# DerekGloudemans/3D-playground

Hardware: AMD Instinct MI355X
Metric: training images/sec at 1920x1080, ResNet-50 3D-RetinaNet (higher is better)
Workload: dtype f32; 1 GPU; resnet50 directional 3D-RetinaNet, 1920x1080 synthetic frames, batch 8 per GPU, 10 GT boxes/image, fp32, fwd+loss+bwd+clip+Adam (BASELINE configs[1]); global_batch=8, parallelism=dp1

## Files before the change

### 3d-playground_amd/csrc/conv_igemm_mf16.hip

```cpp
#include <type_traits>

#include "conv_igemm_tile.h"
#include "conv_wgrad_geom.h"

typedef float f32x4a __attribute__((ext_vector_type(4)));

#ifndef RN_MF16_STG
#define RN_MF16_STG 1
#endif
#ifndef RN_MF16_PF
#define RN_MF16_PF 1
#endif
#ifndef RN_MF16_KO
#define RN_MF16_KO 0
#endif

#define RN_SPLIT_MFMA16(ACC, A, B)                                                        \
    do {                                                                                  \
        ACC = __builtin_amdgcn_mfma_f32_16x16x32_bf16((A).l, (B).h, ACC, 0, 0, 0);        \
        ACC = __builtin_amdgcn_mfma_f32_16x16x32_bf16((A).h, (B).l, ACC, 0, 0, 0);        \
        ACC = __builtin_amdgcn_mfma_f32_16x16x32_bf16((A).m, (B).m, ACC, 0, 0, 0);        \
        ACC = __builtin_amdgcn_mfma_f32_16x16x32_bf16((A).m, (B).h, ACC, 0, 0, 0);        \
        ACC = __builtin_amdgcn_mfma_f32_16x16x32_bf16((A).h, (B).m, ACC, 0, 0, 0);        \
        ACC = __builtin_amdgcn_mfma_f32_16x16x32_bf16((A).h, (B).h, ACC, 0, 0, 0);        \
// ... 311 lines not shown
                        float4 t = *reinterpret_cast<const float4 *>(T + r * LDT + 4 * c4);
                        if constexpr (HALF) { const float ru = row_unscale[32 * wave + 16 * sm + hp * SR + r]; t.x *= ru; t.y *= ru; t.z *= ru; t.w *= ru; }
                        const int64_t off = off_[i];
                        float mk[4] = {mk_[i].x, mk_[i].y, mk_[i].z, mk_[i].w}, ad[4] = {ad_[i].x, ad_[i].y, ad_[i].z, ad_[i].w};
                        if (!RAW && d.add2_mode == 3) {
                            int64_t a2;
                            { RN_EPI_ADDR(GENERAL) a2 = a2off; (void)aoff; (void)off; }
                            if (a2 >= 0) { const float4 q = *reinterpret_cast<const float4 *>(add2 + a2); ad[0] += q.x; ad[1] += q.y; ad[2] += q.z; ad[3] += q.w; }
                        }
#if RN_MF16_KO & 4
                        if (t.x != 1.2345f) continue;
#endif
                        if (RAW) *reinterpret_cast<float4 *>(y + off) = HALF ? make_float4(t.x * sc[0], t.y * sc[1], t.z * sc[2], t.w * sc[3]) : t;
                        else { RN_EPI_FINISH() }
                    }
                }
            }
        }
        __builtin_amdgcn_fence(__ATOMIC_RELEASE, "wavefront");
        __builtin_amdgcn_wave_barrier();
    }
    if (!RAW && !rn_span) rn_amax_note(d.y_amax, m0 / HoWo, rn_am);
}

#ifndef RN_MF16H_OCC
#define RN_MF16H_OCC 3
#endif
template <bool GENERAL, bool RAW, int TERMS, bool STG, int WV = 4>
__global__ __launch_bounds__(64 * WV, WV == 8 ? 2 : (TERMS == 2 ? RN_MF16H_OCC : 3)) void conv_igemm_mf16_kernel(const rn_conv_desc d, const float *__restrict__ x,
                                                              const float *__restrict__ w, float *__restrict__ y,
                                                              const float *__restrict__ scale, const float *__restrict__ shift,
                                                              const float *__restrict__ add, const float *__restrict__ mask,
                                                              const float *__restrict__ add2) {
    conv_mf16_tile<GENERAL, RAW, TERMS, STG, WV>(d, x, w, y, scale, shift, add, mask, add2, xcd_remap(blockIdx.x, gridDim.x));
}

template <int TERMS>
__global__ __launch_bounds__(256, TERMS == 2 ? RN_MF16H_OCC : 3) void conv_igemm_mf16_grouped_kernel(const rn_conv_group g, const float *__restrict__ w,
                                                                      const float *__restrict__ scale,
                                                                      const float *__restrict__ shift) {
    const int tile = xcd_remap(blockIdx.x, gridDim.x);
    const int p = rn_group_index(g, tile);
    rn_conv_desc d = g.d[0];
    const float *x = g.x[0], *add = g.add[0], *mask = g.mask[0];
    float *y = g.y[0];
    int first = 0;
#pragma unroll
    for (int i = 1; i < RN_MAX_GROUP; ++i)
        if (p == i) { d = g.d[i]; x = g.x[i]; y = g.y[i]; add = g.add[i]; mask = g.mask[i]; first = g.tile_end[i - 1]; }
    conv_mf16_tile<true, false, TERMS, TERMS == 2 && RN_MF16_STG != 0>(d, x, w, y, scale, shift, add, mask, nullptr, tile - first);
}

static int mf16_on() { return rn_get_option(RN_OPT_MF16); }
static int mf16_min_tiles() { return rn_get_option(RN_OPT_MF16_MIN); }
static bool mf16_geom_ok(const rn_conv_desc *d) {
    return (d->Cin % 32) == 0 && d->div_shift == 0 && d->kh * d->kw <= 24 && (d->Cout % 4) == 0 && d->Cout > 64 && !d->in_relu;
}
static bool mf16_ok(const rn_conv_desc *d) {
    if (!mf16_on() || !mf16_geom_ok(d)) return false;
    if (d->w_format == 3) return d->x_amax != nullptr && d->w_unscale != nullptr;
    return d->w_format == 1;
}
static int64_t mf16_tiles(const rn_conv_desc *d) { return rn_conv_tiles(d, 128, 128); }

extern "C" int rn_conv_igemm_wants_f16(const rn_conv_desc *d) {
    return rn_get_fp32_mfma() == RN_FP32_SPLIT3 && d->w_batch_stride >= 0;
}

bool rn_igemm_mf16_launch(int variant, const rn_conv_desc *d, const float *x, const float *w, float *y, const float *scale,
                          const float *shift, const float *add, const float *mask, const float *add2, hipStream_t s, int *rc) {
    if (!mf16_ok(d) || (variant != 0 && variant != 4 && variant != 5)) return false;
    const int64_t tiles = mf16_tiles(d);
    if (tiles < mf16_min_tiles() || tiles > 0x7fffffff) return false;
    const dim3 grid((unsigned)tiles), block(256);
#define RN_MF16_LAUNCH(G, R, T, S) hipLaunchKernelGGL((conv_igemm_mf16_kernel<G, R, T, S>), grid, block, 0, s, *d, x, w, y, scale, shift, add, mask, add2)
    if (d->w_format == 3) {
        static const int stg_min_k = rn_env_int("RN_MF16_STG_MIN_K", 256);
        const bool stg = RN_MF16_STG != 0 && d->kh * d->kw * d->Cin >= stg_min_k;
        static const int wv8_min = rn_env_int("RN_MF16_WV8_MIN", 1);
        const int64_t tiles8 = rn_conv_tiles(d, 256, 128);
        if (stg && wv8_min > 0 && d->w_batch_stride == 0 && tiles8 >= wv8_min && tiles8 <= 0x7fffffff) {
            const dim3 grid8((unsigned)tiles8), block8(512);
#define RN_MF16_LAUNCH8(G, R) hipLaunchKernelGGL((conv_igemm_mf16_kernel<G, R, 2, true, 8>), grid8, block8, 0, s, *d, x, w, y, scale, shift, add, mask, add2)
            if (variant == 0) RN_MF16_LAUNCH8(false, true);
            else if (variant == 4) RN_MF16_LAUNCH8(false, false);
            else RN_MF16_LAUNCH8(true, false);
#undef RN_MF16_LAUNCH8
        } else
        if (variant == 0) { if (stg) RN_MF16_LAUNCH(false, true, 2, true); else RN_MF16_LAUNCH(false, true, 2, false); }
        else if (variant == 4) { if (stg) RN_MF16_LAUNCH(false, false, 2, true); else RN_MF16_LAUNCH(false, false, 2, false); }
        else { if (stg) RN_MF16_LAUNCH(true, false, 2, true); else RN_MF16_LAUNCH(true, false, 2, false); }
    } else {
        if (variant == 0) RN_MF16_LAUNCH(false, true, 3, false);
        else if (variant == 4) RN_MF16_LAUNCH(false, false, 3, false);
        else RN_MF16_LAUNCH(true, false, 3, false);
    }
#undef RN_MF16_LAUNCH
    const hipError_t e = hipGetLastError();
    *rc = e == hipSuccess ? RN_OK : (int)e;
    return true;
}

bool rn_igemm_mf16_grouped_launch(const rn_conv_group *g, const float *w, const float *scale, const float *shift, hipStream_t s, int *rc) {
    for (int i = 0; i < g->n; ++i)
        if (!mf16_ok(&g->d[i]) || g->d[i].w_format != g->d[0].w_format) return false;
    rn_conv_group gb = *g;
// ... 14 lines not shown
```

### 3d-playground_amd/csrc/conv_wgrad.hip

```cpp
#include <stdlib.h>
#include <type_traits>

#include "common.h"
#include "conv_wgrad_geom.h"

#ifndef RN_WG_KO
#define RN_WG_KO 0
#endif
#if RN_WG_KO == 1
#define RN_WG_ATOMIC(P, V) do { if ((V) == 1.2345e-30f) atomicAdd((P), (V)); } while (0)
#elif RN_WG_KO == 2
#define RN_WG_ATOMIC(P, V) __hip_atomic_fetch_add((P), (V), __ATOMIC_RELAXED, __HIP_MEMORY_SCOPE_WORKGROUP)
#else
#define RN_WG_ATOMIC(P, V) atomicAdd((P), (V))
#endif
#include "mfma_split.h"

typedef float f32x16 __attribute__((ext_vector_type(16)));
#define WK_MAX 32

struct WgradArgs {
    const float *dy, *x;
    float *dw;
    float *colsum;
    int ldy, N, Hi, Wi, Cin, Ho, Wo, Cout, kh, kw, stride, pad, in_relu;
    int Kflat, Kpad;
    int tiles_n;
    int tiles, splits;
    int xcd_map;
    int tiles_per_batch;
    int colsum_batch;
    int64_t dy_bstride, x_bstride, dw_bstride;
    int64_t pixels, per_split;
    float *slab, *cs_slab;
    int64_t slab_stride;
    const void *dy_amax, *x_amax;
    int dy_amax_n, x_amax_n;
};

__device__ __forceinline__ void wgrad_scales(const void *amax, int count, float &scale, float &unscale) {
    const int e = count > 0 ? rn_amax_exp_all(amax, count)
                            : (int)((__builtin_amdgcn_readfirstlane(*reinterpret_cast<const unsigned *>(amax)) >> 23) & 0xffu);
    const int se = rn_f16_scale_exp_of(e);
    scale = rn_exp_to_float(se);
    unscale = rn_exp_to_float(254 - se);
}

template <int WM, int WN, bool RELU, int WK, int OCC, bool SPLIT = false, bool HALF = false>
__global__ __launch_bounds__(256, OCC) void conv_wgrad_kernel(const WgradArgs p) {
    static_assert(!SPLIT || WK == 16, "split-operand form: 16-pixel K-steps");
    static_assert(!HALF || SPLIT, "the fp16 form is a split form");
    using G = WgradGeom<WM, WN, WK>;
    constexpr int BM = G::BM, BN = G::BN;
    constexpr int TB = G::TB;
    constexpr int CA = G::CA, CB = G::CB;
    constexpr int PA = G::PA, PB = G::PB;
    constexpr int IA = G::IA, IB = G::IB;
    __shared__ float lds[2][WK * (BM + BN)];
    __shared__ int4 pixtab[2][TB * WK];

    const int tid = threadIdx.x, lane = tid & 63, wave = tid >> 6;
    const int wm = wave / WN, wn = wave % WN;
    int slice, tile;
    if (p.xcd_map) {
        const int xcd = blockIdx.x & 7, wi = blockIdx.x >> 3;
        slice = (wi / p.tiles) * 8 + xcd;
        tile = wi % p.tiles;
    } else {
        slice = blockIdx.x / p.tiles;
        tile = blockIdx.x % p.tiles;
// ... 183 lines not shown
                if (c + 1 < p.Cout) atomicAdd(p.colsum + c + 1, cs.y);
            }
        }
    }
    float *out = dw_b;
    if (p.slab != nullptr) out = p.slab + (int64_t)slice * p.slab_stride + (int64_t)batch * p.dw_bstride;
#pragma unroll
    for (int tm = 0; tm < 2; ++tm)
#pragma unroll
        for (int tn = 0; tn < 2; ++tn) {
            const int col = n0 + wn * 64 + tn * 32 + (lane & 31);
#pragma unroll
            for (int e = 0; e < 16; ++e) {
                const int row = m0 + wm * 64 + 2 * ((e & 3) + 8 * (e >> 2) + 4 * (lane >> 5)) + tm;
                if (row < p.Cout && col < p.Kflat) {
                    const float v = HALF ? acc[tm][tn][e] * us : acc[tm][tn][e];
                    if (p.slab != nullptr) out[(int64_t)row * p.Kpad + col] = v;
                    else RN_WG_ATOMIC(out + (int64_t)row * p.Kpad + col, v);
                }
            }
        }
}

typedef short s16x4w __attribute__((ext_vector_type(4)));
__device__ __forceinline__ bf16x8 wgs_operand(const char *img, unsigned a0, unsigned a1) {
    typedef __attribute__((address_space(3))) s16x4w *lp;
    const s16x4w lo = __builtin_amdgcn_ds_read_tr16_b64_v4i16((lp)(__attribute__((address_space(3))) char *)(img + a0));
    const s16x4w hi = __builtin_amdgcn_ds_read_tr16_b64_v4i16((lp)(__attribute__((address_space(3))) char *)(img + a1));
    typedef short s16x8w __attribute__((ext_vector_type(8)));
    const s16x8w v = {lo[0], lo[1], lo[2], lo[3], hi[0], hi[1], hi[2], hi[3]};
    return __builtin_bit_cast(bf16x8, v);
}

template <bool RELU, bool HALF = false>
__global__ __launch_bounds__(256, 3) void conv_wgrad_once_kernel(const WgradArgs p) {
    using G = WgradSplitGeom;
    constexpr int BM = 128, BN = 128, WK = G::WK, TB = G::TB;
    constexpr int NP = HALF ? 2 : 3;
    constexpr int BUFB = 2 * NP * G::IMG;
    static_assert(BUFB <= G::BUF && 8 * BM * 4 <= BUFB, "planes fit; the column-sum reduction fits a buffer");
    __shared__ __attribute__((aligned(16))) char lds[2][BUFB];
    __shared__ int2 pixtab[2][TB * WK];

    const int tid = threadIdx.x, lane = tid & 63, wave = tid >> 6;
    const int wm = wave >> 1, wn = wave & 1;
    int slice, tile;
    if (p.xcd_map) {
        const int xcd = blockIdx.x & 7, wi = blockIdx.x >> 3;
        slice = (wi / p.tiles) * 8 + xcd;
        tile = wi % p.tiles;
    } else {
        slice = blockIdx.x / p.tiles;
        tile = blockIdx.x % p.tiles;
    }
    if (slice >= p.splits) return;
    const int batch = tile / p.tiles_per_batch;
    tile -= batch * p.tiles_per_batch;
    const float *dy_b = p.dy + (int64_t)batch * p.dy_bstride;
    const float *x_b = p.x + (int64_t)batch * p.x_bstride;
    float *dw_b = p.dw + (int64_t)batch * p.dw_bstride;
    const int m0 = (tile / p.tiles_n) * BM, n0 = (tile % p.tiles_n) * BN;
    const int64_t kbeg = (int64_t)slice * p.per_split;
    const int64_t kend = (kbeg + p.per_split < p.pixels) ? kbeg + p.per_split : p.pixels;
    const int nks = (int)((kend - kbeg + WK - 1) / WK);
    if (nks <= 0) return;
    const int HoWo = p.Ho * p.Wo;
    const int n_first = (int)(kbeg / HoWo);
    const int rel0 = (int)(kbeg - (int64_t)n_first * HoWo);
    const int64_t img = (int64_t)p.Hi * p.Wi * p.Cin;
    int64_t xbytes = ((int64_t)p.N - n_first) * img * 4;
    if (xbytes > 0x7FFFFFFF) xbytes = 0x7FFFFFFF;
    const __amdgpu_buffer_rsrc_t rs_a = __builtin_amdgcn_make_buffer_rsrc(const_cast<float *>(dy_b + kbeg * p.ldy), (short)0,
                                                                          (int)(unsigned)((kend - kbeg) * p.ldy * 4), 0x00020000);
    const __amdgpu_buffer_rsrc_t rs_b = __builtin_amdgcn_make_buffer_rsrc(const_cast<float *>(x_b + (int64_t)n_first * img), (short)0,
                                                                          (int)(unsigned)xbytes, 0x00020000);
    const int c = G::chunk(tid), px0 = G::pixel(tid, 0);
    const bool a_col_ok = (m0 + 4 * c) < p.ldy;
    const unsigned a_voff = a_col_ok ? (unsigned)((px0 * p.ldy + m0 + 4 * c) * 4) : 0x80000000u;
    const unsigned a_half = (unsigned)(8 * p.ldy * 4);
    const int jcol = n0 + 4 * c;
    const int tap = jcol / p.Cin;
    const int ci0 = jcol - tap * p.Cin;
    const int fr = tap / p.kw, fs = tap - fr * p.kw;
    const int fr_t = jcol < p.Kflat ? fr : (1 << 24);
    const int tap_off = ((fr * p.Wi + fs) * p.Cin + ci0) * 4;
    const unsigned wr0 = (unsigned)G::wr_addr(tid, 0), wr1 = (unsigned)G::wr_addr(tid, 1);

    auto fill_batch = [&](int j) {
        const int rel = rel0 + j * (TB * WK) + tid;
        int2 e = make_int2(0, 0x8000);
        if (kbeg + (int64_t)j * (TB * WK) + tid < kend) {
            const unsigned n = (unsigned)rel / (unsigned)HoWo;
            const unsigned rem = (unsigned)rel - n * (unsigned)HoWo;
            const unsigned oh = rem / (unsigned)p.Wo, ow = rem - oh * (unsigned)p.Wo;
            const int ih0 = (int)oh * p.stride - p.pad, iw0 = (int)ow * p.stride - p.pad;
            e = make_int2((((int)n * p.Hi + ih0) * p.Wi + iw0) * p.Cin * 4, (ih0 & 0xffff) | (iw0 << 16));
        }
        pixtab[j & 1][tid] = e;
    };
    typedef float f32x4v __attribute__((ext_vector_type(4)));
    struct Regs { f32x4v a[2], b[2]; };
    auto load_step = [&](int ks, Regs &r) {
        const int2 *tab = pixtab[(ks / TB) & 1];
        const unsigned so = (unsigned)ks * (unsigned)(WK * 4) * (unsigned)p.ldy;
        r.a[0] = __builtin_bit_cast(f32x4v, __builtin_amdgcn_raw_buffer_load_b128(rs_a, (int)a_voff, (int)so, 0));
        r.a[1] = __builtin_bit_cast(f32x4v, __builtin_amdgcn_raw_buffer_load_b128(rs_a, (int)a_voff, (int)(so + a_half), 0));
#pragma unroll
        for (int h = 0; h < 2; ++h) {
            const int2 e = tab[G::tab_index(ks, tid, h)];
            const int ih0 = (int)(short)(e.y & 0xffff), iw0 = e.y >> 16;
            const unsigned ok = (((unsigned)(ih0 + fr_t) < (unsigned)p.Hi) & ((unsigned)(iw0 + fs) < (unsigned)p.Wi)) ? 0xFFFFFFFFu : 0u;
            const unsigned v = ((unsigned)(e.x + tap_off) & ok) | (0x80000000u & ~ok);
            r.b[h] = __builtin_bit_cast(f32x4v, __builtin_amdgcn_raw_buffer_load_b128(rs_b, (int)v, 0, 0));
        }
    };
    float cs4[4] = {0.f, 0.f, 0.f, 0.f};
    const bool do_cs = p.colsum != nullptr && batch == p.colsum_batch && (tile % p.tiles_n) == 0;
    float s_a = 1.f, s_b = 1.f, us = 1.f;
    if constexpr (HALF) {
        float ua, ub;
        wgrad_scales(p.dy_amax, p.dy_amax_n, s_a, ua);
        wgrad_scales(p.x_amax, p.x_amax_n, s_b, ub);
        us = ua * ub;
    }
    auto split_store = [&](int buf, const Regs &r) {
        char *B = &lds[buf][0];
#pragma unroll
        for (int h = 0; h < 2; ++h) {
            const unsigned wr = h ? wr1 : wr0;
            float av[4] = {r.a[h][0], r.a[h][1], r.a[h][2], r.a[h][3]};
            float bv[4] = {r.b[h][0], r.b[h][1], r.b[h][2], r.b[h][3]};
            if (RELU) {
#pragma unroll
                for (int j = 0; j < 4; ++j) bv[j] = fmaxf(bv[j], 0.f);
            }
// ... 12 lines not shown
                *reinterpret_cast<uint2 *>(B + 2 * G::IMG + wr) = make_uint2(bh[0], bh[1]);
                *reinterpret_cast<uint2 *>(B + 3 * G::IMG + wr) = make_uint2(bl[0], bl[1]);
                continue;
            }
            unsigned ah[2], am[2], al[2], bh[2], bm[2], bl[2];
            split_pair(av[0], av[1], ah[0], am[0], al[0]);
            split_pair(av[2], av[3], ah[1], am[1], al[1]);
            split_pair(bv[0], bv[1], bh[0], bm[0], bl[0]);
            split_pair(bv[2], bv[3], bh[1], bm[1], bl[1]);
            *reinterpret_cast<uint2 *>(B + 0 * G::IMG + wr) = make_uint2(ah[0], ah[1]);
            *reinterpret_cast<uint2 *>(B + 1 * G::IMG + wr) = make_uint2(am[0], am[1]);
            *reinterpret_cast<uint2 *>(B + 2 * G::IMG + wr) = make_uint2(al[0], al[1]);
            *reinterpret_cast<uint2 *>(B + 3 * G::IMG + wr) = make_uint2(bh[0], bh[1]);
            *reinterpret_cast<uint2 *>(B + 4 * G::IMG + wr) = make_uint2(bm[0], bm[1]);
            *reinterpret_cast<uint2 *>(B + 5 * G::IMG + wr) = make_uint2(bl[0], bl[1]);
        }
    };
    unsigned fa[2][2], fb[2][2];
#pragma unroll
    for (int t = 0; t < 2; ++t)
#pragma unroll
        for (int rd = 0; rd < 2; ++rd) {
            fa[t][rd] = (unsigned)G::tr_addr(wm, t, rd, lane);
            fb[t][rd] = (unsigned)(NP * G::IMG + G::tr_addr(wn, t, rd, lane));
        }
    f32x16 acc[2][2];
#pragma unroll
    for (int i = 0; i < 2; ++i)
#pragma unroll
        for (int j = 0; j < 2; ++j)
#pragma unroll
            for (int e_ = 0; e_ < 16; ++e_) acc[i][j][e_] = 0.f;

    fill_batch(0);
    __syncthreads();
    Regs r0, r1;
    load_step(0, r0);
    split_store(0, r0);
    load_step(1, r0);
    __syncthreads();
    auto k_step = [&](int ks, int buf, Regs &cur, Regs &nxt) {
        const char *S = &lds[buf][0];
        if constexpr (HALF) {
            SplitH8 sa[2], sb[2];
#pragma unroll
            for (int t = 0; t < 2; ++t) {
                sa[t].h = __builtin_bit_cast(f16x8, wgs_operand(S, fa[t][0], fa[t][1]));
                sa[t].l = __builtin_bit_cast(f16x8, wgs_operand(S + G::IMG, fa[t][0], fa[t][1]));
                sb[t].h = __builtin_bit_cast(f16x8, wgs_operand(S, fb[t][0], fb[t][1]));
                sb[t].l = __builtin_bit_cast(f16x8, wgs_operand(S + G::IMG, fb[t][0], fb[t][1]));
            }
            split_store(buf ^ 1, cur);
            load_step(ks + 2, nxt);
#pragma unroll
            for (int tm = 0; tm < 2; ++tm)
#pragma unroll
                for (int tn = 0; tn < 2; ++tn) RN_SPLITH_MFMA(acc[tm][tn], sa[tm], sb[tn]);
        } else {
        Split8 sa[2], sb[2];
#pragma unroll
        for (int t = 0; t < 2; ++t) {
            sa[t].h = wgs_operand(S, fa[t][0], fa[t][1]);
            sa[t].m = wgs_operand(S + G::IMG, fa[t][0], fa[t][1]);
            sa[t].l = wgs_operand(S + 2 * G::IMG, fa[t][0], fa[t][1]);
            sb[t].h = wgs_operand(S, fb[t][0], fb[t][1]);
            sb[t].m = wgs_operand(S + G::IMG, fb[t][0], fb[t][1]);
            sb[t].l = wgs_operand(S + 2 * G::IMG, fb[t][0], fb[t][1]);
        }
        split_store(buf ^ 1, cur);
        load_step(ks + 2, nxt);
#pragma unroll
        for (int tm = 0; tm < 2; ++tm)
#pragma unroll
            for (int tn = 0; tn < 2; ++tn) RN_SPLIT_MFMA(acc[tm][tn], sa[tm], sb[tn]);
        }
        if ((ks % TB) == 4 && (ks / TB + 1) * TB < nks + 2) fill_batch(ks / TB + 1);
        __syncthreads();
    };
    for (int ks = 0; ks < nks; ks += 2) {
        k_step(ks, 0, r0, r1);
        if (ks + 1 < nks) k_step(ks + 1, 1, r1, r0);
    }
    if (do_cs) {
        float (*csred)[BM] = reinterpret_cast<float (*)[BM]>(&lds[0][0]);
#pragma unroll
        for (int j = 0; j < 4; ++j) csred[tid >> 5][4 * c + j] = cs4[j];
        __syncthreads();
        if (tid < BM) {
            float s_ = 0.f;
#pragma unroll
            for (int k = 0; k < 8; ++k) s_ += csred[k][tid];
            const int ch = m0 + tid;
            if (ch < p.Cout) {
                if (p.cs_slab != nullptr) p.cs_slab[(int64_t)slice * p.Cout + ch] = s_;
                else atomicAdd(p.colsum + ch, s_);
            }
        }
    }
    float *out = dw_b;
    if (p.slab != nullptr) out = p.slab + (int64_t)slice * p.slab_stride + (int64_t)batch * p.dw_bstride;
#pragma unroll
    for (int tm = 0; tm < 2; ++tm)
#pragma unroll
        for (int tn = 0; tn < 2; ++tn) {
            const int col = n0 + wn * 64 + tn * 32 + (lane & 31);
#pragma unroll
            for (int e = 0; e < 16; ++e) {
                const int row = m0 + wm * 64 + tm * 32 + (e & 3) + 8 * (e >> 2) + 4 * (lane >> 5);
                if (row < p.Cout && col < p.Kflat) {
                    const float v = HALF ? acc[tm][tn][e] * us : acc[tm][tn][e];
                    if (p.slab != nullptr) out[(int64_t)row * p.Kpad + col] = v;
                    else RN_WG_ATOMIC(out + (int64_t)row * p.Kpad + col, v);
                }
            }
        }
}

__global__ __launch_bounds__(256) void wgrad_combine_kernel(float *__restrict__ dw, const float *__restrict__ slab, int64_t slab_stride,
                                                            int splits, int nbatch, int64_t dw_bstride, int Cout, int Kflat, int Kpad,
                                                            float *__restrict__ colsum, const float *__restrict__ cs_slab) {
    const int64_t per = (int64_t)Cout * Kflat, total = per * nbatch;
    const int64_t i = (int64_t)blockIdx.x * 256 + threadIdx.x;
    if (i < total) {
        const int64_t b = i / per, r = i - b * per;
        const int row = (int)(r / Kflat), col = (int)(r - (int64_t)row * Kflat);
        const int64_t e = b * dw_bstride + (int64_t)row * Kpad + col;
        float v = dw[e];
        for (int s = 0; s < splits; ++s) v += slab[(int64_t)s * slab_stride + e];
        dw[e] = v;
    }
    if (colsum != nullptr && i < Cout) {
        float v = colsum[i];
        for (int s = 0; s < splits; ++s) v += cs_slab[(int64_t)s * Cout + i];
        colsum[i] = v;
    }
}

static int wgrad_launch(const float *dy, int ldy, const float *x, float *dw, float *colsum, int nbatch,
                        int64_t dy_bstride, int64_t x_bstride, int64_t dw_bstride, int colsum_batch, int N, int Hi,
                        int Wi, int Cin, int Ho, int Wo, int Cout, int kh, int kw, int stride, int pad,
                        int in_relu, void *stream, bool det, void *workspace, int64_t workspace_bytes, int64_t *need_bytes,
                        const void *dy_amax = nullptr, int dy_amax_n = 0, const void *x_amax = nullptr, int x_amax_n = 0);

extern "C" int rn_conv_wgrad_batched(const float *dy, int ldy, const float *x, float *dw, float *colsum, int nbatch,
                                     int64_t dy_bstride, int64_t x_bstride, int64_t dw_bstride, int colsum_batch, int N, int Hi,
                                     int Wi, int Cin, int Ho, int Wo, int Cout, int kh, int kw, int stride, int pad,
                                     int in_relu, const void *dy_amax, int dy_amax_n, const void *x_amax, int x_amax_n, void *stream) {
    return wgrad_launch(dy, ldy, x, dw, colsum, nbatch, dy_bstride, x_bstride, dw_bstride, colsum_batch, N, Hi, Wi, Cin, Ho, Wo, Cout,
                        kh, kw, stride, pad, in_relu, stream, false, nullptr, 0, nullptr, dy_amax, dy_amax_n, x_amax, x_amax_n);
}

extern "C" int rn_conv_wgrad_batched_det(const float *dy, int ldy, const float *x, float *dw, float *colsum, int nbatch,
                                         int64_t dy_bstride, int64_t x_bstride, int64_t dw_bstride, int colsum_batch, int N, int Hi,
                                         int Wi, int Cin, int Ho, int Wo, int Cout, int kh, int kw, int stride, int pad,
                                         int in_relu, const void *dy_amax, int dy_amax_n, const void *x_amax, int x_amax_n,
                                         void *workspace, int64_t workspace_bytes, void *stream) {
    if (workspace == nullptr) return RN_EINVAL;
    return wgrad_launch(dy, ldy, x, dw, colsum, nbatch, dy_bstride, x_bstride, dw_bstride, colsum_batch, N, Hi, Wi, Cin, Ho, Wo, Cout,
                        kh, kw, stride, pad, in_relu, stream, true, workspace, workspace_bytes, nullptr, dy_amax, dy_amax_n, x_amax, x_amax_n);
}

extern "C" int64_t rn_conv_wgrad_det_workspace_bytes(int ldy, int nbatch, int64_t dw_bstride, int N, int Hi, int Wi, int Cin, int Ho,
                                                     int Wo, int Cout, int kh, int kw) {
    int64_t need = 0;
    const int rc = wgrad_launch(nullptr, ldy, nullptr, nullptr, nullptr, nbatch, 0, 0, dw_bstride, 0, N, Hi, Wi, Cin, Ho, Wo, Cout, kh, kw,
                                1, 0, 0, nullptr, true, nullptr, 0, &need);
    return rc == RN_OK ? need : -1;
}

static int wgrad_launch(const float *dy, int ldy, const float *x, float *dw, float *colsum, int nbatch,
                        int64_t dy_bstride, int64_t x_bstride, int64_t dw_bstride, int colsum_batch, int N, int Hi,
                        int Wi, int Cin, int Ho, int Wo, int Cout, int kh, int kw, int stride, int pad,
                        int in_relu, void *stream, bool det, void *workspace, int64_t workspace_bytes, int64_t *need_bytes,
                        const void *dy_amax, int dy_amax_n, const void *x_amax, int x_amax_n) {
    if (N <= 0 || Hi <= 0 || Wi <= 0 || Ho <= 0 || Wo <= 0 || Cout <= 0 || Cin < 4 || (Cin & 3) || (ldy & 3) || ldy < Cout)
        return RN_EINVAL;
    if (nbatch < 1 || nbatch > 4096 || dy_bstride < 0 || x_bstride < 0 || dw_bstride < 0 || colsum_batch < 0 || colsum_batch >= nbatch)
        return RN_EINVAL;
    WgradArgs a;
    a.dy_bstride = dy_bstride; a.x_bstride = x_bstride; a.dw_bstride = dw_bstride; a.colsum_batch = colsum_batch;
    a.dy = dy; a.x = x; a.dw = dw; a.colsum = colsum; a.ldy = ldy;
    a.N = N; a.Hi = Hi; a.Wi = Wi; a.Cin = Cin; a.Ho = Ho; a.Wo = Wo; a.Cout = Cout;
    a.kh = kh; a.kw = kw; a.stride = stride; a.pad = pad; a.in_relu = in_relu;
    a.Kflat = kh * kw * Cin;
    a.Kpad = (a.Kflat + 31) / 32 * 32;
    a.pixels = (int64_t)N * Ho * Wo;
    const int shape = Cout <= 64 ? 0 : (a.Kflat <= 64 ? 1 : 2);
    const int BM = shape == 0 ? 64 : (shape == 1 ? 256 : 128), BN = shape == 0 ? 256 : (shape == 1 ? 64 : 128);
    const int tiles_m = (Cout + BM - 1) / BM;
    a.tiles_n = (a.Kflat + BN - 1) / BN;
    a.tiles_per_batch = tiles_m * a.tiles_n;
    const int tiles = a.tiles_per_batch * nbatch;
    static const int wgs_native = rn_env_int("RN_WGRAD_WGS", 2048);
    static const int wgs_split = rn_env_int("RN_WGRAD_SPLIT_WGS", 1536);
    const int wg_target = rn_get_fp32_mfma() != RN_FP32_NATIVE ? wgs_split : wgs_native;
    int64_t splits = (wg_target + tiles - 1) / tiles;
    const int64_t max_splits = (a.pixels + 16 * WK_MAX - 1) / (16 * WK_MAX);
    if (splits > max_splits) splits = max_splits;
    if (splits < 1) splits = 1;
    if (splits > 65535) splits = 65535;
    a.xcd_map = tiles >= 16 && splits > 8 && splits + 7 <= max_splits;
    if (a.xcd_map) splits = (splits + 7) / 8 * 8;
    const int64_t HoWo = (int64_t)Ho * Wo, img_bytes = (int64_t)Hi * Wi * Cin * 4;
    for (;;) {
        a.per_split = ((a.pixels + splits - 1) / splits + WK_MAX - 1) / WK_MAX * WK_MAX;
        const int64_t span_imgs = (a.per_split + HoWo - 2) / HoWo + 1;
        if ((a.per_split + WK_MAX) * ldy * 4 <= 0x7FFFFFFF && span_imgs * img_bytes <= 0x7FFFFFFF) break;
        if (a.per_split <= WK_MAX || splits >= 65535) return RN_EINVAL;
        splits = splits * 2 > 65535 ? 65535 : splits * 2;
        a.xcd_map = 0;
    }
    splits = (a.pixels + a.per_split - 1) / a.per_split;
    a.tiles = tiles;
    a.splits = (int)splits;
    a.slab = a.cs_slab = nullptr;
    a.slab_stride = 0;
    if (det) {
        a.slab_stride = nbatch > 1 ? (int64_t)nbatch * dw_bstride : (int64_t)Cout * a.Kpad;
        const int64_t need = splits * (a.slab_stride + Cout) * (int64_t)sizeof(float);
        if (need_bytes != nullptr) { *need_bytes = need; return RN_OK; }
        if (workspace_bytes < need) return RN_EINVAL;
        a.slab = reinterpret_cast<float *>(workspace);
        a.cs_slab = a.slab + splits * a.slab_stride;
    }
    const dim3 grid((unsigned)(tiles * (a.xcd_map ? (splits + 7) / 8 * 8 : splits)));
    const bool split = rn_get_fp32_mfma() != RN_FP32_NATIVE;
    const bool half = rn_get_fp32_mfma() == RN_FP32_SPLIT3 && dy_amax != nullptr && x_amax != nullptr && dy_amax_n != 0 && x_amax_n != 0;
    a.dy_amax = dy_amax;
    a.x_amax = x_amax;
    a.dy_amax_n = dy_amax_n;
    a.x_amax_n = x_amax_n;
#define RN_WGRAD_LAUNCH(WM_, WN_)                                                                                        \
    do {                                                                                                                 \
        if (half) {                                                                                                      \
            if (in_relu) hipLaunchKernelGGL((conv_wgrad_kernel<WM_, WN_, true, 16, 3, true, true>), grid, dim3(256), 0, (hipStream_t)stream, a);  \
            else hipLaunchKernelGGL((conv_wgrad_kernel<WM_, WN_, false, 16, 3, true, true>), grid, dim3(256), 0, (hipStream_t)stream, a);         \
        } else if (split) {                                                                                              \
            if (in_relu) hipLaunchKernelGGL((conv_wgrad_kernel<WM_, WN_, true, 16, 3, true>), grid, dim3(256), 0, (hipStream_t)stream, a);  \
            else hipLaunchKernelGGL((conv_wgrad_kernel<WM_, WN_, false, 16, 3, true>), grid, dim3(256), 0, (hipStream_t)stream, a);         \
        } else if (in_relu) hipLaunchKernelGGL((conv_wgrad_kernel<WM_, WN_, true, 16, 3>), grid, dim3(256), 0, (hipStream_t)stream, a);  \
        else hipLaunchKernelGGL((conv_wgrad_kernel<WM_, WN_, false, 16, 3>), grid, dim3(256), 0, (hipStream_t)stream, a);         \
    } while (0)
    const bool once = split && shape == 2 && rn_get_option(RN_OPT_WGRAD_ONCE) != 0 && Hi + pad < 32000 && Wi + pad < 32000;
    if (once && half) {
        if (in_relu) hipLaunchKernelGGL((conv_wgrad_once_kernel<true, true>), grid, dim3(256), 0, (hipStream_t)stream, a);
        else hipLaunchKernelGGL((conv_wgrad_once_kernel<false, true>), grid, dim3(256), 0, (hipStream_t)stream, a);
    } else if (once) {
        if (in_relu) hipLaunchKernelGGL((conv_wgrad_once_kernel<true>), grid, dim3(256), 0, (hipStream_t)stream, a);
        else hipLaunchKernelGGL((conv_wgrad_once_kernel<false>), grid, dim3(256), 0, (hipStream_t)stream, a);
    } else if (shape == 0) RN_WGRAD_LAUNCH(1, 4);
    else if (shape == 1) RN_WGRAD_LAUNCH(4, 1);
    else RN_WGRAD_LAUNCH(2, 2);
#undef RN_WGRAD_LAUNCH
    RN_LAUNCH_CHECK();
    if (det) {
        const int64_t total = (int64_t)nbatch * Cout * a.Kflat;
        hipLaunchKernelGGL(wgrad_combine_kernel, dim3((unsigned)((total + 255) / 256)), dim3(256), 0, (hipStream_t)stream, dw,
                           (const float *)a.slab, a.slab_stride, a.splits, nbatch, dw_bstride, Cout, a.Kflat, a.Kpad, colsum,
                           (const float *)a.cs_slab);
        RN_LAUNCH_CHECK();
    }
    return RN_OK;
}

extern "C" int rn_conv_wgrad(const float *dy, int ldy, const float *x, float *dw, float *colsum, int N, int Hi, int Wi,
                             int Cin, int Ho, int Wo, int Cout, int kh, int kw, int stride, int pad, int in_relu,
                             void *stream) {
    return rn_conv_wgrad_batched(dy, ldy, x, dw, colsum, 1, 0, 0, 0, 0, N, Hi, Wi, Cin, Ho, Wo, Cout, kh, kw, stride, pad,
                                 in_relu, nullptr, 0, nullptr, 0, stream);
}
```

### 3d-playground_amd/csrc/conv_wino.hip

```cpp
#include "common.h"
#include "mfma_split.h"

__device__ __forceinline__ float4 f4(float s) { return make_float4(s, s, s, s); }
typedef float nt_f4 __attribute__((ext_vector_type(4)));
__device__ __forceinline__ float4 ld_stream(const float *p) {
    const nt_f4 v = __builtin_nontemporal_load(reinterpret_cast<const nt_f4 *>(p));
    return make_float4(v.x, v.y, v.z, v.w);
}
__device__ __forceinline__ void st_stream(float *p, float4 v) { *reinterpret_cast<float4 *>(p) = v; }
__device__ __forceinline__ float4 operator+(float4 a, float4 b) { return make_float4(a.x + b.x, a.y + b.y, a.z + b.z, a.w + b.w); }
__device__ __forceinline__ float4 operator-(float4 a, float4 b) { return make_float4(a.x - b.x, a.y - b.y, a.z - b.z, a.w - b.w); }
__device__ __forceinline__ float4 operator*(float s, float4 a) { return make_float4(s * a.x, s * a.y, s * a.z, s * a.w); }

__device__ __forceinline__ void bt6(const float4 d[6], float4 o[6]) {
    o[0] = 4.f * d[0] - 5.f * d[2] + d[4];
    o[1] = d[3] + d[4] - 4.f * (d[1] + d[2]);
    o[2] = 4.f * (d[1] - d[2]) - d[3] + d[4];
    o[3] = 2.f * (d[3] - d[1]) - d[2] + d[4];
    o[4] = 2.f * (d[1] - d[3]) - d[2] + d[4];
    o[5] = 4.f * d[1] - 5.f * d[3] + d[5];
}
__device__ __forceinline__ void at6(const float4 m[6], float4 o[4]) {
    const float4 s12 = m[1] + m[2], d12 = m[1] - m[2], s34 = m[3] + m[4], d34 = m[3] - m[4];
    o[0] = m[0] + s12 + s34;
// ... 66 lines not shown
        const int e_img = rn_amax_exp_lanes(xw != nullptr ? reinterpret_cast<const unsigned char *>(xw) + (int64_t)n * RN_AMAX_BYTES : nullptr);
        if (gt_raw < t_last && c4 == 0) row_amax[t0 + gt] = rn_amax_word_of_exp(e_img, WINO_GAIN_BT);
    }
    if (gt_raw >= t_last) return;
    float4 t[6][6];
#pragma unroll
    for (int j = 0; j < 6; ++j) {
        float4 d[6], o[6];
        const int w = w0 + j;
#pragma unroll
        for (int i = 0; i < 6; ++i) {
            const int h = h0 + i;
#ifdef RN_WINO_ABL
            const bool ok = (unsigned)h < (unsigned)H && (unsigned)w < (unsigned)W && i >= 1 && i <= 4 && j >= 1 && j <= 4;
#else
            const bool ok = (unsigned)h < (unsigned)H && (unsigned)w < (unsigned)W;
#endif
            d[i] = ok ? *reinterpret_cast<const float4 *>(xb + ((int64_t)h * W + w) * C) : f4(0.f);
        }
        bt6(d, o);
#pragma unroll
        for (int i = 0; i < 6; ++i) t[i][j] = o[i];
    }
    float *vb = V + (t0 + gt) * C + c4;
#pragma unroll
    for (int i = 0; i < 6; ++i) {
        float4 o[6];
        bt6(t[i], o);
#pragma unroll
        for (int j = 0; j < 6; ++j) st_stream(vb + (int64_t)(i * 6 + j) * Tpad * C, o[j]);
    }
}

template <bool PBITS, bool PADD>
__global__ __launch_bounds__(256, 2) void wino_out_kernel(const WinoTable g, const float *__restrict__ M, int Cout, int64_t t0,
                                                       int64_t Tpad, const float *__restrict__ scale,
                                                       const float *__restrict__ shift, int mask_mode, int act, int64_t y_bs) {
    const int cq = Cout >> 2;
    const int64_t id = (int64_t)blockIdx.x * 256 + threadIdx.x;
    const int64_t gt = id / cq;
    float am = 0.f;
    unsigned *yam = nullptr;
    int n_img = 0;
    bool live = false;
    do {
    if (gt >= g.tile_end[g.n - 1]) break;
    live = true;
    const int c4 = (int)(id - gt * cq) * 4;
    int64_t tile;
    const int q = wino_locate(g, gt, tile);
    float *y = g.dst[0];
    const float *add = g.add[0], *mask = g.mask[0];
    unsigned *sign = g.sign[0];
    yam = g.amax[0];
    WINO_SELECT(q, g, pr, y = g.dst[i_]; add = g.add[i_]; mask = g.mask[i_]; sign = g.sign[i_]; yam = g.amax[i_];)
    n_img = (int)(tile / (pr.TH * pr.TW));
    const bool mbits = (mask_mode & RN_MASK_BITS) != 0;
    mask_mode &= 3;
    const int H = pr.H, W = pr.W, TW = pr.TW;
    const int n = (int)(tile / (pr.TH * TW));
    const int r = (int)(tile - (int64_t)n * pr.TH * TW);
    const int th = r / TW, tw = r - th * TW;
    const float *mb = M + (t0 + gt) * Cout + c4;
    float4 t[4][6];
#pragma unroll
    for (int j = 0; j < 6; ++j) {
        float4 m[6], o[4];
#pragma unroll
        for (int i = 0; i < 6; ++i) m[i] = ld_stream(mb + (int64_t)(i * 6 + j) * Tpad * Cout);
        at6(m, o);
#pragma unroll
        for (int i = 0; i < 4; ++i) t[i][j] = o[i];
    }
    float4 sc = f4(1.f), sh = f4(0.f);
    if (scale) sc = *reinterpret_cast<const float4 *>(scale + c4);
    if (shift) sh = *reinterpret_cast<const float4 *>(shift + c4);
    const int64_t ybs = y_bs ? y_bs : (int64_t)H * W * Cout;
#pragma unroll
    for (int i = 0; i < 4; ++i) {
        float4 o[4];
        at6(t[i], o);
        const int oh = 4 * th + i;
        if (oh >= H) break;
        unsigned mkw[4];
        float4 adv[4];
        if constexpr (PBITS || PADD) {
#pragma unroll
            for (int j = 0; j < 4; ++j) {
                const int owc = 4 * tw + j < W ? 4 * tw + j : W - 1;
                const int64_t off = (((int64_t)n * H + oh) * W + owc) * Cout + c4;
                if constexpr (PBITS) mkw[j] = reinterpret_cast<const unsigned *>(mask)[off >> 5] >> ((unsigned)off & 28u);
                if constexpr (PADD) adv[j] = *reinterpret_cast<const float4 *>(add + off);
            }
        }
#pragma unroll
        for (int j = 0; j < 4; ++j) {
            const int ow = 4 * tw + j;
            if (ow >= W) break;
            const int64_t off = (((int64_t)n * H + oh) * W + ow) * Cout + c4;
            const int64_t yoff = (int64_t)n * ybs + ((int64_t)oh * W + ow) * Cout + c4;
            float v[4] = {sc.x * o[j].x + sh.x, sc.y * o[j].y + sh.y, sc.z * o[j].z + sh.z, sc.w * o[j].w + sh.w};
            float mk[4] = {1.f, 1.f, 1.f, 1.f}, ad[4] = {0.f, 0.f, 0.f, 0.f};
            if constexpr (PBITS) {
                const unsigned nb = mkw[j];
                mk[0] = (nb & 1u) ? 1.f : 0.f; mk[1] = (nb & 2u) ? 1.f : 0.f; mk[2] = (nb & 4u) ? 1.f : 0.f; mk[3] = (nb & 8u) ? 1.f : 0.f;
            } else if (mask_mode != 0) { const float4 q4 = rn_mask_load4(mask, off, mbits); mk[0] = q4.x; mk[1] = q4.y; mk[2] = q4.z; mk[3] = q4.w; }
            if constexpr (PADD) { const float4 q4 = adv[j]; ad[0] = q4.x; ad[1] = q4.y; ad[2] = q4.z; ad[3] = q4.w; }
            else if (add) { const float4 q4 = *reinterpret_cast<const float4 *>(add + off); ad[0] = q4.x; ad[1] = q4.y; ad[2] = q4.z; ad[3] = q4.w; }
#pragma unroll
            for (int k = 0; k < 4; ++k) {
                float u = v[k];
                if (mask_mode == 1) u = mk[k] > 0.f ? u : 0.f;
                u += ad[k];
                if (act == 1) u = fmaxf(u, 0.f);
                else if (act == 2) u = 1.0f / (1.0f + expf(-u));
                if (mask_mode == 2) u = mk[k] > 0.f ? u : 0.f;
                v[k] = u;
            }
            *reinterpret_cast<float4 *>(y + yoff) = make_float4(v[0], v[1], v[2], v[3]);
            if (sign != nullptr) rn_sign_store(sign, off, v[0], v[1], v[2], v[3]);
            am = fmaxf(fmaxf(am, fmaxf(fabsf(v[0]), fabsf(v[1]))), fmaxf(fabsf(v[2]), fabsf(v[3])));
        }
    }
    } while (0);
    if (live) rn_amax_note(yam, n_img, am);
}

__global__ void wino_weight_kernel(const float *__restrict__ w, float *__restrict__ U, int Cout, int Cin, int mode,
                                   const float *__restrict__ scale, int rows, int Kpad) {
    const int64_t id = (int64_t)blockIdx.x * 256 + threadIdx.x;
    if (id >= (int64_t)rows * Kpad) return;
    const int row = (int)(id / Kpad), k = (int)(id - (int64_t)row * Kpad);
    const int kdim = mode == 0 ? Cin : Cout;
    float g[3][3];
#pragma unroll
    for (int r = 0; r < 3; ++r)
#pragma unroll
        for (int s = 0; s < 3; ++s) {
            float v = 0.f;
            if (k < kdim) {
                if (mode == 0) v = w[(((int64_t)row * Cin + k) * 3 + r) * 3 + s];
                else v = w[(((int64_t)k * Cin + row) * 3 + (2 - r)) * 3 + (2 - s)] * (scale ? scale[k] : 1.f);
            }
            g[r][s] = v;
        }
    float t[6][3];
#pragma unroll
    for (int s = 0; s < 3; ++s) {
        const float a = g[0][s], b = g[1][s], c = g[2][s];
        t[0][s] = a * (1.f / 4.f);
        t[1][s] = -(a + b + c) * (1.f / 6.f);
        t[2][s] = (b - a - c) * (1.f / 6.f);
        t[3][s] = a * (1.f / 24.f) + b * (1.f / 12.f) + c * (1.f / 6.f);
        t[4][s] = a * (1.f / 24.f) - b * (1.f / 12.f) + c * (1.f / 6.f);
// ... 32 lines not shown
    int64_t tile;
    const int q = wino_locate(g, gt, tile);
    const float *dy = g.src[0];
    WINO_SELECT(q, g, pr, dy = g.src[i_];)
    const int H = pr.H, W = pr.W, TW = pr.TW;
    const int n = (int)(tile / (pr.TH * TW));
    const int r = (int)(tile - (int64_t)n * pr.TH * TW);
    const int th = r / TW, tw = r - th * TW;
    const float *yb = dy + (int64_t)n * H * W * C + c4;
    float4 t[6][4];
#pragma unroll
    for (int j = 0; j < 4; ++j) {
        float4 v[4], o[6];
        const int w = 4 * tw + j;
#pragma unroll
        for (int i = 0; i < 4; ++i) {
            const int h = 4 * th + i;
            v[i] = (h < H && w < W) ? *reinterpret_cast<const float4 *>(yb + ((int64_t)h * W + w) * C) : f4(0.f);
        }
        a6(v, o);
#pragma unroll
        for (int a = 0; a < 6; ++a) t[a][j] = o[a];
    }
    float *zb = Z + (t0 + gt) * C + c4;
#pragma unroll
    for (int a = 0; a < 6; ++a) {
        float4 o[6];
        a6(t[a], o);
#pragma unroll
        for (int b = 0; b < 6; ++b) st_stream(zb + (int64_t)(a * 6 + b) * Tpad * C, o[b]);
    }
}

__global__ __launch_bounds__(256) void wino_in_both_kernel(const WinoTable g, float *__restrict__ V, float *__restrict__ Z, int C,
                                                           int64_t t0, int64_t Tpad, unsigned *__restrict__ v_row_amax,
                                                           unsigned *__restrict__ z_tensor_amax) {
    wino_tensor_word(g, z_tensor_amax, WINO_GAIN_A);
    const int cq = C >> 2;
    const int64_t id = (int64_t)xcd_remap(blockIdx.x, gridDim.x) * 256 + threadIdx.x;
    const int64_t gt_raw = id / cq, t_last = g.tile_end[g.n - 1];
    const int64_t gt = gt_raw < t_last ? gt_raw : t_last - 1;
    const int c4 = (int)(id - gt_raw * cq) * 4;
    int64_t tile;
    const int q = wino_locate(g, gt, tile);
    const float *x = g.src[0];
    const unsigned *xw = g.amax[0];
    WINO_SELECT(q, g, pr, x = g.src[i_]; xw = g.amax[i_];)
    const int H = pr.H, W = pr.W, TW = pr.TW;
    const int n = (int)(tile / (pr.TH * TW));
    const int r = (int)(tile - (int64_t)n * pr.TH * TW);
    const int th = r / TW, tw = r - th * TW;
    const int h0 = 4 * th - 1, w0 = 4 * tw - 1;
    const float *xb = x + (int64_t)n * H * W * C + c4;
    if (v_row_amax != nullptr) {
        const int e_img = rn_amax_exp_lanes(xw != nullptr ? reinterpret_cast<const unsigned char *>(xw) + (int64_t)n * RN_AMAX_BYTES : nullptr);
        if (gt_raw < t_last && c4 == 0) v_row_amax[t0 + gt] = rn_amax_word_of_exp(e_img, WINO_GAIN_BT);
    }
    if (gt_raw >= t_last) return;
    float4 t[6][6];
    float4 tz[6][4];
#pragma unroll
    for (int j = 0; j < 6; ++j) {
        float4 d[6], o[6];
        const int w = w0 + j;
#pragma unroll
        for (int i = 0; i < 6; ++i) {
            const int h = h0 + i;
            const bool ok = (unsigned)h < (unsigned)H && (unsigned)w < (unsigned)W;
            d[i] = ok ? *reinterpret_cast<const float4 *>(xb + ((int64_t)h * W + w) * C) : f4(0.f);
        }
        bt6(d, o);
#pragma unroll
        for (int i = 0; i < 6; ++i) t[i][j] = o[i];
        if (j >= 1 && j <= 4) {
            float4 oz[6];
            a6(d + 1, oz);
#pragma unroll
            for (int a = 0; a < 6; ++a) tz[a][j - 1] = oz[a];
        }
    }
    float *zb = Z + (t0 + gt) * C + c4;
#pragma unroll
    for (int a = 0; a < 6; ++a) {
        float4 o[6];
        a6(tz[a], o);
#pragma unroll
        for (int b = 0; b < 6; ++b) st_stream(zb + (int64_t)(a * 6 + b) * Tpad * C, o[b]);
    }
    float *vb = V + (t0 + gt) * C + c4;
#pragma unroll
    for (int i = 0; i < 6; ++i) {
// ... 36 lines not shown
    int64_t end = 0;
    for (int i = 0; i < RN_MAX_GROUP; ++i) {
        const int k = i < g->n ? i : g->n - 1;
        if (g->N[k] <= 0 || g->H[k] <= 0 || g->W[k] <= 0) return RN_EINVAL;
        t.p[i].N = g->N[k]; t.p[i].H = g->H[k]; t.p[i].W = g->W[k];
        t.p[i].TH = (g->H[k] + 3) / 4; t.p[i].TW = (g->W[k] + 3) / 4;
        if (i < g->n) end += (int64_t)g->N[k] * t.p[i].TH * t.p[i].TW;
        t.tile_end[i] = end;
        t.src[i] = g->src[k]; t.dst[i] = g->dst[k]; t.add[i] = g->add[k]; t.mask[i] = g->mask[k];
        t.sign[i] = reinterpret_cast<unsigned *>(g->sign[k]);
        t.amax[i] = reinterpret_cast<unsigned *>(g->amax[k]);
    }
    return RN_OK;
}

extern "C" int rn_wino_input_group(const rn_wino_group *g, float *V, int C, int64_t tile_offset, int64_t Tpad, int dy_form,
                                   void *row_amax, void *tensor_amax, void *stream) {
    WinoTable t;
    const int rc = wino_table(g, t);
    if (rc) return rc;
    if (C <= 0 || (C & 3) || tile_offset < 0 || tile_offset + t.tile_end[t.n - 1] > Tpad) return RN_EINVAL;
    for (int i = 0; i < t.n; ++i)
        if (!t.src[i]) return RN_EINVAL;
    const dim3 grid(rn_blocks(t.tile_end[t.n - 1] * (C >> 2), 256));
    if (dy_form && row_amax != nullptr) return RN_EINVAL;
    if (dy_form) hipLaunchKernelGGL(wino_dy_kernel, grid, dim3(256), 0, (hipStream_t)stream, t, V, C, tile_offset, Tpad,
                                    reinterpret_cast<unsigned *>(tensor_amax));
    else hipLaunchKernelGGL(wino_in_kernel, grid, dim3(256), 0, (hipStream_t)stream, t, V, C, tile_offset, Tpad,
                            reinterpret_cast<unsigned *>(row_amax), reinterpret_cast<unsigned *>(tensor_amax));
    RN_LAUNCH_CHECK();
    return RN_OK;
}

extern "C" int rn_wino_input_both_group(const rn_wino_group *g, float *V, float *Z, int C, int64_t tile_offset, int64_t Tpad,
                                        void *v_row_amax, void *z_tensor_amax, void *stream) {
    WinoTable t;
    const int rc = wino_table(g, t);
    if (rc) return rc;
    if (!V || !Z || C <= 0 || (C & 3) || tile_offset < 0 || tile_offset + t.tile_end[t.n - 1] > Tpad) return RN_EINVAL;
    for (int i = 0; i < t.n; ++i)
        if (!t.src[i]) return RN_EINVAL;
    hipLaunchKernelGGL(wino_in_both_kernel, dim3(rn_blocks(t.tile_end[t.n - 1] * (C >> 2), 256)), dim3(256), 0, (hipStream_t)stream, t,
                       V, Z, C, tile_offset, Tpad, reinterpret_cast<unsigned *>(v_row_amax), reinterpret_cast<unsigned *>(z_tensor_amax));
    RN_LAUNCH_CHECK();
    return RN_OK;
}

extern "C" int rn_wino_output_group(const rn_wino_group *g, const float *M, int Cout, int64_t tile_offset, int64_t Tpad,
                                    const float *scale, const float *shift, int mask_mode, int act, int64_t y_batch_stride,
                                    void *stream) {
    WinoTable t;
    const int rc = wino_table(g, t);
    if (rc) return rc;
    if (Cout <= 0 || (Cout & 3) || tile_offset < 0 || tile_offset + t.tile_end[t.n - 1] > Tpad) return RN_EINVAL;
    if (mask_mode < 0 || (mask_mode & ~(3 | RN_MASK_BITS)) || (mask_mode & 3) == 3 || mask_mode == RN_MASK_BITS) return RN_EINVAL;
    if (act < 0 || act > 2 || y_batch_stride < 0 || (y_batch_stride & 3)) return RN_EINVAL;
    for (int i = 0; i < t.n; ++i) {
        if (!t.dst[i] || (mask_mode != 0) != (t.mask[i] != nullptr)) return RN_EINVAL;
        if (((mask_mode & RN_MASK_BITS) || t.sign[i]) && (Cout & 31)) return RN_EINVAL;
        if (y_batch_stride && y_batch_stride < (int64_t)t.p[i].H * t.p[i].W * Cout) return RN_EINVAL;
    }
    const bool pbits = (mask_mode & RN_MASK_BITS) != 0;
    bool padd = true;
    for (int i = 0; i < t.n; ++i) padd = padd && t.add[i] != nullptr;
    const dim3 grid(rn_blocks(t.tile_end[t.n - 1] * (Cout >> 2), 256));
#define RN_WINO_OUT(B, A) hipLaunchKernelGGL((wino_out_kernel<B, A>), grid, dim3(256), 0, (hipStream_t)stream, t, M, Cout, tile_offset, Tpad, \
                                             scale, shift, mask_mode, act, y_batch_stride)
    if (pbits && padd) RN_WINO_OUT(true, true);
    else if (pbits) RN_WINO_OUT(true, false);
    else if (padd) RN_WINO_OUT(false, true);
    else RN_WINO_OUT(false, false);
#undef RN_WINO_OUT
    RN_LAUNCH_CHECK();
    return RN_OK;
}

static rn_wino_group wino_single(const float *src, float *dst, const float *add, const float *mask, int N, int H, int W) {
    rn_wino_group g = {};
    g.n = 1; g.N[0] = N; g.H[0] = H; g.W[0] = W; g.src[0] = src; g.dst[0] = dst; g.add[0] = add; g.mask[0] = mask;
    return g;
}
extern "C" int rn_wino_input(const float *x, float *V, int N, int H, int W, int C, int64_t tile_offset, int64_t Tpad,
                             void *stream) {
    const rn_wino_group g = wino_single(x, nullptr, nullptr, nullptr, N, H, W);
    return rn_wino_input_group(&g, V, C, tile_offset, Tpad, 0, nullptr, nullptr, stream);
}
extern "C" int rn_wino_dy(const float *dy, float *Z, int N, int H, int W, int C, int64_t tile_offset, int64_t Tpad, void *stream) {
    const rn_wino_group g = wino_single(dy, nullptr, nullptr, nullptr, N, H, W);
    return rn_wino_input_group(&g, Z, C, tile_offset, Tpad, 1, nullptr, nullptr, stream);
}
extern "C" int rn_wino_output(const float *M, float *y, int N, int H, int W, int Cout, int64_t tile_offset, int64_t Tpad,
                              const float *scale, const float *shift, const float *add, const float *mask, int mask_mode,
                              int act, int64_t y_batch_stride, void *stream) {
    const rn_wino_group g = wino_single(nullptr, y, add, mask, N, H, W);
    return rn_wino_output_group(&g, M, Cout, tile_offset, Tpad, scale, shift, mask_mode, act, y_batch_stride, stream);
}

extern "C" int rn_wino_weights(const float *w, float *U, int Cout, int Cin, int mode, const float *scale, void *stream) {
    if (Cout <= 0 || Cin <= 0 || mode < 0 || mode > 1) return RN_EINVAL;
    const int rows = mode == 0 ? Cout : Cin;
    const int Kpad = ((mode == 0 ? Cin : Cout) + 31) / 32 * 32;
    hipLaunchKernelGGL(wino_weight_kernel, dim3(rn_blocks((int64_t)rows * Kpad, 256)), dim3(256), 0, (hipStream_t)stream, w, U,
                       Cout, Cin, mode, scale, rows, Kpad);
    RN_LAUNCH_CHECK();
    return RN_OK;
}

// ... 9 lines not shown
```

### 3d-playground_amd/csrc/elementwise.hip

```cpp
#include "common.h"
#include "mfma_split.h"

__global__ void pack_weights_kernel(const float *__restrict__ src, float *__restrict__ dst, int Cout, int Cin, int kh, int kw,
                                    int kw_pad, int c_pad, int mode, const float *__restrict__ scale, int rows, int Kpad,
                                    int r0, int nr, int s0, int ns) {
    const int64_t i = (int64_t)blockIdx.x * 256 + threadIdx.x;
    if (i >= (int64_t)rows * Kpad) return;
    const int row = (int)(i / Kpad), k = (int)(i - (int64_t)row * Kpad);
    const int tap = k / c_pad, c = k - tap * c_pad;
    int r = tap / kw_pad, s = tap - r * kw_pad;
    bool in_filter = r < kh && s < kw;
    if (mode == 2) {
        r = tap / ns;
        s = tap - r * ns;
        in_filter = r < nr;
        r = r0 + 2 * r;
        s = s0 + 2 * s;
    }
    float v = 0.f;
    if (in_filter) {
        if (mode == 0) {
            if (c < Cin) v = src[(((int64_t)row * Cin + c) * kh + r) * kw + s];
        } else {
            if (c < Cout) {
// ... 399 lines not shown
extern "C" int rn_relu_mask(float *g, const float *z, int64_t n, void *stream) {
    if (n <= 0) return RN_EINVAL;
    hipLaunchKernelGGL(relu_mask_kernel, dim3(rn_blocks(n, 256)), dim3(256), 0, (hipStream_t)stream, g, z, n);
    RN_LAUNCH_CHECK();
    return RN_OK;
}

__global__ void sigmoid_bwd_pad_kernel(const float *__restrict__ dy, const float *__restrict__ s, float *__restrict__ out,
                                       int64_t rows, int64_t rpi, int C, int ld, int64_t bstride, unsigned *__restrict__ amax) {
    const int64_t i = (int64_t)blockIdx.x * 256 + threadIdx.x;
    if (i >= rows * ld) return;
    const int64_t r = i / ld;
    const int c = (int)(i - r * ld);
    const int64_t b = r / rpi;
    float v = 0.f;
    if (c < C) {
        const int64_t src = b * bstride + (r - b * rpi) * C + c;
        v = dy[src];
        if (s) { const float p = s[src]; v *= p * (1.0f - p); }
    }
    out[i] = v;
    rn_amax_note(amax, b, fabsf(v));
}
extern "C" int rn_sigmoid_bwd_pad(const float *dy, const float *s, float *out, int B, int64_t rows_per_image, int C, int ld,
                                  int64_t src_batch_stride, void *amax, void *stream) {
    const int64_t rows = (int64_t)B * rows_per_image;
    if (rows <= 0 || C <= 0 || ld < C) return RN_EINVAL;
    hipLaunchKernelGGL(sigmoid_bwd_pad_kernel, dim3(rn_blocks(rows * ld, 256)), dim3(256), 0, (hipStream_t)stream, dy, s, out,
                       rows, rows_per_image, C, ld, src_batch_stride, reinterpret_cast<unsigned *>(amax));
    RN_LAUNCH_CHECK();
    return RN_OK;
}

__global__ void add_inplace_kernel(float *__restrict__ dst, const float *__restrict__ src, int64_t n, int64_t per_image, unsigned *__restrict__ amax) {
    const int64_t i = (int64_t)blockIdx.x * 256 + threadIdx.x;
    if (i >= n) return;
    const int64_t img = amax != nullptr ? i / per_image : 0;
    const float v = dst[i] + src[i];
    dst[i] = v;
    rn_amax_note(amax, img, fabsf(v));
}
extern "C" int rn_add_inplace(float *dst, const float *src, int64_t n, int64_t per_image, void *amax, void *stream) {
    if (n <= 0 || (amax != nullptr && per_image <= 0)) return RN_EINVAL;
    hipLaunchKernelGGL(add_inplace_kernel, dim3(rn_blocks(n, 256)), dim3(256), 0, (hipStream_t)stream, dst, src, n, per_image,
                       reinterpret_cast<unsigned *>(amax));
    RN_LAUNCH_CHECK();
    return RN_OK;
}
```

### 3d-playground_amd/retinanet_mi355x/_hip.py

```python
import ctypes
import os

import torch

_HERE = os.path.dirname(os.path.abspath(__file__))
LIB_PATH = os.environ.get("RN_LIB_PATH") or os.path.join(_HERE, "lib", "libretinanet_mi355x.so")
_lib = None

c_i32, c_i64, c_f32, c_f64, c_vp = ctypes.c_int, ctypes.c_int64, ctypes.c_float, ctypes.c_double, ctypes.c_void_p

SIGNATURES = {
    "rn_version": (ctypes.c_char_p, []),
    "rn_check_device": (c_i32, []),
    "rn_get_fp32_mfma": (c_i32, []),
    "rn_set_fp32_mfma": (c_i32, [c_i32]),
    "rn_get_option": (c_i32, [c_i32]),
    "rn_set_option": (c_i32, [c_i32, c_i32]),
    "rn_fp32_split_min_k": (c_i32, []),
    "rn_split_weights": (c_i32, [c_vp, c_vp, c_i64, c_i32, c_vp]),
    "rn_split_weights_f16": (c_i32, [c_vp, c_vp, c_vp, c_i64, c_i32, c_vp]),
    "rn_amax": (c_i32, [c_vp, c_i64, c_i32, c_vp, c_vp]),
    "rn_stream_capture_id": (c_i32, [c_vp, ctypes.POINTER(ctypes.c_ulonglong)]),
    "rn_anchor_count": (c_i64, [c_i32, c_i32]),
    "rn_anchor_base_boxes": (None, [c_vp]),
# ... 58 lines not shown
    "rn_vanishing_points": (c_i32, [c_vp, c_i64, c_vp, c_i64, c_vp, c_vp, c_vp, c_vp]),
    "rn_hg_reproj_error": (c_i32, [c_vp, c_vp, c_vp, c_vp, c_vp, c_i64, c_i64, c_vp, c_vp]),
    "rn_hg_scale_z": (c_i32, [c_vp, c_vp, c_vp, c_vp, c_i64, c_f64, c_f64, c_i32, c_vp, c_vp, c_vp, c_vp]),
    "rn_fit_homography": (c_i32, [c_vp, c_vp, c_i64, c_vp, c_i64, c_i32, c_vp, c_vp, c_vp]),
    "rn_reinterp_mate": (c_i32, [c_vp, c_vp, c_i64, c_i64, c_vp, c_vp, c_vp]),
    "rn_reinterp_offsets": (c_i32, [c_vp, c_vp, c_i64, c_i64, c_vp, c_i64] + [c_vp] * 5),
    "rn_reinterp_rows": (c_i32, [c_vp] * 7 + [c_i64] * 4 + [c_vp] * 5),
    "rn_track_rows": (c_i32, [c_vp] * 5 + [c_i64, c_i64] + [c_vp] * 7),
    "rn_render_edges": (c_i32, [c_vp, c_vp, c_i64, c_i32, c_i32, c_vp, c_i32, c_i32, c_i32, c_vp]),
    "rn_render_rects": (c_i32, [c_vp, c_i64, c_vp, c_i64, c_vp, c_i32, c_i32, c_i32, c_vp]),
    "rn_render_text": (c_i32, [c_vp, c_i64, c_vp, c_i64, c_vp, c_vp, c_i64, c_vp, c_i32, c_i32, c_i32, c_vp]),
    "rn_render_compose": (c_i32, [c_vp] + [c_f32] * 6 + [c_vp, c_i32, c_vp, c_i32, c_i32, c_i32, c_i32, c_vp]),
    "rn_replay_boxes": (c_i32, [c_vp, c_i64, c_vp, c_vp, c_vp, c_i32, c_vp, c_vp, c_vp, c_vp, c_vp]),
    "rn_replay_compose": (c_i32, [c_vp, c_i32, c_vp, c_vp] + [c_i32] * 6 + [c_vp]),
    "rn_frame_absdiff": (c_i32, [c_vp, c_vp] + [c_i32] * 6 + [c_vp, c_vp, c_vp]),
    "rn_running_frame": (c_i32, [c_vp, c_vp, c_i64, c_i32, c_vp]),
    "rn_label_pair_samples": (c_i32, [c_vp, c_vp, c_i64, c_i32, c_i64, c_i32, c_i32, c_i32, c_vp, c_vp, c_vp, c_vp]),
    "rn_label_outliers": (c_i32, [c_vp, c_vp, c_vp, c_i64, c_i64, c_i64, c_i64, c_vp, c_vp, c_vp]),
    "rn_label_interpolate_workspace_bytes": (c_i64, [c_i64, c_i64]),
    "rn_label_interpolate": (c_i32, [c_vp] * 4 + [c_i64] * 3 + [c_i32, c_i64] + [c_vp] * 7),
}

class ConvDesc(ctypes.Structure):
    _fields_ = [("N", c_i32), ("Hi", c_i32), ("Wi", c_i32), ("Cin", c_i32),
                ("Ho", c_i32), ("Wo", c_i32), ("Cout", c_i32),
                ("kh", c_i32), ("kw", c_i32),
                ("a", c_i32), ("b", c_i32), ("p", c_i32), ("p_w", c_i32), ("div_shift", c_i32),
                ("act", c_i32), ("add_mode", c_i32), ("Ha", c_i32), ("Wa", c_i32),
                ("mask_mode", c_i32), ("in_relu", c_i32),
                ("os", c_i32), ("oo_h", c_i32), ("oo_w", c_i32), ("Hy", c_i32), ("Wy", c_i32),
                ("add2_mode", c_i32), ("Ha2", c_i32), ("Wa2", c_i32), ("add2_batch_stride", c_i64),
                ("x_batch_stride", c_i64), ("y_batch_stride", c_i64), ("add_batch_stride", c_i64),
                ("w_batch_stride", c_i64), ("w_format", c_i32), ("sign_out", c_vp),
                ("x_amax", c_vp), ("y_amax", c_vp), ("w_unscale", c_vp), ("x_amax_img_stride", c_i32), ("x_amax_row_stride", c_i32)]


RN_MAX_GROUP = 5


class ConvGroup(ctypes.Structure):
    _fields_ = [("n", c_i32), ("tile_end", c_i32 * RN_MAX_GROUP), ("d", ConvDesc * RN_MAX_GROUP),
                ("x", c_vp * RN_MAX_GROUP), ("y", c_vp * RN_MAX_GROUP), ("add", c_vp * RN_MAX_GROUP),
                ("mask", c_vp * RN_MAX_GROUP)]


class PrepJob(ctypes.Structure):
    _fields_ = [("kind", c_i32)] + [(n, c_i32) for n in ("Cout", "Cin", "kh", "kw", "kw_pad", "c_pad", "mode", "r0", "nr", "s0",
                                                          "ns", "rows", "Kpad")] + \
               [("eps", c_f32), ("src", c_vp), ("dst", c_vp), ("scale", c_vp), ("gamma", c_vp), ("beta", c_vp), ("mean", c_vp),
                ("var", c_vp), ("bn_scale", c_vp), ("bn_shift", c_vp), ("bn_rstd", c_vp)]


class UnpackJob(ctypes.Structure):
    _fields_ = [("dw", c_vp), ("w_packed", c_vp), ("dweight", c_vp)] + \
               [(n, c_i32) for n in ("Cout", "Cin", "kh", "kw", "kw_pad", "c_pad", "Kpad")] + \
               [("scale", c_vp), ("mean", c_vp), ("rstd", c_vp), ("colsum", c_vp), ("dgamma", c_vp), ("dbeta", c_vp)]


class WinoGroup(ctypes.Structure):
    _fields_ = [("n", c_i32), ("N", c_i32 * RN_MAX_GROUP), ("H", c_i32 * RN_MAX_GROUP), ("W", c_i32 * RN_MAX_GROUP),
                ("src", c_vp * RN_MAX_GROUP), ("dst", c_vp * RN_MAX_GROUP), ("add", c_vp * RN_MAX_GROUP),
                ("mask", c_vp * RN_MAX_GROUP), ("sign", c_vp * RN_MAX_GROUP), ("amax", c_vp * RN_MAX_GROUP)]


SIGNATURES.update({
    "rn_unpack_batched": (c_i32, [c_vp, c_vp, c_i32, c_vp]),
    "rn_prep_batched": (c_i32, [c_vp, c_vp, c_i32, c_vp]),
    "rn_wino_input_group": (c_i32, [ctypes.POINTER(WinoGroup), c_vp, c_i32, c_i64, c_i64, c_i32, c_vp, c_vp, c_vp]),
    "rn_wino_input_both_group": (c_i32, [ctypes.POINTER(WinoGroup), c_vp, c_vp, c_i32, c_i64, c_i64, c_vp, c_vp, c_vp]),
    "rn_wino_output_group": (c_i32, [ctypes.POINTER(WinoGroup), c_vp, c_i32, c_i64, c_i64, c_vp, c_vp, c_i32, c_i32, c_i64, c_vp]),
    "rn_conv_igemm_grouped": (c_i32, [ctypes.POINTER(ConvGroup), c_vp, c_vp, c_vp, c_vp]),
    "rn_conv_igemm": (c_i32, [ctypes.POINTER(ConvDesc), c_vp, c_vp, c_vp, c_vp, c_vp, c_vp, c_vp, c_vp, c_vp]),
    "rn_conv_splitk_workspace_bytes": (c_i64, [ctypes.POINTER(ConvDesc)]),
    "rn_conv_igemm_wants_f16": (c_i32, [ctypes.POINTER(ConvDesc)]),
    "rn_conv_igemm_splitk": (c_i32, [ctypes.POINTER(ConvDesc)] + [c_vp] * 10),
    "rn_conv_wgrad": (c_i32, [c_vp, c_i32, c_vp, c_vp, c_vp] + [c_i32] * 12 + [c_vp]),
    "rn_pack_weights": (c_i32, [c_vp, c_vp] + [c_i32] * 7 + [c_vp] + [c_i32] * 4 + [c_vp]),
    "rn_unpack_wgrad": (c_i32, [c_vp, c_vp, c_vp] + [c_i32] * 6 + [c_vp] * 7),
    "rn_bn_fold": (c_i32, [c_vp, c_vp, c_vp, c_vp, c_f32, c_i32, c_vp, c_vp, c_vp, c_vp]),
    "rn_nchw_to_nhwc4": (c_i32, [c_vp, c_vp, c_i32, c_i32, c_i32, c_vp, c_vp]),
    "rn_maxpool_fwd": (c_i32, [c_vp, c_vp, c_vp] + [c_i32] * 6 + [c_vp]),
    "rn_maxpool_bwd": (c_i32, [c_vp, c_vp, c_vp, c_vp] + [c_i32] * 7 + [c_vp, c_vp]),
    "rn_colsum": (c_i32, [c_vp, c_i64, c_i32, c_i32, c_vp, c_i32, c_vp, c_vp]),
    "rn_colsum_workspace_bytes": (c_i64, [c_i64, c_i32]),
    "rn_upsample_add_bwd": (c_i32, [c_vp, c_vp] + [c_i32] * 6 + [c_vp, c_vp]),
    "rn_relu_mask": (c_i32, [c_vp, c_vp, c_i64, c_vp]),
    "rn_sigmoid_bwd_pad": (c_i32, [c_vp, c_vp, c_vp, c_i32, c_i64, c_i32, c_i32, c_i64, c_vp, c_vp]),
    "rn_add_inplace": (c_i32, [c_vp, c_vp, c_i64, c_i64, c_vp, c_vp]),
    "rn_wino_input": (c_i32, [c_vp, c_vp, c_i32, c_i32, c_i32, c_i32, c_i64, c_i64, c_vp]),
    "rn_wino_output": (c_i32, [c_vp, c_vp, c_i32, c_i32, c_i32, c_i32, c_i64, c_i64, c_vp, c_vp, c_vp, c_vp, c_i32, c_i32, c_i64, c_vp]),
    "rn_wino_weights": (c_i32, [c_vp, c_vp, c_i32, c_i32, c_i32, c_vp, c_vp]),
    "rn_wino_dy": (c_i32, [c_vp, c_vp, c_i32, c_i32, c_i32, c_i32, c_i64, c_i64, c_vp]),
    "rn_wino_dw": (c_i32, [c_vp, c_vp, c_i32, c_i32, c_vp]),
    "rn_conv_wgrad_batched": (c_i32, [c_vp, c_i32, c_vp, c_vp, c_vp, c_i32, c_i64, c_i64, c_i64, c_i32] + [c_i32] * 12 + [c_vp, c_i32, c_vp, c_i32, c_vp]),
    "rn_conv_wgrad_batched_det": (c_i32, [c_vp, c_i32, c_vp, c_vp, c_vp, c_i32, c_i64, c_i64, c_i64, c_i32] + [c_i32] * 12 + [c_vp, c_i32, c_vp, c_i32, c_vp, c_i64, c_vp]),
    "rn_conv_wgrad_det_workspace_bytes": (c_i64, [c_i32, c_i32, c_i64] + [c_i32] * 9),
    "rn_f32_to_bf16": (c_i32, [c_vp, c_vp, c_i64, c_vp]),
    "rn_bf16_to_f32": (c_i32, [c_vp, c_vp, c_i64, c_vp]),
    "rn_conv_igemm_bf16": (c_i32, [ctypes.POINTER(ConvDesc), c_vp, c_vp, c_vp, c_i32, c_vp, c_vp, c_vp, c_vp, c_vp]),
    "rn_conv_igemm_bf16_grouped": (c_i32, [ctypes.POINTER(ConvGroup), c_vp, c_i32, c_vp, c_vp, c_vp]),
    "rn_conv_igemm_bf16_tile_rows": (c_i32, [ctypes.POINTER(ConvGroup), c_i32]),
    "rn_maxpool_fwd_fp8out": (c_i32, [c_vp, c_vp] + [c_i32] * 6 + [c_f32, c_vp]),
    "rn_conv_igemm_fp8_tile_rows": (c_i32, [ctypes.POINTER(ConvGroup), c_i32]),
    "rn_conv_igemm_fp8_tile": (c_i32, [ctypes.POINTER(ConvDesc), c_i32]),
    "rn_conv_igemm_bf16_tile": (c_i32, [ctypes.POINTER(ConvDesc), c_i32]),
    "rn_fp8_quantize": (c_i32, [c_vp, c_vp, c_i64, c_f32, c_vp]),
    "rn_fp8_dequantize": (c_i32, [c_vp, c_vp, c_i64, c_f32, c_vp]),
    "rn_fp8_to_bf16": (c_i32, [c_vp, c_vp, c_i64, c_f32, c_vp]),
    "rn_bf16_to_fp8": (c_i32, [c_vp, c_vp, c_i64, c_f32, c_vp]),
    "rn_fp8_quantize_rows": (c_i32, [c_vp, c_vp, c_vp, c_i64, c_i32, c_vp]),
    "rn_conv_igemm_fp8": (c_i32, [ctypes.POINTER(ConvDesc), c_vp, c_vp, c_vp, c_i32, c_vp, c_vp, c_vp, c_f32, c_f32, c_vp]),
    "rn_conv_igemm_fp8_grouped": (c_i32, [ctypes.POINTER(ConvGroup), c_vp, c_i32, c_vp, c_vp, c_f32, c_f32, c_vp]),
    "rn_conv_wgrad_bf16": (c_i32, [c_vp, c_i32, c_vp, c_vp, c_vp] + [c_i32] * 11 + [c_vp]),
    "rn_conv_wgrad_bf16_grouped": (c_i32, [c_i32, ctypes.POINTER(c_vp), c_i32, ctypes.POINTER(c_vp), c_vp, c_vp, c_i32,
                                           ctypes.POINTER(c_i32), ctypes.POINTER(c_i32)] + [c_i32] * 6 + [c_vp]),
    "rn_maxpool_fwd_bf16out": (c_i32, [c_vp, c_vp, c_vp] + [c_i32] * 6 + [c_vp]),
    "rn_maxpool_bwd_bf16in": (c_i32, [c_vp, c_vp, c_vp, c_vp] + [c_i32] * 7 + [c_vp]),
    "rn_upsample_add_bwd_bf16": (c_i32, [c_vp, c_vp] + [c_i32] * 6 + [c_vp]),
    "rn_sigmoid_bwd_pad_bf16": (c_i32, [c_vp, c_vp, c_vp, c_i32, c_i64, c_i32, c_i32, c_i64, c_vp]),
    "rn_relu_bf16": (c_i32, [c_vp, c_vp, c_i64, c_vp]),
    "rn_opt_workspace_bytes": (c_i64, [c_i32]),
    "rn_opt_clip_adam": (c_i32, [c_vp, c_vp, c_i32, c_f32, c_f32, c_f32, c_f32, c_f32, c_i32, c_i32, c_vp, c_vp, c_vp]),
    "rn_opt_clip_adam_dev": (c_i32, [c_vp, c_vp, c_i32, c_f32, c_f32, c_f32, c_f32, c_f32, c_vp, c_i32, c_vp, c_vp, c_vp]),
    "rn_opt_clip_adam_hp": (c_i32, [c_vp, c_vp, c_i32, c_vp, c_vp, c_i32, c_vp, c_vp, c_vp]),
})


RN_ERRORS = {10001: "RN_EINVAL (bad size / unsupported shape)",
# ... 43 lines not shown
```

### 3d-playground_amd/retinanet_mi355x/conv.py

```python
import ctypes
import os

import torch

from . import _hip, prof

ConvDesc = _hip.ConvDesc

ACT_NONE, ACT_RELU, ACT_SIGMOID = 0, 1, 2


def kpad(kh, kw, c):
    return (kh * kw * c + 31) // 32 * 32


def out_size(n, k, stride, pad):
    return (n + 2 * pad - k) // stride + 1


def pack_weights(weight, mode=0, scale=None, kw_pad=None, c_pad=None, taps=None, presplit=True):
    lib = _hip.load()
    w = _hip.f32c(weight.detach())
    _hip.need_gpu(w, scale)
    cout, cin, kh, kw = w.shape
# ... 9 lines not shown
    out = torch.empty((rows, (ktaps * c_pad + 31) // 32 * 32), dtype=torch.float32, device=w.device)
    _hip.check(lib.rn_pack_weights(w.data_ptr(), out.data_ptr(), cout, cin, kh, kw, kw_pad, c_pad, mode,
                                   _hip.ptr(scale), r0, nr, s0, ns, _hip.stream()), "rn_pack_weights")
    return _maybe_split(out, rows=rows, cin=c_pad, taps=ktaps) if presplit else out


BITMASKS = os.environ.get("RN_BITMASKS", "1") != "0"
BITMASKS_BF16 = os.environ.get("RN_BITMASKS_BF16", "0") == "1"
MASK_BITS = 4


def _sign_words(y, want):
    if hasattr(y, "_rn_sign"):
        del y._rn_sign
    if not (want and BITMASKS) or y.dtype not in (torch.float32, torch.bfloat16) or y.shape[-1] % 32 or not y.is_contiguous():
        return None
    bits = torch.empty(y.numel() // 32, dtype=torch.int32, device=y.device)
    y._rn_sign = bits
    return bits


def _mask_operand(mask, mask_mode):
    if mask is None:
        return None, 0
    bits = getattr(mask, "_rn_sign", None) if BITMASKS else None
    if bits is not None:
        return bits.data_ptr(), mask_mode | MASK_BITS
    return mask.data_ptr(), mask_mode


def conv_igemm(x, w_packed, y, geom, scale=None, shift=None, add=None, add_mode=0, add_hw=(0, 0), mask=None,
               mask_mode=2, act=ACT_NONE, y_batch_stride=None, add_batch_stride=None, in_relu=False, flops=0.0,
               out_map=None, add2=None, w_batch_stride=0, kind=None, sign=False, bf16_products=False, x_amax=None, x_amax_rows=False,
               amax=None):
    lib = _hip.load()
    N, Hi, Wi, Cin = x.shape
    Ho, Wo, Cout, kh, kw, a, b, p, ds = geom
    p_h, p_w = p if isinstance(p, tuple) else (p, p)
    os_, oo_h, oo_w, Hy, Wy = (1, 0, 0, Ho, Wo) if out_map is None else out_map
    ybs = Hy * Wy * Cout if y_batch_stride is None else y_batch_stride
    if add_batch_stride is None:
        add_batch_stride = ybs if add_mode == 1 else add_hw[0] * add_hw[1] * Cout
    a2 = (0, 0, 0, 0) if add2 is None else (3, add2.shape[1], add2.shape[2], add2.shape[1] * add2.shape[2] * Cout)
    mask_ptr, mask_mode = _mask_operand(mask, mask_mode)
    d = ConvDesc(N, Hi, Wi, Cin, Ho, Wo, Cout, kh, kw, a, b, p_h, p_w, ds, act, add_mode, add_hw[0], add_hw[1],
                 mask_mode, int(in_relu), os_, oo_h, oo_w, Hy, Wy,
                 a2[0], a2[1], a2[2], a2[3], Hi * Wi * Cin, ybs, add_batch_stride, w_batch_stride)
    amax_drop(y)
    bits = _sign_words(y, sign and y_batch_stride is None and out_map is None)
    d.sign_out = None if bits is None else bits.data_ptr()
    yam = None
    if want_amax() and not w_batch_stride and y_batch_stride is None and (out_map is None or amax is not None):
        yam = amax if amax is not None else amax_slot(y.device, N)
        d.y_amax = yam.data_ptr()
    if kind is None:
        kind = "conv_igemm_4x1" if Cout <= 64 else "conv_igemm_2x2"
    if prof.BY_SHAPE:
        kind += " %dx%dx%d %d->%d k%d a%d b%d ds%d%s" % (N, Ho, Wo, Cin, Cout, kh, a, b, ds, " x36" if w_batch_stride else "")
    ws_bytes = 0 if w_batch_stride else lib.rn_conv_splitk_workspace_bytes(ctypes.byref(d))
    if ws_bytes > 0:
        ws = torch.empty(ws_bytes, dtype=torch.uint8, device=x.device)
        rc = prof.timed(kind, flops, lambda: lib.rn_conv_igemm_splitk(
            ctypes.byref(d), x.data_ptr(), w_packed.data_ptr(), y.data_ptr(), _hip.ptr(scale), _hip.ptr(shift),
            _hip.ptr(add), mask_ptr, _hip.ptr(add2), ws.data_ptr(), _hip.stream()))
        _hip.check(rc, "rn_conv_igemm_splitk")
        if yam is not None and amax is None:
            amax_attach(y, yam)
        return y
    wptr, d.w_format, d.w_unscale = _w_operand(w_packed, d)
    if d.w_format == 3:
        d.x_amax = (x_amax if x_amax is not None else amax_words(x)).data_ptr()
        d.x_amax_img_stride, d.x_amax_row_stride = (0, 1) if x_amax_rows else (1, 0)
    if bf16_products:
        ws = getattr(w_packed, "_rn_split", None)
        if ws is None:
            ws = split_weights(w_packed)._rn_split
        wptr, d.w_format = ws.data_ptr(), 2
    nb = 0.0
    if prof.ACTIVE is not None:
        out_el = N * Ho * Wo * Cout
        mask_el = 0.0 if mask is None else (1.0 / 32 if mask_mode & MASK_BITS else 1.0)
# ... 150 lines not shown


def amax_carry(view, src):
    w = getattr(src, "_rn_amax_words", None)
    if w is not None and w.numel() == view.shape[0] * AMAX_SUB:
        amax_attach(view, w)
    return view


def amax_drop(t):
    if hasattr(t, "_rn_amax"):
        del t._rn_amax


def want_amax():
    return get_fp32_mfma() == "split3"


OPT_SPLITK, OPT_DETERMINISTIC, OPT_MF16, OPT_MF16_MIN, OPT_WGRAD_ONCE, OPT_BF16_P8, OPT_FP8_P8 = range(7)


def set_option(option, value):
    _hip.check(_hip.load().rn_set_option(option, int(value)), "rn_set_option")


def get_option(option):
    return int(_hip.load().rn_get_option(option))


def set_deterministic(on=True):
    set_option(OPT_DETERMINISTIC, on)


def _wgrad_call(lib, dev, dy_ptr, ldy, x_ptr, dw_ptr, cs_ptr, nbatch, dy_bs, x_bs, dw_bs, cs_batch, geom, amax=(None, None)):
    cnt = lambda a: 0 if a is None else (-1 if a.numel() == 1 else a.numel() // AMAX_SUB)
    am = (_hip.ptr(amax[0]), cnt(amax[0]), _hip.ptr(amax[1]), cnt(amax[1]))
    if not lib.rn_get_option(OPT_DETERMINISTIC):
        return lib.rn_conv_wgrad_batched(dy_ptr, ldy, x_ptr, dw_ptr, cs_ptr, nbatch, dy_bs, x_bs, dw_bs, cs_batch, *geom, *am, _hip.stream())
    N, Hi, Wi, Cin, Ho, Wo, Cout, kh, kw = geom[:9]
    nb = lib.rn_conv_wgrad_det_workspace_bytes(ldy, nbatch, dw_bs, N, Hi, Wi, Cin, Ho, Wo, Cout, kh, kw)
    if nb < 0:
        return 1
    ws = torch.empty(nb, dtype=torch.uint8, device=dev)
    return lib.rn_conv_wgrad_batched_det(dy_ptr, ldy, x_ptr, dw_ptr, cs_ptr, nbatch, dy_bs, x_bs, dw_bs, cs_batch, *geom, *am,
                                         ws.data_ptr(), nb, _hip.stream())


def wino_weights(weight, mode=0, scale=None):
    lib = _hip.load()
    w = _hip.f32c(weight.detach())
    _hip.need_gpu(w, scale)
    cout, cin, kh, kw = w.shape
    assert kh == 3 and kw == 3
    rows, k = (cout, cin) if mode == 0 else (cin, cout)
    U = torch.empty((36, rows, (k + 31) // 32 * 32), dtype=torch.float32, device=w.device)
    _hip.check(lib.rn_wino_weights(w.data_ptr(), U.data_ptr(), cout, cin, mode, _hip.ptr(scale), _hip.stream()),
               "rn_wino_weights")
    return _maybe_split(U, rows=rows, cin=U.shape[2], taps=1)


_WINO_WS = {}
_WINO_ODD_PLANES = os.environ.get("RN_WINO_ODD_PLANES", "1") != "0"


def wino_tpad(T):
    n = (T + 255) // 256
    if _WINO_ODD_PLANES and n % 2 == 0:
        n += 1
    return n * 256
# ... 13 lines not shown
            g.mask[i] = masks[i]._rn_sign.data_ptr() if mask_bits else masks[i].data_ptr()
        g.sign[i] = None if signs is None or signs[i] is None else signs[i].data_ptr()
        g.amax[i] = None if amaxs is None or amaxs[i] is None else amaxs[i].data_ptr()
    return g


def _wino_transform_in(xs, V, C, Tpad, dy_form, want_rows=False, want_tensor=False):
    lib = _hip.load()
    off = 0
    am = want_amax() and (want_rows or want_tensor)
    rows = torch.zeros(Tpad, dtype=torch.int32, device=V.device) if am and want_rows else None
    tword = amax_single(V.device) if am and want_tensor else None
    for k in range(0, len(xs), _hip.RN_MAX_GROUP):
        part = xs[k:k + _hip.RN_MAX_GROUP]
        t = sum(x.shape[0] * ((x.shape[1] + 3) // 4) * ((x.shape[2] + 3) // 4) for x in part)
        g = _wino_group(part, srcs=part, amaxs=[amax_words(x) for x in part] if am else None)
        nb = 4.0 * (sum(x.numel() for x in part) + 36 * t * C)
        _hip.check(prof.timed("wino_input", nb, lambda: lib.rn_wino_input_group(
            ctypes.byref(g), V.data_ptr(), C, off, Tpad, dy_form, _hip.ptr(rows), _hip.ptr(tword), _hip.stream())), "rn_wino_input_group")
        off += t
    return rows, tword


def _wino_workspace(device, floats_v, floats_m):
    key = (device, torch.cuda.current_stream(device).cuda_stream)
    ws = _WINO_WS.get(key)
    if ws is None or ws[0].numel() < floats_v or ws[1].numel() < floats_m:
        ws = (torch.empty(max(floats_v, ws[0].numel() if ws else 0), dtype=torch.float32, device=device),
              torch.empty(max(floats_m, ws[1].numel() if ws else 0), dtype=torch.float32, device=device))
        _WINO_WS[key] = ws
    return ws


def wino_conv_group(xs, U, outs=None, scale=None, shift=None, act=ACT_NONE, adds=None, masks=None, mask_mode=2,
                    flops=0.0, keep_v=False, y_batch_stride=0, V_in=None, V_ready=None, sign=False):
    lib = _hip.load()
    dev = xs[0].device
    C = xs[0].shape[3]
    cout = U.shape[1]
    tiles = [x.shape[0] * ((x.shape[1] + 3) // 4) * ((x.shape[2] + 3) // 4) for x in xs]
    T = sum(tiles)
    Tpad = wino_tpad(T)
    V, M = _wino_workspace(dev, 0 if keep_v else 36 * Tpad * C, 36 * Tpad * cout)
    shapes = tuple(tuple(x.shape) for x in xs)
    reuse = keep_v and V_in is not None and V_in[1] == shapes and V_in[0].numel() == 36 * Tpad * C
    ready = not keep_v and isinstance(V_ready, tuple) and V_ready[1] == shapes and V_ready[0].numel() >= 36 * Tpad * C
    if ready:
        V, reuse = V_ready[0], True
    elif reuse:
        V = V_in[0]
    elif keep_v:
        V = torch.empty(36 * Tpad * C, dtype=torch.float32, device=dev)
    assert all(x.is_contiguous() for x in xs)
    v_am = (None, None)
    if reuse:
        src = V_ready if ready else V_in
        v_am = src[2] if len(src) > 2 and src[2] is not None else (None, None)
    else:
        v_am = _wino_transform_in(xs, V, C, Tpad, 0, want_rows=True, want_tensor=keep_v)
    Vv = V[:36 * Tpad * C].view(36, 1, Tpad, C)
    Mv = M[:36 * Tpad * cout].view(36, 1, Tpad, cout)
    Uv = _carry_split(U, U.view(36 * cout, U.shape[2]))
    if want_amax() and v_am[0] is None:
        Uv = U.view(36 * cout, U.shape[2])
    conv_igemm(Vv, Uv, Mv, (1, Tpad, cout, 1, 1, 1, 1, 0, 0), flops=2.0 * 36 * T * cout * C, w_batch_stride=cout * U.shape[2],
               x_amax=v_am[0], x_amax_rows=True)
    if outs is None:
        outs = [torch.empty((x.shape[0], x.shape[1], x.shape[2], cout), dtype=torch.float32, device=dev) for x in xs]
    off = 0
    for k in range(0, len(xs), _hip.RN_MAX_GROUP):
        sl = slice(k, k + _hip.RN_MAX_GROUP)
        part, t = xs[sl], sum(tiles[sl])
        pa = None if adds is None else adds[sl]
        pm = None if masks is None else masks[sl]
        has_mask = pm is not None and pm[0] is not None
        mbits = has_mask and BITMASKS and all(getattr(m, "_rn_sign", None) is not None for m in pm)
        for o in outs[sl]:
            amax_drop(o)
        signs = [_sign_words(o, sign and not y_batch_stride) for o in outs[sl]]
        yams = [amax_slot(dev, o.shape[0]) for o in outs[sl]] if want_amax() and not y_batch_stride else None
        g = _wino_group(part, dsts=outs[sl], adds=pa, masks=pm, mask_bits=mbits, signs=signs, amaxs=yams)
        nops = 1 + (pa is not None and pa[0] is not None) + (1.0 / 32 if mbits else 1.0) * has_mask + (1.0 / 32 if signs[0] is not None else 0.0)
        nb = 4.0 * (36 * t * cout + nops * sum(x.shape[0] * x.shape[1] * x.shape[2] for x in part) * cout)
        mm = (mask_mode | (MASK_BITS if mbits else 0)) if has_mask else 0
        _hip.check(prof.timed("wino_output", nb, lambda: lib.rn_wino_output_group(
            ctypes.byref(g), M.data_ptr(), cout, off, Tpad, _hip.ptr(scale), _hip.ptr(shift), mm,
            act, y_batch_stride, _hip.stream())), "rn_wino_output_group")
        if yams is not None:
            for o, w_ in zip(outs[sl], yams):
                amax_attach(o, w_)
        off += t
    return (outs, (V, tuple(tuple(x.shape) for x in xs), v_am)) if keep_v else outs


_WINO_Z = {}
SIDE_HELD = {}


def side_release(side=None):
    if side is None:
        SIDE_HELD.clear()
    else:
        SIDE_HELD.pop(side.cuda_stream, None)


def _wino_z_buffer(device, floats):
    cur = torch.cuda.current_stream(device)
    st = _WINO_Z.setdefault((device, cur.cuda_stream), {"bufs": [None, None], "ev": [None, None], "i": 0})
    k = st["i"]
    st["i"] ^= 1
    if st["bufs"][k] is None or st["bufs"][k].numel() < floats:
        st["bufs"][k] = torch.empty(floats, dtype=torch.float32, device=device)
    if st["ev"][k] is not None:
        cur.wait_event(st["ev"][k])
    return st, k


def wino_wgrad_group(gs, xs, dw, colsum, flops=0.0, V=None, dU=None, fuse_dgrad_input=False, side=None):
    lib = _hip.load()
    dev = xs[0].device
    C, cout = xs[0].shape[3], gs[0].shape[3]
    zst = None
    tiles = [x.shape[0] * ((x.shape[1] + 3) // 4) * ((x.shape[2] + 3) // 4) for x in xs]
    T = sum(tiles)
    Tpad = wino_tpad(T)
    have_v = V is not None and V[1] == tuple(tuple(x.shape) for x in xs) and V[0].numel() == 36 * Tpad * C
    v_tw = V[2][1] if have_v and len(V) > 2 and V[2] is not None else None
    V = V[0] if have_v else None
    Vw, Z = _wino_workspace(dev, 0 if have_v else 36 * Tpad * C, 36 * Tpad * cout)
    if not have_v:
        V = Vw
    assert all(g.shape[:3] == x.shape[:3] and g.is_contiguous() and x.is_contiguous() for g, x in zip(gs, xs))
    if not have_v:
        v_tw = _wino_transform_in(xs, V, C, Tpad, 0, want_tensor=True)[1]
    v_dy, z_tw = None, None
    if fuse_dgrad_input and have_v and len(gs) <= _hip.RN_MAX_GROUP:
        Vd, Z = _wino_workspace(dev, 36 * Tpad * cout, 36 * Tpad * cout)
        if side is not None:
            zst, zk = _wino_z_buffer(dev, 36 * Tpad * cout)
            Z = zst["bufs"][zk]
        am_on = want_amax()
        g = _wino_group(gs, srcs=gs, amaxs=[amax_words(t) for t in gs] if am_on else None)
        vd_rows = torch.zeros(Tpad, dtype=torch.int32, device=dev) if am_on else None
        z_tw = amax_single(dev) if am_on else None
        nb = 4.0 * (sum(t.numel() for t in gs) + 2 * 36 * T * cout)
        _hip.check(prof.timed("wino_input", nb, lambda: lib.rn_wino_input_both_group(
            ctypes.byref(g), Vd.data_ptr(), Z.data_ptr(), cout, 0, Tpad, _hip.ptr(vd_rows), _hip.ptr(z_tw), _hip.stream())),
            "rn_wino_input_both_group")
        v_dy = (Vd, tuple(tuple(t.shape) for t in gs), (vd_rows, None))
    else:
        z_tw = _wino_transform_in(gs, Z, cout, Tpad, 1, want_tensor=True)[1]
    am = (z_tw, v_tw) if (want_amax() and z_tw is not None and v_tw is not None) else (None, None)
    ku = (C + 31) // 32 * 32
    if dU is None or tuple(dU.shape) != (36, cout, ku):
        dU = torch.zeros((36, cout, ku), dtype=torch.float32, device=dev)
    def reductions():
        rc = prof.timed("conv_wgrad" + (" winograd T%d %d->%d" % (T, C, cout) if prof.BY_SHAPE else ""), 2.0 * 36 * T * cout * C, lambda: _wgrad_call(
            lib, dev, Z.data_ptr(), cout, V.data_ptr(), dU.data_ptr(), _hip.ptr(colsum), 36, Tpad * cout, Tpad * C, cout * ku, 7,
            (1, 1, T, C, 1, T, cout, 1, 1, 1, 0, 0), amax=am))
        _hip.check(rc, "rn_conv_wgrad_batched")
        _hip.check(lib.rn_wino_dw(dU.data_ptr(), dw.data_ptr(), cout, C, _hip.stream()), "rn_wino_dw")
    if zst is None:
        reductions()
    else:
        side.wait_event(torch.cuda.current_stream(dev).record_event())
        with torch.cuda.stream(side):
            reductions()
            zst["ev"][zk] = side.record_event()
        SIDE_HELD.setdefault(side.cuda_stream, []).append((V, dU) + tuple(am))
    return v_dy


def conv_igemm_grouped(problems, w_packed, scale=None, shift=None, act=ACT_NONE, flops=0.0):
    lib = _hip.load()
    g = _hip.ConvGroup()
    g.n = len(problems)
    total = 0
    wptr, wfmt, wus = None, None, None
    yams = []
    for i, pr in enumerate(problems):
        x, geom = pr["x"], pr["geom"]
        add, mask = pr.get("add"), pr.get("mask")
        mask_ptr, mmode = _mask_operand(mask, pr.get("mask_mode", 2))
        d = _make_desc(x, geom, act, 1 if add is not None else 0, (0, 0), mmode, False, None, pr.get("y_batch_stride"), None, None)
        if wfmt is None:
            wptr, wfmt, wus = _w_operand(w_packed, d)
        d.w_format, d.w_unscale = wfmt, wus
        if wfmt == 3:
            d.x_amax, d.x_amax_img_stride, d.x_amax_row_stride = amax_words(x).data_ptr(), 1, 0
        amax_drop(pr["y"])
        bits = _sign_words(pr["y"], pr.get("sign", False) and pr.get("y_batch_stride") is None)
        d.sign_out = None if bits is None else bits.data_ptr()
        yam = amax_slot(x.device, x.shape[0]) if want_amax() and pr.get("y_batch_stride") is None else None
        yams.append(yam)
        d.y_amax = None if yam is None else yam.data_ptr()
        g.d[i] = d
        M = d.N * d.Ho * d.Wo
        total += (M + 255) // 256 if d.Cout <= 64 else ((M + 127) // 128) * ((d.Cout + 127) // 128)
        g.tile_end[i] = total
        g.x[i], g.y[i], g.add[i], g.mask[i] = x.data_ptr(), pr["y"].data_ptr(), _hip.ptr(add), mask_ptr
    kind = "conv_igemm_4x1" if problems[0]["geom"][2] <= 64 else "conv_igemm_2x2"
    if prof.BY_SHAPE:
# ... 151 lines not shown
    C = ld if C is None else C
    rows = g.numel() // ld
    ws = torch.empty(lib.rn_colsum_workspace_bytes(rows, C), dtype=torch.uint8, device=g.device)
    acc = out is not None
    if out is None:
        out = torch.empty(C, dtype=torch.float32, device=g.device)
    _hip.check(lib.rn_colsum(g.data_ptr(), rows, C, ld, out.data_ptr(), int(acc), ws.data_ptr(), _hip.stream()),
               "rn_colsum")
    return out


def upsample_add_bwd(src, dst):
    lib = _hip.load()
    N, Hs, Ws, C = src.shape
    assert src.dtype == dst.dtype
    amax_drop(dst)
    if src.dtype == torch.bfloat16:
        _hip.check(lib.rn_upsample_add_bwd_bf16(src.data_ptr(), dst.data_ptr(), N, Hs, Ws, dst.shape[1], dst.shape[2], C, _hip.stream()),
                   "rn_upsample_add_bwd_bf16")
        return dst
    am = amax_slot(dst.device, N) if want_amax() else None
    _hip.check(lib.rn_upsample_add_bwd(src.data_ptr(), dst.data_ptr(), N, Hs, Ws, dst.shape[1], dst.shape[2], C, _hip.ptr(am), _hip.stream()),
               "rn_upsample_add_bwd")
    if am is not None:
        amax_attach(dst, am)
    return dst


def relu_mask_(g, z):
    _hip.check(_hip.load().rn_relu_mask(g.data_ptr(), z.data_ptr(), g.numel(), _hip.stream()), "rn_relu_mask")
    return g


def sigmoid_bwd_pad(dy_ptr, s_ptr, B, rows_per_image, C, ld, src_batch_stride, device, bf16=False):
    lib = _hip.load()
    out = torch.empty((B * rows_per_image, ld), dtype=torch.bfloat16 if bf16 else torch.float32, device=device)
    if bf16:
        _hip.check(lib.rn_sigmoid_bwd_pad_bf16(dy_ptr, s_ptr, out.data_ptr(), B, rows_per_image, C, ld, src_batch_stride, _hip.stream()),
                   "rn_sigmoid_bwd_pad_bf16")
        return out
    am = amax_slot(device, B) if want_amax() else None
    _hip.check(lib.rn_sigmoid_bwd_pad(dy_ptr, s_ptr, out.data_ptr(), B, rows_per_image, C, ld, src_batch_stride, _hip.ptr(am), _hip.stream()),
               "rn_sigmoid_bwd_pad")
    if am is not None:
        out._rn_amax_words = am
    return out


def add_(dst, src):
    amax_drop(dst)
    am = amax_slot(dst.device, dst.shape[0]) if want_amax() and dst.dim() == 4 else None
    _hip.check(_hip.load().rn_add_inplace(dst.data_ptr(), src.data_ptr(), dst.numel(), dst.numel() // max(dst.shape[0], 1), _hip.ptr(am),
                                          _hip.stream()), "rn_add_inplace")
    if am is not None:
        amax_attach(dst, am)
    return dst


def to_bf16(t):
    t = _hip.f32c(t)
    _hip.need_gpu(t)
    out = torch.empty(t.shape, dtype=torch.bfloat16, device=t.device)
    if t.numel():
        _hip.check(_hip.load().rn_f32_to_bf16(t.data_ptr(), out.data_ptr(), t.numel(), _hip.stream()), "rn_f32_to_bf16")
    return out


def to_f32(t):
    _hip.need_gpu(t)
# ... 278 lines not shown
```

### 3d-playground_amd/retinanet_mi355x/engine.py

```python
import os

import torch

from . import _hip, arch, conv as cv, ops, prof


FUSE_DY = os.environ.get("RN_WINO_FUSE_DY", "1") != "0"
GROUPED_WGRAD_BF16 = os.environ.get("RN_GROUPED_WGRAD_BF16", "1") != "0"
S2_SHORTCUT_COMPACT = os.environ.get("RN_S2_SHORTCUT_COMPACT", "1") != "0"
STEM_BF16_PRODUCTS = os.environ.get("RN_STEM_BF16_PRODUCTS", "1") != "0"


def _qscale(t):
    return getattr(t, "_rn_scale", None) or getattr(t, "_rn_qscale", None)


def _as_fp8(t):
    if t is None or t.dtype == torch.uint8:
        return t
    q = getattr(t, "_rn_q8", None)
    if q is None:
        sc = _qscale(t)
        assert sc, "a tensor entering an fp8 layer needs its calibrated scale (Layer.fwd tags its outputs)"
        q = t._rn_q8 = cv.fp8_quantize(t, sc) if t.dtype == torch.float32 else cv.bf16_to_fp8(t, sc)
    return q


def _as_f32(t):
    if t is None or t.dtype == torch.float32:
        return t
    y = cv.fp8_dequantize(t) if t.dtype == torch.uint8 else cv.to_f32(t)
    y._rn_qscale = _qscale(t)
    return y


def _as_bf16(t):
    if t is None or t.dtype == torch.bfloat16:
        return t
    y = cv.fp8_to_bf16(t) if t.dtype == torch.uint8 else cv.to_bf16(t)
    y._rn_qscale = _qscale(t)
# ... 186 lines not shown
                N, Hi, Wi, _ = x.shape
                y = outs[i] if outs is not None else torch.empty((N, Hi, Wi, s.cout), dtype=torch.bfloat16, device=x.device)
                ys.append(y)
                fl += self.flops(N, Hi, Wi)
                probs.append({"x": x, "y": y, "geom": (Hi, Wi, s.cout, s.k, self.kw_pad, 1, 1, -s.pad, 0),
                              "y_batch_stride": y_batch_stride, "sign": self.sign and act == cv.ACT_RELU})
            cv.conv_igemm_bf16_grouped(probs, self.wf16, scale=self.scale, shift=self.shift, act=act, flops=fl)
            for y in ys:
                y._rn_qscale = self.out_scale
            return ys
        if (wino or self.wino_active) and self.wino_ok and (outs is None or y_batch_stride is not None):
            fl = sum(self.flops(x.shape[0], x.shape[1], x.shape[2]) for x in xs)
            r = cv.wino_conv_group(xs, self.wino_weights(0), outs=outs, scale=self.scale, shift=self.shift, act=act, flops=fl,
                                   keep_v=self.keep_v, y_batch_stride=y_batch_stride or 0, V_in=shared_v if self.keep_v else None,
                                   sign=self.sign and act == cv.ACT_RELU)
            ys, self.saved_v = r if self.keep_v else (r, None)
            return ys
        probs, ys, fl = [], [], 0.0
        for i, x in enumerate(xs):
            N, Hi, Wi, _ = x.shape
            Ho, Wo = cv.out_size(Hi, s.k, s.stride, s.pad), cv.out_size(Wi, s.k, s.stride, s.pad)
            y = outs[i] if outs is not None else torch.empty((N, Ho, Wo, s.cout), dtype=torch.float32, device=x.device)
            ys.append(y)
            fl += self.flops(N, Ho, Wo)
            probs.append({"x": x, "y": y, "geom": (Ho, Wo, s.cout, s.k, self.kw_pad, s.stride, 1, -s.pad, 0),
                          "y_batch_stride": y_batch_stride, "sign": self.sign and act == cv.ACT_RELU})
        cv.conv_igemm_grouped(probs, self.wf, scale=self.scale, shift=self.shift, act=act, flops=fl)
        if outs is None:
            for y in ys:
                self._tap(y)
                y._rn_qscale = self.out_scale
        return ys

    def bwd_data_group(self, gs, in_hws, adds=None, masks=None, wino=False):
        s = self.spec
        assert s.stride == 1
        if self.bf16:
            probs, outs, fl = [], [], 0.0
            for i, g in enumerate(gs):
                Hi, Wi = in_hws[i]
                dx = torch.empty((g.shape[0], Hi, Wi, s.cin), dtype=torch.bfloat16, device=g.device)
                outs.append(dx)
                fl += self.flops(g.shape[0], g.shape[1], g.shape[2])
                probs.append({"x": g, "y": dx, "geom": (Hi, Wi, s.cin, s.k, s.k, 1, -1, s.pad, 0),
                              "add": None if adds is None else adds[i], "mask": None if masks is None else masks[i]})
            cv.conv_igemm_bf16_grouped(probs, self.dgrad_weights16(), flops=fl)
            return outs
        if (wino or self.wino_active) and self.wino_ok and all(g.shape[3] == s.cout for g in gs):
            fl = sum(self.flops(g.shape[0], g.shape[1], g.shape[2]) for g in gs)
            ready, self.dy_v = getattr(self, "dy_v", None), None
            return cv.wino_conv_group(gs, self.wino_weights(1), adds=adds, masks=masks, mask_mode=2, flops=fl, V_ready=ready)
        probs, outs, fl = [], [], 0.0
        for i, g in enumerate(gs):
            N = g.shape[0]
            Hi, Wi = in_hws[i]
            dx = torch.empty((N, Hi, Wi, s.cin), dtype=torch.float32, device=g.device)
            outs.append(dx)
            fl += self.flops(N, g.shape[1], g.shape[2])
            probs.append({"x": g, "y": dx, "geom": (Hi, Wi, s.cin, s.k, s.k, 1, -1, s.pad, 0),
                          "add": None if adds is None else adds[i], "mask": None if masks is None else masks[i]})
        cv.conv_igemm_grouped(probs, self.dgrad_weights(), flops=fl)
        return outs

    def flops(self, N, Ho, Wo):
        s = self.spec
        return 2.0 * N * Ho * Wo * s.cout * s.cin * s.k * s.k

    def bwd_params(self, g, x, in_relu=False, side=None):
        s = self.spec
        if self.dw is None:
            self.dw = torch.zeros_like(self.wf)
            self.cs = torch.zeros(s.cout, dtype=torch.float32, device=g.device)
        if self.bf16:
            assert not in_relu
            cv.wgrad_bf16(g, x, self.dw, s.cout, s.k, s.stride, s.pad, flops=self.flops(g.shape[0], g.shape[1], g.shape[2]),
                          colsum=self.cs)
            return
        if self.wino_active and not in_relu and g.shape[3] == s.cout and g.is_contiguous() and x.is_contiguous():
            du, self.du = getattr(self, "du", None), None
            self.dy_v = cv.wino_wgrad_group([g], [x], self.dw, self.cs, V=self.saved_v, dU=du, fuse_dgrad_input=FUSE_DY, side=side)
            self.saved_v = None
            return
        cv.wgrad(g, x, self.dw, s.cout, s.k, s.stride, s.pad, kw_pad=self.kw_pad, in_relu=in_relu,
                 flops=self.flops(g.shape[0], g.shape[1], g.shape[2]), colsum=self.cs)

    def bwd_params_group(self, gs, xs, wino=False, side=None):
        s = self.spec
        if (wino or self.wino_active) and self.wino_ok and all(g.shape[3] == s.cout and g.is_contiguous() for g in gs):
            if self.dw is None:
                self.dw = torch.zeros_like(self.wf)
                self.cs = torch.zeros(s.cout, dtype=torch.float32, device=gs[0].device)
            fl = sum(self.flops(g.shape[0], g.shape[1], g.shape[2]) for g in gs)
            du, self.du = getattr(self, "du", None), None
            self.dy_v = cv.wino_wgrad_group(gs, xs, self.dw, self.cs, flops=fl, V=self.saved_v, dU=du, fuse_dgrad_input=FUSE_DY, side=side)
            self.saved_v = None
            return
        if self.bf16 and GROUPED_WGRAD_BF16 and 1 < len(gs) <= 5 and all(g.is_contiguous() and x.is_contiguous() for g, x in zip(gs, xs)) \
                and len({g.shape[3] for g in gs}) == 1:
            if self.dw is None:
                self.dw = torch.zeros_like(self.wf)
                self.cs = torch.zeros(s.cout, dtype=torch.float32, device=gs[0].device)
            fl = sum(self.flops(g.shape[0], g.shape[1], g.shape[2]) for g in gs)
            cv.wgrad_bf16_grouped(gs, xs, self.dw, s.cout, s.k, s.stride, s.pad, flops=fl, colsum=self.cs)
            return
        for g, x in zip(gs, xs):
            self.bwd_params(g, x)

    def bwd_data(self, g, in_hw, add=None, mask=None, mask_mode=2, add2=None):
        s = self.spec
        if self.bf16:
            assert add2 is None
            kw = dict(add=add, add_mode=1 if add is not None else 0, mask=mask, mask_mode=mask_mode,
                      flops=self.flops(g.shape[0], g.shape[1], g.shape[2]))
            if s.stride == 2 and s.k > 1:
                return cv.dgrad_s2_classes_bf16(g, self.dgrad_weights16(), in_hw, s.cin, s.k, s.pad, **kw)
            if s.stride == 2 and s.k == 1 and s.pad == 0 and mask is None and S2_SHORTCUT_COMPACT:
                Hi, Wi = in_hw
                N, Ho, Wo, _ = g.shape
                if add is None:
                    dx = torch.zeros((N, Hi, Wi, s.cin), dtype=torch.bfloat16, device=g.device)
                else:
                    assert add.shape == (N, Hi, Wi, s.cin) and add.dtype == torch.bfloat16 and add.is_contiguous()
                    dx = add
                return cv.conv_igemm_bf16(g, self.dgrad_weights16(), dx, (Ho, Wo, s.cin, 1, 1, 1, -1, 0, 0), out_map=(2, 0, 0, Hi, Wi),
                                          add=add, add_mode=1 if add is not None else 0, flops=kw["flops"])
            return cv.dgrad_any_bf16(g, self.dgrad_weights16(), in_hw, s.cin, s.k, s.stride, s.pad, **kw)
        if self.wino_active and add2 is None and g.shape[3] == s.cout and g.is_contiguous():
# ... 350 lines not shown
                continue
            arr = (_hip.PrepJob * len(jobs))(*jobs)
            jt = torch.frombuffer(bytearray(bytes(arr)), dtype=torch.uint8).to(dev)
            ct = torch.tensor(chunks, dtype=torch.int32).to(dev)
            out.append((jt, ct, len(chunks)))
        return {"key": key, "launches": out, "bufs": bufs}

    def _unpack_bucket(self, index, layers, views):
        key = tuple((L.dw.data_ptr(), L.wf.data_ptr(), views[L.grad_names()[0]].data_ptr(), _hip.ptr(L.scale) or 0, _hip.ptr(L.mean) or 0)
                    for L in layers)
        cache = self.__dict__.setdefault("_unpack_tables", {})
        hit = cache.get(index)
        if hit is None or hit[0] != key:
            jobs, chunks = [], []
            for L in layers:
                s, names = L.spec, L.grad_names()
                cout, cin, kh, kw = L.weight.shape
                j = _hip.UnpackJob()
                j.dw, j.w_packed, j.dweight = L.dw.data_ptr(), L.wf.data_ptr(), views[names[0]].data_ptr()
                j.Cout, j.Cin, j.kh, j.kw, j.kw_pad, j.c_pad, j.Kpad = cout, cin, kh, kw, L.kw_pad, L.cin_pad, L.wf.shape[1]
                j.scale, j.mean, j.rstd, j.colsum = _hip.ptr(L.scale), _hip.ptr(L.mean), _hip.ptr(L.rstd), L.cs.data_ptr()
                j.dgamma = views[names[1]].data_ptr() if s.bn else None
                j.dbeta = views[names[-1]].data_ptr() if len(names) > 1 else None
                chunks.extend((len(jobs), co) for co in range(cout))
                jobs.append(j)
            arr = (_hip.UnpackJob * len(jobs))(*jobs)
            dev = layers[0].dw.device
            hit = cache[index] = (key, torch.frombuffer(bytearray(bytes(arr)), dtype=torch.uint8).to(dev),
                                  torch.tensor(chunks, dtype=torch.int32).to(dev), len(chunks))
        _hip.check(_hip.load().rn_unpack_batched(hit[1].data_ptr(), hit[2].data_ptr(), hit[3], _hip.stream()), "rn_unpack_batched")
        for L in layers:
            L.dw = L.cs = L.wd = L.uf = L.ud = L.saved_v = L.dy_v = None

    def _zero_grad_accumulators(self, device):
        wino = self.use_wino and not self.bwd16
        sizes = []
        for L in self.layers.values():
            s = L.spec
            du = 36 * s.cout * ((s.cin + 31) // 32 * 32) if (wino and L.wino_layer) else 0
            sizes.append((L, L.wf.numel(), (s.cout + 3) // 4 * 4, du))
        total = sum(a + b + c for _, a, b, c in sizes)
        arena = getattr(self, "_arena", None)
        if arena is None or arena.numel() != total or arena.device != device:
            arena = self._arena = torch.empty(total, dtype=torch.float32, device=device)
        arena.zero_()
        o = 0
        for L, a, b, c in sizes:
            L.dw = arena[o:o + a].view_as(L.wf)
            L.cs = arena[o + a:o + a + L.spec.cout]
            L.du = arena[o + a + b:o + a + b + c].view(36, L.spec.cout, -1) if c else None
            o += a + b + c

    def calibrate(self, P, frames, margin=1.0):
        if self.fp8 or self.bf16:
            raise RuntimeError("calibrate with the fp32 engine (ResNet.calibrate_fp8 switches to it): the magnitudes are recorded "
                               "by the fp32 direct kernels' path only")
        rec = {}
        wino_eval, self.wino_eval = self.wino_eval, False
        for L in self.layers.values():
            L.calib = rec
        self.calib = rec
        try:
            with torch.no_grad():
                self.forward(P, frames, save=False)
        finally:
            for L in self.layers.values():
                L.calib = None
            self.calib = None
            self.wino_eval = wino_eval
        missing = [n for n in self.fp8_scale_names() if n not in rec]
        assert not missing, "calibration pass did not record %s" % missing
        return {k: v * margin for k, v in rec.items()}

    def fp8_scale_names(self):
        return ["pool"] + [n for n in self.layers if n != "conv1" and not n.endswith(".output")]

    def set_fp8_layers(self, fp8=None, other="fp32"):
        assert self.fp8 and other in ("fp32", "bf16")
        pick = (lambda n: True) if fp8 is None else (fp8 if callable(fp8) else (lambda n, names=set(fp8): n in names))
        self._fp8_explicit = True
        on = []
        for n, L in self.layers.items():
            if n == "conv1":
                continue
# ... 109 lines not shown
                side[ti].wait_event(fork)
                if ti == 1 and v_ready is not None:
                    side[ti].wait_event(v_ready)
            with torch.cuda.stream(side[ti] if side is not None else main):
                ts = pyramid
                acts = []
                for i in range(1, 5):
                    first = Ls["regressionModel.conv1"]
                    shared = first.saved_v if (i == 1 and prefix == "classificationModel") else None
                    ts = Ls["%s.conv%d" % (prefix, i)].fwd_group(ts, act=cv.ACT_RELU, wino=save and self.use_wino and not self.bf16 and not self.fp8,
                                                                 shared_v=shared)
                    acts.append(ts)
                    if side is not None and ti == 0 and i == 1:
                        v_ready = side[0].record_event()
                views, off = [], 0
                for cnt in counts:
                    views.append(out.view(B, -1)[:, off * width:])
                    off += cnt
                Ls[prefix + ".output"].fwd_group(ts, act=act, outs=views, y_batch_stride=A * width)
            if save:
                S["towers"][prefix] = [[acts[i][li] for i in range(4)] for li in range(5)]
        if side is not None:
            main.wait_stream(side[0])
            main.wait_stream(side[1])
        if save:
            S["wino_v"] = {n: L.saved_v for n, L in Ls.items() if L.saved_v is not None}
        for L in Ls.values():
            L.saved_v = None
        return reg, cls, S

    def backward(self, S, dreg, dcls, cls):
        Ls = self.layers
        grads = {}
        self._zero_grad_accumulators(dreg.device)
        for L in Ls.values():
            L.saved_v = L.dy_v = None
        for n, v in S.pop("wino_v", {}).items():
            Ls[n].saved_v = v

        flat = views = None
        next_bucket = 0
        if self.flat_bucket_bytes:
            flat, views = self._flat_views(dreg.device)
            buckets = self._flat["buckets"]

        batched = flat is not None and self.grad_hook is None and os.environ.get("RN_BATCHED_UNPACK", "1") != "0"
        pending = []

        main0 = torch.cuda.current_stream(dreg.device) if dreg.is_cuda else None
        wss = self.wgrad_streams(dreg.device) if batched else None
        wg_count = 0
        held = []

        def join():
            for ws in wss or ():
                main0.wait_stream(ws)
                cv.side_release(ws)
            held.clear()

        def aside(fn, tensors):
            nonlocal wg_count
            ws = wss[wg_count % len(wss)]
            wg_count += 1
            if cv.want_amax():
                for t in tensors:
                    if t.dtype == torch.float32 and t.is_contiguous():
                        cv.amax_words(t)
            ws.wait_event(torch.cuda.current_stream(dreg.device).record_event())
            with torch.cuda.stream(ws):
                fn()
            held.append(tuple(tensors) + tuple(getattr(t, "_rn_amax", (None,))[0] for t in tensors))

        def wg(L, g, x, in_relu=False):
            if wss is None:
                L.bwd_params(g, x, in_relu=in_relu)
            elif L.wino_active and not L.bf16:
                L.bwd_params(g, x, in_relu=in_relu, side=wss[0] if os.environ.get("RN_WGRAD_WINO", "1") != "0" else None)
            else:
                aside(lambda: L.bwd_params(g, x, in_relu=in_relu), (g, x))

        def wg_group(L, gs, xs, wino=False):
            if wss is None or os.environ.get("RN_WGRAD_TOWERS", "0") == "0":
                L.bwd_params_group(gs, xs, wino=wino)
            elif wino or L.wino_active:
                L.bwd_params_group(gs, xs, wino=wino, side=wss[0])
            else:
                aside(lambda: L.bwd_params_group(gs, xs), tuple(gs) + tuple(xs))

        def done(layer):
            nonlocal next_bucket
            if batched:
                pending.append(layer)
                grads.update({n: views[n] for n in layer.grad_names()})
            else:
                g = layer.finish(views)
                grads.update(g)
                if self.grad_hook is not None:
                    self.grad_hook(g)
            if flat is not None and layer.spec.name == buckets[next_bucket][2]:
                if batched:
                    join()
                    self._unpack_bucket(next_bucket, pending, views)
                    pending.clear()
                if self.bucket_hook is not None:
                    self.bucket_hook(next_bucket, flat[buckets[next_bucket][0]:buckets[next_bucket][1]])
                next_bucket += 1

        ACT = _as_bf16 if self.fp8 else (lambda t: t)
        pyramid, counts = [ACT(t) for t in S["pyramid"]], S["counts"]
        B = dreg.shape[0]
        A = dreg.shape[1]
        dpyr = [None] * 5
        hws = [(f.shape[1], f.shape[2]) for f in pyramid]
        side = self.tower_streams(dreg.device)
        main = torch.cuda.current_stream(dreg.device)
        if side is not None:
            fork = main.record_event()
        retired = []
        for ti, (prefix, dout, width, sig) in enumerate((("regressionModel", dreg, self.n_reg, None),
                                                         ("classificationModel", dcls, self.num_classes, cls))):
            Lout = Ls[prefix + ".output"]
            tower = [Ls["%s.conv%d" % (prefix, i)] for i in range(1, 5)]
            if side is not None:
                side[ti].wait_event(fork)
            with torch.cuda.stream(side[ti] if side is not None else main):
                acts = [[ACT(t) for t in lvl] for lvl in S["towers"][prefix]]
                gs, off = [], 0
                for (Hh, Ww), cnt in zip(hws, counts):
                    byte_off = 4 * off * width
                    g = cv.sigmoid_bwd_pad(dout.data_ptr() + byte_off, None if sig is None else sig.data_ptr() + byte_off,
                                           B, Hh * Ww, arch.NUM_ANCHORS * width, Lout.cout_pad, A * width, dout.device,
                                           bf16=self.bwd16)
                    gs.append(cv.amax_carry(g.view(B, Hh, Ww, Lout.cout_pad), g))
                    off += cnt
                wg_group(Lout, gs, [acts[li][3] for li in range(5)])
                gs = Lout.bwd_data_group(gs, hws, masks=[acts[li][3] for li in range(5)])
                for i in (3, 2, 1):
                    wg_group(tower[i], gs, [acts[li][i - 1] for li in range(5)], wino=self.use_wino and not self.bwd16)
                    gs = tower[i].bwd_data_group(gs, hws, masks=[acts[li][i - 1] for li in range(5)], wino=self.use_wino and not self.bwd16)
                wg_group(tower[0], gs, pyramid, wino=self.use_wino and not self.bwd16)
                first = dpyr[0] is None
                if side is not None and not first:
                    side[ti].wait_stream(side[0])
                dpyr = tower[0].bwd_data_group(gs, hws, adds=None if first else dpyr, wino=self.use_wino and not self.bwd16)
            S["towers"][prefix] = None
            retired.append(Lout)
            retired.extend(reversed(tower))
        if side is not None:
            main.wait_stream(side[0])
            main.wait_stream(side[1])
        for L in retired:
            done(L)
        c3, c4, c5, p5lat, p4sum, p3sum, p6 = (ACT(t) for t in S["fpn"])
        dp3, dp4, dp5, dp6, dp7 = dpyr
        hw = lambda t: (t.shape[1], t.shape[2])
        L = Ls["fpn.P7_2"]
        if self.bwd16:
            wg(L, dp7, ACT(S["p6r"]))
        else:
            wg(L, dp7, p6, in_relu=True)
        dp6 = L.bwd_data(dp7, hw(p6), add=dp6, mask=p6, mask_mode=1)
        done(L)
        L = Ls["fpn.P6"]
        wg(L, dp6, c5)
        dc5 = L.bwd_data(dp6, hw(c5))
        done(L)
        L = Ls["fpn.P3_2"]
        wg(L, dp3, p3sum)
        dp3sum = L.bwd_data(dp3, hw(p3sum))
        done(L)
        L = Ls["fpn.P3_1"]
        wg(L, dp3sum, c3)
        dc3 = L.bwd_data(dp3sum, hw(c3))
# ... 64 lines not shown
```

### include/retinanet_mi355x.h

```cpp
#ifndef RETINANET_MI355X_H
#define RETINANET_MI355X_H

#include <stdint.h>

#ifdef __cplusplus
extern "C" {
#endif

#define RN_OK 0
#define RN_EINVAL 10001
#define RN_ETOOMANY 10002
#define RN_MAX_GT 256
#define RN_LEVELS 5

const char *rn_version(void);
int rn_check_device(void);

int64_t rn_anchor_count(int height, int width);
void rn_anchor_base_boxes(double out[RN_LEVELS * 9 * 4]);
int rn_anchors_fwd(float *out, int height, int width, void *stream);

int rn_pairwise_iou(const float *a, const float *b, float *iou, int64_t A, int N, void *stream);

int64_t rn_focal_workspace_bytes(int B, int64_t A);
// ... 154 lines not shown
    int32_t win[4];
    float factors[3];
    int32_t occluded;
    int32_t occlude[4];
} rn_augment_crop_params;
int64_t rn_augment_crops_workspace_bytes(int B, int win_max, int crop);
int rn_augment_crops(const uint8_t *frames, int B, int H, int W, const rn_augment_crop_params *params, const int32_t *table_x,
                     const int32_t *table_y, const int32_t *table_cx, const int32_t *table_cy, int K, int win_max, int crop,
                     const uint8_t *noise, const float *occlusion, uint64_t seed, float mean0, float mean1, float mean2,
                     float std0, float std1, float std2, void *workspace, float *out, void *stream);

typedef struct rn_conv_desc {
    int N, Hi, Wi, Cin;
    int Ho, Wo, Cout;
    int kh, kw;
    int a, b, p, p_w, div_shift;
    int act;
    int add_mode;
    int Ha, Wa;
    int mask_mode;
    int in_relu;
    int os, oo_h, oo_w, Hy, Wy;
    int add2_mode;
    int Ha2, Wa2;
    int64_t add2_batch_stride;
    int64_t x_batch_stride, y_batch_stride, add_batch_stride;
    int64_t w_batch_stride;
    int w_format;
    void *sign_out;
    const void *x_amax;
    void *y_amax;
    const float *w_unscale;
    int x_amax_img_stride, x_amax_row_stride;
} rn_conv_desc;
#define RN_MASK_BITS 4

#define RN_FP32_NATIVE 0
#define RN_FP32_SPLIT 1
#define RN_FP32_SPLIT3 2
#define RN_FP32_DEFAULT RN_FP32_SPLIT3
int rn_get_fp32_mfma(void);
int rn_set_fp32_mfma(int mode);
#define RN_OPT_SPLITK 0
#define RN_OPT_DETERMINISTIC 1
#define RN_OPT_MF16 2
#define RN_OPT_MF16_MIN 3
#define RN_OPT_WGRAD_ONCE 4
#define RN_OPT_BF16_P8 5
#define RN_OPT_FP8_P8 6
#define RN_OPT_COUNT 7
int rn_get_option(int option);
int rn_set_option(int option, int value);
int rn_fp32_split_min_k(void);
int rn_split_weights(const float *w_packed, void *w_split, int64_t rows, int Kpad, void *stream);
int rn_split_weights_f16(const float *w_packed, void *w_split, float *row_unscale, int64_t rows, int Kpad, void *stream);
int rn_amax(const float *x, int64_t per_image, int n_images, void *amax, void *stream);
int rn_stream_capture_id(void *stream, unsigned long long *id);
int rn_conv_igemm_wants_f16(const rn_conv_desc *d);

int rn_conv_igemm(const rn_conv_desc *d, const float *x, const float *w_packed, float *y,
                  const float *scale, const float *shift, const float *add, const float *mask, const float *add2,
                  void *stream);

int64_t rn_conv_splitk_workspace_bytes(const rn_conv_desc *d);
int rn_conv_igemm_splitk(const rn_conv_desc *d, const float *x, const float *w_packed, float *y, const float *scale,
                         const float *shift, const float *add, const float *mask, const float *add2, void *workspace,
                         void *stream);

#define RN_MAX_GROUP 5
typedef struct rn_conv_group {
    int n;
    int tile_end[RN_MAX_GROUP];
    rn_conv_desc d[RN_MAX_GROUP];
    const float *x[RN_MAX_GROUP];
    float *y[RN_MAX_GROUP];
    const float *add[RN_MAX_GROUP];
    const float *mask[RN_MAX_GROUP];
} rn_conv_group;
int rn_conv_igemm_grouped(const rn_conv_group *g, const float *w_packed, const float *scale, const float *shift,
                          void *stream);

int rn_conv_wgrad(const float *dy, int ldy, const float *x, float *dw, float *colsum, int N, int Hi, int Wi,
                  int Cin, int Ho, int Wo, int Cout, int kh, int kw, int stride, int pad, int in_relu, void *stream);
int rn_conv_wgrad_batched(const float *dy, int ldy, const float *x, float *dw, float *colsum, int nbatch,
                          int64_t dy_bstride, int64_t x_bstride, int64_t dw_bstride, int colsum_batch, int N, int Hi, int Wi,
                          int Cin, int Ho, int Wo, int Cout, int kh, int kw, int stride, int pad, int in_relu,
                          const void *dy_amax, int dy_amax_n, const void *x_amax, int x_amax_n, void *stream);
int64_t rn_conv_wgrad_det_workspace_bytes(int ldy, int nbatch, int64_t dw_bstride, int N, int Hi, int Wi, int Cin, int Ho, int Wo,
                                          int Cout, int kh, int kw);
int rn_conv_wgrad_batched_det(const float *dy, int ldy, const float *x, float *dw, float *colsum, int nbatch,
                              int64_t dy_bstride, int64_t x_bstride, int64_t dw_bstride, int colsum_batch, int N, int Hi, int Wi,
                              int Cin, int Ho, int Wo, int Cout, int kh, int kw, int stride, int pad, int in_relu,
                              const void *dy_amax, int dy_amax_n, const void *x_amax, int x_amax_n, void *workspace, int64_t workspace_bytes,
                              void *stream);

int rn_f32_to_bf16(const float *src, void *dst, int64_t n, void *stream);
int rn_bf16_to_f32(const void *src, float *dst, int64_t n, void *stream);
int rn_conv_igemm_bf16(const rn_conv_desc *d, const void *x, const void *w_packed, void *y, int y_is_f32,
                       const float *scale, const float *shift, const void *add, const void *mask, void *stream);
int rn_conv_igemm_bf16_grouped(const rn_conv_group *g, const void *w_packed, int y_is_f32, const float *scale,
                               const float *shift, void *stream);
int rn_conv_igemm_bf16_tile_rows(const rn_conv_group *g, int y_is_f32);
int rn_fp8_quantize(const float *src, void *dst, int64_t n, float inv_scale, void *stream);
int rn_maxpool_fwd_fp8out(const float *x, void *y, int N, int H, int W, int C, int Ho, int Wo, float inv_scale, void *stream);
int rn_fp8_dequantize(const void *src, float *dst, int64_t n, float scale, void *stream);
int rn_fp8_to_bf16(const void *src, void *dst, int64_t n, float scale, void *stream);
int rn_bf16_to_fp8(const void *src, void *dst, int64_t n, float inv_scale, void *stream);
int rn_fp8_quantize_rows(const float *w_packed, void *w_q, float *row_scale, int64_t rows, int Kpad, void *stream);
int rn_conv_igemm_fp8(const rn_conv_desc *d, const void *x_q, const void *w_q, void *y, int y_is_f32, const float *scale,
                      const float *shift, const void *add_q, float add_scale, float out_inv_scale, void *stream);
int rn_conv_igemm_fp8_tile_rows(const rn_conv_group *g, int y_is_f32);
int rn_conv_igemm_fp8_tile(const rn_conv_desc *d, int y_is_f32);
int rn_conv_igemm_bf16_tile(const rn_conv_desc *d, int y_is_f32);
int rn_conv_igemm_fp8_grouped(const rn_conv_group *g, const void *w_q, int y_is_f32, const float *scale, const float *shift,
                              float add_scale, float out_inv_scale, void *stream);

int rn_conv_wgrad_bf16(const void *dy, int ldy, const void *x, float *dw, float *colsum, int N, int Hi, int Wi, int Cin,
                       int Ho, int Wo, int Cout, int kh, int kw, int stride, int pad, void *stream);
int rn_conv_wgrad_bf16_grouped(int n, const void *const *dy, int ldy, const void *const *x, float *dw, float *colsum, int N,
                               const int *Hi, const int *Wi, int Cin, int Cout, int kh, int kw, int stride, int pad, void *stream);

int rn_maxpool_fwd_bf16out(const float *x, void *y, uint8_t *argmax, int N, int H, int W, int C, int Ho, int Wo, void *stream);
int rn_maxpool_bwd_bf16in(const float *x, const void *dy, const uint8_t *argmax, float *dx, int N, int H, int W, int C, int Ho,
                          int Wo, int relu_mask, void *stream);
int rn_upsample_add_bwd_bf16(const void *src, void *dst, int N, int Hs, int Ws, int Hd, int Wd, int C, void *stream);
int rn_sigmoid_bwd_pad_bf16(const float *dy, const float *s, void *out, int B, int64_t rows_per_image, int C, int ld,
                            int64_t src_batch_stride, void *stream);
int rn_relu_bf16(const void *src, void *dst, int64_t n, void *stream);

typedef struct rn_wino_group {
    int n;
    int N[RN_MAX_GROUP], H[RN_MAX_GROUP], W[RN_MAX_GROUP];
    const float *src[RN_MAX_GROUP];
    float *dst[RN_MAX_GROUP];
    const float *add[RN_MAX_GROUP];
    const float *mask[RN_MAX_GROUP];
    void *sign[RN_MAX_GROUP];
    void *amax[RN_MAX_GROUP];
} rn_wino_group;
int rn_wino_input_group(const rn_wino_group *g, float *V, int C, int64_t tile_offset, int64_t Tpad, int dy_form,
                        void *row_amax, void *tensor_amax, void *stream);
int rn_wino_input_both_group(const rn_wino_group *g, float *V, float *Z, int C, int64_t tile_offset, int64_t Tpad,
                             void *v_row_amax, void *z_tensor_amax, void *stream);
int rn_wino_output_group(const rn_wino_group *g, const float *M, int Cout, int64_t tile_offset, int64_t Tpad,
                         const float *scale, const float *shift, int mask_mode, int act, int64_t y_batch_stride, void *stream);
int rn_wino_input(const float *x, float *V, int N, int H, int W, int C, int64_t tile_offset, int64_t Tpad, void *stream);
int rn_wino_output(const float *M, float *y, int N, int H, int W, int Cout, int64_t tile_offset, int64_t Tpad,
                   const float *scale, const float *shift, const float *add, const float *mask, int mask_mode, int act,
                   int64_t y_batch_stride, void *stream);
int rn_wino_weights(const float *w, float *U, int Cout, int Cin, int mode, const float *scale, void *stream);
int rn_wino_dy(const float *dy, float *Z, int N, int H, int W, int C, int64_t tile_offset, int64_t Tpad, void *stream);
int rn_wino_dw(const float *dU, float *dw, int Cout, int Cin, void *stream);

typedef struct rn_prep_job {
    int kind;
    int Cout, Cin, kh, kw, kw_pad, c_pad, mode, r0, nr, s0, ns, rows, Kpad;
    float eps;
    const float *src;
    float *dst;
    const float *scale;
    const float *gamma, *beta, *mean, *var;
    float *bn_scale, *bn_shift, *bn_rstd;
} rn_prep_job;
int rn_prep_batched(const rn_prep_job *jobs_dev, const int32_t *chunks_dev, int nchunks, void *stream);

int rn_pack_weights(const float *src, float *dst, int Cout, int Cin, int kh, int kw, int kw_pad, int c_pad,
                    int mode, const float *scale, int r0, int nr, int s0, int ns, void *stream);
int rn_unpack_wgrad(const float *dw, const float *w_packed, float *dweight, int Cout, int Cin, int kh, int kw,
                    int kw_pad, int c_pad, const float *scale, const float *mean, const float *rstd,
                    const float *colsum, float *dgamma, float *dbeta, void *stream);

typedef struct rn_unpack_job {
    const float *dw, *w_packed;
    float *dweight;
    int Cout, Cin, kh, kw, kw_pad, c_pad, Kpad;
    const float *scale, *mean, *rstd, *colsum;
    float *dgamma, *dbeta;
} rn_unpack_job;
int rn_unpack_batched(const rn_unpack_job *jobs_dev, const int32_t *chunks_dev, int nchunks, void *stream);

int rn_bn_fold(const float *gamma, const float *beta, const float *mean, const float *var, float eps, int C,
               float *scale, float *shift, float *rstd, void *stream);

int rn_nchw_to_nhwc4(const float *src, float *dst, int N, int H, int W, void *amax, void *stream);
int rn_maxpool_fwd(const float *x, float *y, uint8_t *argmax, int N, int H, int W, int C, int Ho, int Wo, void *stream);
int rn_maxpool_bwd(const float *x, const float *dy, const uint8_t *argmax, float *dx, int N, int H, int W, int C,
                   int Ho, int Wo, int relu_mask, void *amax, void *stream);
int rn_colsum(const float *g, int64_t rows, int C, int ld, float *out, int accumulate, void *workspace, void *stream);
int64_t rn_colsum_workspace_bytes(int64_t rows, int C);
int rn_upsample_add_bwd(const float *src, float *dst, int N, int Hs, int Ws, int Hd, int Wd, int C, void *amax, void *stream);
int rn_relu_mask(float *g, const float *z, int64_t n, void *stream);
int rn_sigmoid_bwd_pad(const float *dy, const float *s, float *out, int B, int64_t rows_per_image, int C, int ld,
                       int64_t src_batch_stride, void *amax, void *stream);
int rn_add_inplace(float *dst, const float *src, int64_t n, int64_t per_image, void *amax, void *stream);

int64_t rn_opt_workspace_bytes(int n_chunks);
int rn_opt_clip_adam(const void *tensor_table, const void *chunk_table, int n_chunks, float max_norm, float lr,
                     float beta1, float beta2, float eps, int step, int write_clipped, void *workspace,
                     float *total_norm, void *stream);
int rn_opt_clip_adam_dev(const void *tensor_table, const void *chunk_table, int n_chunks, float max_norm, float lr,
                         float beta1, float beta2, float eps, int *step_dev, int write_clipped, void *workspace,
                         float *total_norm, void *stream);
int rn_opt_clip_adam_hp(const void *tensor_table, const void *chunk_table, int n_chunks, const float *hp, int *step_dev,
                        int write_clipped, void *workspace, float *total_norm, void *stream);

#define RN_MOT_MAX 512
#define RN_MOT_MAX_IDS 16384
#define RN_MOT_RESULT 152
#define RN_MOT_OK 0
#define RN_MOT_INVALID 1
#define RN_MOT_INFEASIBLE 2
#define RN_MOT_TOO_LARGE 3
int rn_mot_prepare(const double *gt_im, const float *gt_h0, const float *gt_vel, int64_t G, const float *pred_state,
                   int64_t M, const double *H, const double *P, float *gt_state, float *gt_box, float *pred_box,
                   double *pred_im, void *stream);
int rn_mot_iou(const float *gt_box, const float *pred_box, const int32_t *gt_off, const int32_t *pr_off,
               const int64_t *iou_off, int64_t F, int64_t max_cells, double *iou, void *stream);
int rn_mot_assign(const double *iou, const int32_t *gt_off, const int32_t *pr_off, const int64_t *iou_off,
                  const int32_t *slot_off, int64_t F, int64_t max_n, int64_t S, int64_t M, int32_t *slot_row,
                  int32_t *slot_col, uint8_t *pred_assigned, int32_t *frame_status, void *stream);
int rn_mot_frame_metrics(const double *iou, const int32_t *gt_off, const int32_t *pr_off, const int64_t *iou_off,
                         const int32_t *slot_off, int64_t F, int64_t S, const int32_t *slot_row, const int32_t *slot_col,
                         const int32_t *frame_status, double match_iou, const float *gt_state, const float *pred_state,
                         const double *gt_im, const double *pred_im, const int32_t *gt_cls, const int32_t *pred_cls,
                         const int32_t *gt_id, const int32_t *pred_id, const uint8_t *pred_assigned, double *slot_iou,
                         int32_t *slot_gid, int32_t *slot_pid, float *slot_state_err, double *slot_bot, double *slot_top,
// ... 103 lines not shown
```

Measured before the change: 127.1 images/sec.

## Propagate sparse regression-gradient tile flags to skip zero work in backward towers

Regression-head gradients are nonzero only near GT boxes, so activity flags per Winograd tile are now computed in sigmoid backward and carried through each tower layer's data-gradient pass. Each layer dilates the flags by one tile. Winograd input/output transforms, the RAW mf16 conv kernel and the wgrad once-kernel use them to skip zero tiles or K-steps; the wgrad kernel compacts the active steps into a list. This adds flag arrays in the accumulator arena and extra launch constraints such as alignment and a cap on the step count. It also depends on the inputs being sparse, so dense gradients would gain little.

```diff
diff --git a/3d-playground_amd/csrc/conv_igemm_mf16.hip b/3d-playground_amd/csrc/conv_igemm_mf16.hip
--- a/3d-playground_amd/csrc/conv_igemm_mf16.hip
+++ b/3d-playground_amd/csrc/conv_igemm_mf16.hip
@@ -367,7 +367,20 @@
                                                               const float *__restrict__ scale, const float *__restrict__ shift,
                                                               const float *__restrict__ add, const float *__restrict__ mask,
                                                               const float *__restrict__ add2) {
-    conv_mf16_tile<GENERAL, RAW, TERMS, STG, WV>(d, x, w, y, scale, shift, add, mask, add2, xcd_remap(blockIdx.x, gridDim.x));
+    const int tile = xcd_remap(blockIdx.x, gridDim.x);
+    if constexpr (RAW) {
+        if (d.row_active != nullptr && d.w_batch_stride != 0) {
+            constexpr int BM = 32 * WV;
+            const int m0 = (tile / ((d.Cout + 127) / 128)) * BM;
+            int nz = 0;
+            if (threadIdx.x < BM / 16) {
+                const uint4 u = reinterpret_cast<const uint4 *>(reinterpret_cast<const unsigned char *>(d.row_active) + m0 % (d.Ho * d.Wo))[threadIdx.x];
+                nz = (u.x | u.y | u.z | u.w) != 0u;
+            }
+            if (!__syncthreads_or(nz)) return;
+        }
+    }
+    conv_mf16_tile<GENERAL, RAW, TERMS, STG, WV>(d, x, w, y, scale, shift, add, mask, add2, tile);
 }
 
 template <int TERMS>
@@ -407,6 +420,8 @@
     if (!mf16_ok(d) || (variant != 0 && variant != 4 && variant != 5)) return false;
     const int64_t tiles = mf16_tiles(d);
     if (tiles < mf16_min_tiles() || tiles > 0x7fffffff) return false;
+    if (variant == 0 && d->row_active != nullptr && d->w_batch_stride != 0 &&
+        (((uintptr_t)d->row_active & 15) || ((int64_t)d->Ho * d->Wo) % 256 != 0)) { *rc = RN_EINVAL; return true; }
     const dim3 grid((unsigned)tiles), block(256);
 #define RN_MF16_LAUNCH(G, R, T, S) hipLaunchKernelGGL((conv_igemm_mf16_kernel<G, R, T, S>), grid, block, 0, s, *d, x, w, y, scale, shift, add, mask, add2)
     if (d->w_format == 3) {
diff --git a/3d-playground_amd/csrc/conv_wgrad.hip b/3d-playground_amd/csrc/conv_wgrad.hip
--- a/3d-playground_amd/csrc/conv_wgrad.hip
+++ b/3d-playground_amd/csrc/conv_wgrad.hip
@@ -36,6 +36,7 @@
     int64_t slab_stride;
     const void *dy_amax, *x_amax;
     int dy_amax_n, x_amax_n;
+    const unsigned char *k_active;
 };
 
 __device__ __forceinline__ void wgrad_scales(const void *amax, int count, float &scale, float &unscale) {
@@ -285,7 +286,8 @@
     return __builtin_bit_cast(bf16x8, v);
 }
 
-template <bool RELU, bool HALF = false>
+#define RN_WG_SKIP_MAX 2040
+template <bool RELU, bool HALF = false, bool SKIP = false>
 __global__ __launch_bounds__(256, 3) void conv_wgrad_once_kernel(const WgradArgs p) {
     using G = WgradSplitGeom;
     constexpr int BM = 128, BN = 128, WK = G::WK, TB = G::TB;
@@ -351,9 +353,52 @@
         }
         pixtab[j & 1][tid] = e;
     };
+    unsigned short *klist = reinterpret_cast<unsigned short *>(&pixtab[0][0]);
+    int *wcnt = reinterpret_cast<int *>(klist + RN_WG_SKIP_MAX);
+    int nact = nks;
+    if constexpr (SKIP) {
+        static_assert(RN_WG_SKIP_MAX * 2 + 16 <= (int)sizeof(pixtab), "the list fits the pixel table");
+        nact = 0;
+        for (int k0 = 0; k0 < nks; k0 += 256) {
+            const int ks = k0 + tid;
+            bool on = false;
+            if (ks < nks) {
+                const uint4 u = *reinterpret_cast<const uint4 *>(p.k_active + kbeg + (int64_t)ks * WK);
+                on = (u.x | u.y | u.z | u.w) != 0u;
+            }
+            const unsigned long long b = __ballot(on);
+            if (lane == 0) wcnt[wave] = __popcll(b);
+            __syncthreads();
+            int before = nact, all = 0;
+#pragma unroll
+            for (int w_ = 0; w_ < 4; ++w_) { const int c_ = wcnt[w_]; all += c_; before += w_ < wave ? c_ : 0; }
+            if (on) klist[before + __popcll(b & ((1ull << lane) - 1ull))] = (unsigned short)ks;
+            nact += all;
+            __syncthreads();
+        }
+        if (nact == 0 && p.slab == nullptr) return;
+    }
     typedef float f32x4v __attribute__((ext_vector_type(4)));
     struct Regs { f32x4v a[2], b[2]; };
     auto load_step = [&](int ks, Regs &r) {
+        if constexpr (SKIP) {
+            if (ks >= nact) {
+                r.a[0] = r.a[1] = r.b[0] = r.b[1] = f32x4v{0.f, 0.f, 0.f, 0.f};
+                return;
+            }
+            const int kq = klist[ks];
+            const unsigned so = (unsigned)kq * (unsigned)(WK * 4) * (unsigned)p.ldy;
+            r.a[0] = __builtin_bit_cast(f32x4v, __builtin_amdgcn_raw_buffer_load_b128(rs_a, (int)a_voff, (int)so, 0));
+            r.a[1] = __builtin_bit_cast(f32x4v, __builtin_amdgcn_raw_buffer_load_b128(rs_a, (int)a_voff, (int)(so + a_half), 0));
+#pragma unroll
+            for (int h = 0; h < 2; ++h) {
+                const int64_t px = kbeg + (int64_t)kq * WK + G::pixel(tid, h);
+                const bool ok = px < kend && jcol < p.Kflat;
+                const unsigned v = ok ? (unsigned)((int)px * p.Cin * 4 + tap_off) : 0x80000000u;
+                r.b[h] = __builtin_bit_cast(f32x4v, __builtin_amdgcn_raw_buffer_load_b128(rs_b, (int)v, 0, 0));
+            }
+            return;
+        }
         const int2 *tab = pixtab[(ks / TB) & 1];
         const unsigned so = (unsigned)ks * (unsigned)(WK * 4) * (unsigned)p.ldy;
         r.a[0] = __builtin_bit_cast(f32x4v, __builtin_amdgcn_raw_buffer_load_b128(rs_a, (int)a_voff, (int)so, 0));
@@ -432,8 +477,10 @@
 #pragma unroll
             for (int e_ = 0; e_ < 16; ++e_) acc[i][j][e_] = 0.f;
 
-    fill_batch(0);
-    __syncthreads();
+    if constexpr (!SKIP) {
+        fill_batch(0);
+        __syncthreads();
+    }
     Regs r0, r1;
     load_step(0, r0);
     split_store(0, r0);
@@ -474,12 +521,14 @@
 #pragma unroll
             for (int tn = 0; tn < 2; ++tn) RN_SPLIT_MFMA(acc[tm][tn], sa[tm], sb[tn]);
         }
-        if ((ks % TB) == 4 && (ks / TB + 1) * TB < nks + 2) fill_batch(ks / TB + 1);
+        if constexpr (!SKIP) {
+            if ((ks % TB) == 4 && (ks / TB + 1) * TB < nks + 2) fill_batch(ks / TB + 1);
+        }
         __syncthreads();
     };
-    for (int ks = 0; ks < nks; ks += 2) {
+    for (int ks = 0; ks < nact; ks += 2) {
         k_step(ks, 0, r0, r1);
-        if (ks + 1 < nks) k_step(ks + 1, 1, r1, r0);
+        if (ks + 1 < nact) k_step(ks + 1, 1, r1, r0);
     }
     if (do_cs) {
         float (*csred)[BM] = reinterpret_cast<float (*)[BM]>(&lds[0][0]);
@@ -540,7 +589,8 @@
                         int64_t dy_bstride, int64_t x_bstride, int64_t dw_bstride, int colsum_batch, int N, int Hi,
                         int Wi, int Cin, int Ho, int Wo, int Cout, int kh, int kw, int stride, int pad,
                         int in_relu, void *stream, bool det, void *workspace, int64_t workspace_bytes, int64_t *need_bytes,
-                        const void *dy_amax = nullptr, int dy_amax_n = 0, const void *x_amax = nullptr, int x_amax_n = 0);
+                        const void *dy_amax = nullptr, int dy_amax_n = 0, const void *x_amax = nullptr, int x_amax_n = 0,
+                        const void *k_active = nullptr);
 
 extern "C" int rn_conv_wgrad_batched(const float *dy, int ldy, const float *x, float *dw, float *colsum, int nbatch,
                                      int64_t dy_bstride, int64_t x_bstride, int64_t dw_bstride, int colsum_batch, int N, int Hi,
@@ -560,6 +610,18 @@
                         kh, kw, stride, pad, in_relu, stream, true, workspace, workspace_bytes, nullptr, dy_amax, dy_amax_n, x_amax, x_amax_n);
 }
 
+extern "C" int rn_conv_wgrad_batched_flags(const float *dy, int ldy, const float *x, float *dw, float *colsum, int nbatch,
+                                           int64_t dy_bstride, int64_t x_bstride, int64_t dw_bstride, int colsum_batch, int N, int Hi,
+                                           int Wi, int Cin, int Ho, int Wo, int Cout, int kh, int kw, int stride, int pad,
+                                           int in_relu, const void *dy_amax, int dy_amax_n, const void *x_amax, int x_amax_n,
+                                           const void *k_active, void *workspace, int64_t workspace_bytes, void *stream) {
+    if (k_active == nullptr || ((uintptr_t)k_active & 15)) return RN_EINVAL;
+    if (N != 1 || Hi != 1 || Ho != 1 || Wi != Wo || kh != 1 || kw != 1 || stride != 1 || pad != 0 || in_relu) return RN_EINVAL;
+    return wgrad_launch(dy, ldy, x, dw, colsum, nbatch, dy_bstride, x_bstride, dw_bstride, colsum_batch, N, Hi, Wi, Cin, Ho, Wo, Cout,
+                        kh, kw, stride, pad, in_relu, stream, workspace != nullptr, workspace, workspace_bytes, nullptr, dy_amax, dy_amax_n,
+                        x_amax, x_amax_n, k_active);
+}
+
 extern "C" int64_t rn_conv_wgrad_det_workspace_bytes(int ldy, int nbatch, int64_t dw_bstride, int N, int Hi, int Wi, int Cin, int Ho,
                                                      int Wo, int Cout, int kh, int kw) {
     int64_t need = 0;
@@ -572,7 +634,7 @@
                         int64_t dy_bstride, int64_t x_bstride, int64_t dw_bstride, int colsum_batch, int N, int Hi,
                         int Wi, int Cin, int Ho, int Wo, int Cout, int kh, int kw, int stride, int pad,
                         int in_relu, void *stream, bool det, void *workspace, int64_t workspace_bytes, int64_t *need_bytes,
-                        const void *dy_amax, int dy_amax_n, const void *x_amax, int x_amax_n) {
+                        const void *dy_amax, int dy_amax_n, const void *x_amax, int x_amax_n, const void *k_active) {
     if (N <= 0 || Hi <= 0 || Wi <= 0 || Ho <= 0 || Wo <= 0 || Cout <= 0 || Cin < 4 || (Cin & 3) || (ldy & 3) || ldy < Cout)
         return RN_EINVAL;
     if (nbatch < 1 || nbatch > 4096 || dy_bstride < 0 || x_bstride < 0 || dw_bstride < 0 || colsum_batch < 0 || colsum_batch >= nbatch)
@@ -630,6 +692,7 @@
     a.x_amax = x_amax;
     a.dy_amax_n = dy_amax_n;
     a.x_amax_n = x_amax_n;
+    a.k_active = reinterpret_cast<const unsigned char *>(k_active);
 #define RN_WGRAD_LAUNCH(WM_, WN_)                                                                                        \
     do {                                                                                                                 \
         if (half) {                                                                                                      \
@@ -642,7 +705,11 @@
         else hipLaunchKernelGGL((conv_wgrad_kernel<WM_, WN_, false, 16, 3>), grid, dim3(256), 0, (hipStream_t)stream, a);         \
     } while (0)
     const bool once = split && shape == 2 && rn_get_option(RN_OPT_WGRAD_ONCE) != 0 && Hi + pad < 32000 && Wi + pad < 32000;
-    if (once && half) {
+    if (k_active != nullptr) {
+        if (!once || in_relu || (a.per_split + 15) / 16 > RN_WG_SKIP_MAX) return RN_EINVAL;
+        if (half) hipLaunchKernelGGL((conv_wgrad_once_kernel<false, true, true>), grid, dim3(256), 0, (hipStream_t)stream, a);
+        else hipLaunchKernelGGL((conv_wgrad_once_kernel<false, false, true>), grid, dim3(256), 0, (hipStream_t)stream, a);
+    } else if (once && half) {
         if (in_relu) hipLaunchKernelGGL((conv_wgrad_once_kernel<true, true>), grid, dim3(256), 0, (hipStream_t)stream, a);
         else hipLaunchKernelGGL((conv_wgrad_once_kernel<false, true>), grid, dim3(256), 0, (hipStream_t)stream, a);
     } else if (once) {
diff --git a/3d-playground_amd/csrc/conv_wino.hip b/3d-playground_amd/csrc/conv_wino.hip
--- a/3d-playground_amd/csrc/conv_wino.hip
+++ b/3d-playground_amd/csrc/conv_wino.hip
@@ -122,10 +122,12 @@
     }
 }
 
-template <bool PBITS, bool PADD>
+template <bool PBITS, bool PADD, bool FLAGS = false>
 __global__ __launch_bounds__(256, 2) void wino_out_kernel(const WinoTable g, const float *__restrict__ M, int Cout, int64_t t0,
                                                        int64_t Tpad, const float *__restrict__ scale,
-                                                       const float *__restrict__ shift, int mask_mode, int act, int64_t y_bs) {
+                                                       const float *__restrict__ shift, int mask_mode, int act, int64_t y_bs,
+                                                       const unsigned char *__restrict__ fin = nullptr,
+                                                       unsigned char *__restrict__ fout = nullptr) {
     const int cq = Cout >> 2;
     const int64_t id = (int64_t)blockIdx.x * 256 + threadIdx.x;
     const int64_t gt = id / cq;
@@ -153,15 +155,25 @@
     const int th = r / TW, tw = r - th * TW;
     const float *mb = M + (t0 + gt) * Cout + c4;
     float4 t[4][6];
-#pragma unroll
-    for (int j = 0; j < 6; ++j) {
-        float4 m[6], o[4];
-#pragma unroll
-        for (int i = 0; i < 6; ++i) m[i] = ld_stream(mb + (int64_t)(i * 6 + j) * Tpad * Cout);
-        at6(m, o);
-#pragma unroll
-        for (int i = 0; i < 4; ++i) t[i][j] = o[i];
-    }
+    bool active = true;
+    if constexpr (FLAGS) active = fin == nullptr || fin[t0 + gt] != 0;
+    if (active) {
+#pragma unroll
+        for (int j = 0; j < 6; ++j) {
+            float4 m[6], o[4];
+#pragma unroll
+            for (int i = 0; i < 6; ++i) m[i] = ld_stream(mb + (int64_t)(i * 6 + j) * Tpad * Cout);
+            at6(m, o);
+#pragma unroll
+            for (int i = 0; i < 4; ++i) t[i][j] = o[i];
+        }
+    } else {
+#pragma unroll
+        for (int j = 0; j < 6; ++j)
+#pragma unroll
+            for (int i = 0; i < 4; ++i) t[i][j] = f4(0.f);
+    }
+    unsigned wake = 0u;
     float4 sc = f4(1.f), sh = f4(0.f);
     if (scale) sc = *reinterpret_cast<const float4 *>(scale + c4);
     if (shift) sh = *reinterpret_cast<const float4 *>(shift + c4);
@@ -210,6 +222,27 @@
             *reinterpret_cast<float4 *>(y + yoff) = make_float4(v[0], v[1], v[2], v[3]);
             if (sign != nullptr) rn_sign_store(sign, off, v[0], v[1], v[2], v[3]);
             am = fmaxf(fmaxf(am, fmaxf(fabsf(v[0]), fabsf(v[1]))), fmaxf(fabsf(v[2]), fabsf(v[3])));
+            if constexpr (FLAGS) {
+                if (v[0] != 0.f || v[1] != 0.f || v[2] != 0.f || v[3] != 0.f) {
+                    const unsigned rows = 2u | (i == 0 ? 1u : 0u) | (i == 3 ? 4u : 0u);
+                    const unsigned cols = 2u | (j == 0 ? 1u : 0u) | (j == 3 ? 4u : 0u);
+#pragma unroll
+                    for (int a = 0; a < 3; ++a)
+                        if (rows & (1u << a)) wake |= cols << (3 * a);
+                }
+            }
+        }
+    }
+    if constexpr (FLAGS) {
+        if (fout != nullptr && wake != 0u) {
+#pragma unroll
+            for (int a = 0; a < 3; ++a)
+#pragma unroll
+                for (int b = 0; b < 3; ++b) {
+                    const int th2 = th + a - 1, tw2 = tw + b - 1;
+                    if ((wake & (1u << (3 * a + b))) && (unsigned)th2 < (unsigned)pr.TH && (unsigned)tw2 < (unsigned)TW)
+                        fout[t0 + gt + (int64_t)(a - 1) * TW + (b - 1)] = 1;
+                }
         }
     }
     } while (0);
@@ -308,9 +341,11 @@
     }
 }
 
+template <bool FLAGS = false>
 __global__ __launch_bounds__(256) void wino_in_both_kernel(const WinoTable g, float *__restrict__ V, float *__restrict__ Z, int C,
                                                            int64_t t0, int64_t Tpad, unsigned *__restrict__ v_row_amax,
-                                                           unsigned *__restrict__ z_tensor_amax) {
+                                                           unsigned *__restrict__ z_tensor_amax,
+                                                           const unsigned char *__restrict__ flags = nullptr) {
     wino_tensor_word(g, z_tensor_amax, WINO_GAIN_A);
     const int cq = C >> 2;
     const int64_t id = (int64_t)xcd_remap(blockIdx.x, gridDim.x) * 256 + threadIdx.x;
@@ -333,6 +368,18 @@
         if (gt_raw < t_last && c4 == 0) v_row_amax[t0 + gt] = rn_amax_word_of_exp(e_img, WINO_GAIN_BT);
     }
     if (gt_raw >= t_last) return;
+    if constexpr (FLAGS) {
+        const int64_t row = t0 + gt;
+        if (flags[row] == 0) {
+            const uint4 u = *reinterpret_cast<const uint4 *>(flags + (row & ~(int64_t)15));
+            if ((u.x | u.y | u.z | u.w) != 0u) {
+                float *zb0 = Z + row * C + c4;
+#pragma unroll
+                for (int p = 0; p < 36; ++p) st_stream(zb0 + (int64_t)p * Tpad * C, f4(0.f));
+            }
+            return;
+        }
+    }
     float4 t[6][6];
     float4 tz[6][4];
 #pragma unroll
@@ -435,23 +482,35 @@
     return RN_OK;
 }
 
-extern "C" int rn_wino_input_both_group(const rn_wino_group *g, float *V, float *Z, int C, int64_t tile_offset, int64_t Tpad,
-                                        void *v_row_amax, void *z_tensor_amax, void *stream) {
+extern "C" int rn_wino_input_both_group_flags(const rn_wino_group *g, float *V, float *Z, int C, int64_t tile_offset, int64_t Tpad,
+                                              void *v_row_amax, void *z_tensor_amax, const void *flags, void *stream) {
     WinoTable t;
     const int rc = wino_table(g, t);
     if (rc) return rc;
     if (!V || !Z || C <= 0 || (C & 3) || tile_offset < 0 || tile_offset + t.tile_end[t.n - 1] > Tpad) return RN_EINVAL;
+    if (flags != nullptr && (((uintptr_t)flags & 15) || (Tpad & 15))) return RN_EINVAL;
     for (int i = 0; i < t.n; ++i)
         if (!t.src[i]) return RN_EINVAL;
-    hipLaunchKernelGGL(wino_in_both_kernel, dim3(rn_blocks(t.tile_end[t.n - 1] * (C >> 2), 256)), dim3(256), 0, (hipStream_t)stream, t,
-                       V, Z, C, tile_offset, Tpad, reinterpret_cast<unsigned *>(v_row_amax), reinterpret_cast<unsigned *>(z_tensor_amax));
+    const dim3 grid(rn_blocks(t.tile_end[t.n - 1] * (C >> 2), 256));
+    if (flags != nullptr)
+        hipLaunchKernelGGL(wino_in_both_kernel<true>, grid, dim3(256), 0, (hipStream_t)stream, t, V, Z, C, tile_offset, Tpad,
+                           reinterpret_cast<unsigned *>(v_row_amax), reinterpret_cast<unsigned *>(z_tensor_amax),
+                           reinterpret_cast<const unsigned char *>(flags));
+    else
+        hipLaunchKernelGGL(wino_in_both_kernel<false>, grid, dim3(256), 0, (hipStream_t)stream, t, V, Z, C, tile_offset, Tpad,
+                           reinterpret_cast<unsigned *>(v_row_amax), reinterpret_cast<unsigned *>(z_tensor_amax),
+                           (const unsigned char *)nullptr);
     RN_LAUNCH_CHECK();
     return RN_OK;
 }
-
-extern "C" int rn_wino_output_group(const rn_wino_group *g, const float *M, int Cout, int64_t tile_offset, int64_t Tpad,
-                                    const float *scale, const float *shift, int mask_mode, int act, int64_t y_batch_stride,
-                                    void *stream) {
+extern "C" int rn_wino_input_both_group(const rn_wino_group *g, float *V, float *Z, int C, int64_t tile_offset, int64_t Tpad,
+                                        void *v_row_amax, void *z_tensor_amax, void *stream) {
+    return rn_wino_input_both_group_flags(g, V, Z, C, tile_offset, Tpad, v_row_amax, z_tensor_amax, nullptr, stream);
+}
+
+extern "C" int rn_wino_output_group_flags(const rn_wino_group *g, const float *M, int Cout, int64_t tile_offset, int64_t Tpad,
+                                          const float *scale, const float *shift, int mask_mode, int act, int64_t y_batch_stride,
+                                          const void *flags_in, void *flags_out, void *stream) {
     WinoTable t;
     const int rc = wino_table(g, t);
     if (rc) return rc;
@@ -467,15 +526,27 @@
     bool padd = true;
     for (int i = 0; i < t.n; ++i) padd = padd && t.add[i] != nullptr;
     const dim3 grid(rn_blocks(t.tile_end[t.n - 1] * (Cout >> 2), 256));
-#define RN_WINO_OUT(B, A) hipLaunchKernelGGL((wino_out_kernel<B, A>), grid, dim3(256), 0, (hipStream_t)stream, t, M, Cout, tile_offset, Tpad, \
-                                             scale, shift, mask_mode, act, y_batch_stride)
-    if (pbits && padd) RN_WINO_OUT(true, true);
-    else if (pbits) RN_WINO_OUT(true, false);
-    else if (padd) RN_WINO_OUT(false, true);
-    else RN_WINO_OUT(false, false);
+    const unsigned char *fin = reinterpret_cast<const unsigned char *>(flags_in);
+    unsigned char *fout = reinterpret_cast<unsigned char *>(flags_out);
+#define RN_WINO_OUT(B, A, F) hipLaunchKernelGGL((wino_out_kernel<B, A, F>), grid, dim3(256), 0, (hipStream_t)stream, t, M, Cout, tile_offset, Tpad, \
+                                                scale, shift, mask_mode, act, y_batch_stride, fin, fout)
+    if (fin != nullptr || fout != nullptr) {
+        if (pbits && padd) RN_WINO_OUT(true, true, true);
+        else if (pbits) RN_WINO_OUT(true, false, true);
+        else if (padd) RN_WINO_OUT(false, true, true);
+        else RN_WINO_OUT(false, false, true);
+    } else if (pbits && padd) RN_WINO_OUT(true, true, false);
+    else if (pbits) RN_WINO_OUT(true, false, false);
+    else if (padd) RN_WINO_OUT(false, true, false);
+    else RN_WINO_OUT(false, false, false);
 #undef RN_WINO_OUT
     RN_LAUNCH_CHECK();
     return RN_OK;
+}
+extern "C" int rn_wino_output_group(const rn_wino_group *g, const float *M, int Cout, int64_t tile_offset, int64_t Tpad,
+                                    const float *scale, const float *shift, int mask_mode, int act, int64_t y_batch_stride,
+                                    void *stream) {
+    return rn_wino_output_group_flags(g, M, Cout, tile_offset, Tpad, scale, shift, mask_mode, act, y_batch_stride, nullptr, nullptr, stream);
 }
 
 static rn_wino_group wino_single(const float *src, float *dst, const float *add, const float *mask, int N, int H, int W) {
diff --git a/3d-playground_amd/csrc/elementwise.hip b/3d-playground_amd/csrc/elementwise.hip
--- a/3d-playground_amd/csrc/elementwise.hip
+++ b/3d-playground_amd/csrc/elementwise.hip
@@ -455,6 +455,49 @@
     return RN_OK;
 }
 
+__global__ void sigmoid_bwd_pad_flags_kernel(const float *__restrict__ dy, const float *__restrict__ s, float *__restrict__ out,
+                                             int64_t rows, int H, int W, int C, int ld, int64_t bstride, unsigned *__restrict__ amax,
+                                             unsigned char *__restrict__ flags) {
+    const int64_t i = (int64_t)blockIdx.x * 256 + threadIdx.x;
+    if (i >= rows * ld) return;
+    const int64_t rpi = (int64_t)H * W;
+    const int64_t r = i / ld;
+    const int c = (int)(i - r * ld);
+    const int64_t b = r / rpi;
+    const int pix = (int)(r - b * rpi);
+    float v = 0.f;
+    if (c < C) {
+        const int64_t src = b * bstride + (int64_t)pix * C + c;
+        v = dy[src];
+        if (s) { const float p = s[src]; v *= p * (1.0f - p); }
+    }
+    out[i] = v;
+    rn_amax_note(amax, b, fabsf(v));
+    if (v != 0.f) {
+        const int h = pix / W, w = pix - h * W;
+        const int TH = (H + 3) >> 2, TW = (W + 3) >> 2;
+        const int th = h >> 2, tw = w >> 2, hi = h & 3, wi = w & 3;
+        unsigned char *f = flags + (b * TH + th) * TW + tw;
+#pragma unroll
+        for (int a = -1; a <= 1; ++a)
+#pragma unroll
+            for (int e = -1; e <= 1; ++e) {
+                const bool rows_ok = a == 0 || (a < 0 ? hi == 0 && th > 0 : hi == 3 && th + 1 < TH);
+                const bool cols_ok = e == 0 || (e < 0 ? wi == 0 && tw > 0 : wi == 3 && tw + 1 < TW);
+                if (rows_ok && cols_ok) f[a * TW + e] = 1;
+            }
+    }
+}
+extern "C" int rn_sigmoid_bwd_pad_flags(const float *dy, const float *s, float *out, int B, int H, int W, int C, int ld,
+                                        int64_t src_batch_stride, void *amax, void *flags, void *stream) {
+    const int64_t rows = (int64_t)B * H * W;
+    if (B <= 0 || H <= 0 || W <= 0 || C <= 0 || ld < C || flags == nullptr || (int64_t)H * W > 0x7fffffff) return RN_EINVAL;
+    hipLaunchKernelGGL(sigmoid_bwd_pad_flags_kernel, dim3(rn_blocks(rows * ld, 256)), dim3(256), 0, (hipStream_t)stream, dy, s, out,
+                       rows, H, W, C, ld, src_batch_stride, reinterpret_cast<unsigned *>(amax), reinterpret_cast<unsigned char *>(flags));
+    RN_LAUNCH_CHECK();
+    return RN_OK;
+}
+
 __global__ void add_inplace_kernel(float *__restrict__ dst, const float *__restrict__ src, int64_t n, int64_t per_image, unsigned *__restrict__ amax) {
     const int64_t i = (int64_t)blockIdx.x * 256 + threadIdx.x;
     if (i >= n) return;
diff --git a/3d-playground_amd/retinanet_mi355x/_hip.py b/3d-playground_amd/retinanet_mi355x/_hip.py
--- a/3d-playground_amd/retinanet_mi355x/_hip.py
+++ b/3d-playground_amd/retinanet_mi355x/_hip.py
@@ -114,7 +114,8 @@
                 ("add2_mode", c_i32), ("Ha2", c_i32), ("Wa2", c_i32), ("add2_batch_stride", c_i64),
                 ("x_batch_stride", c_i64), ("y_batch_stride", c_i64), ("add_batch_stride", c_i64),
                 ("w_batch_stride", c_i64), ("w_format", c_i32), ("sign_out", c_vp),
-                ("x_amax", c_vp), ("y_amax", c_vp), ("w_unscale", c_vp), ("x_amax_img_stride", c_i32), ("x_amax_row_stride", c_i32)]
+                ("x_amax", c_vp), ("y_amax", c_vp), ("w_unscale", c_vp), ("x_amax_img_stride", c_i32), ("x_amax_row_stride", c_i32),
+                ("row_active", c_vp)]
 
 
 RN_MAX_GROUP = 5
@@ -150,6 +151,8 @@
     "rn_prep_batched": (c_i32, [c_vp, c_vp, c_i32, c_vp]),
     "rn_wino_input_group": (c_i32, [ctypes.POINTER(WinoGroup), c_vp, c_i32, c_i64, c_i64, c_i32, c_vp, c_vp, c_vp]),
     "rn_wino_input_both_group": (c_i32, [ctypes.POINTER(WinoGroup), c_vp, c_vp, c_i32, c_i64, c_i64, c_vp, c_vp, c_vp]),
+    "rn_wino_input_both_group_flags": (c_i32, [ctypes.POINTER(WinoGroup), c_vp, c_vp, c_i32, c_i64, c_i64, c_vp, c_vp, c_vp, c_vp]),
+    "rn_wino_output_group_flags": (c_i32, [ctypes.POINTER(WinoGroup), c_vp, c_i32, c_i64, c_i64, c_vp, c_vp, c_i32, c_i32, c_i64, c_vp, c_vp, c_vp]),
     "rn_wino_output_group": (c_i32, [ctypes.POINTER(WinoGroup), c_vp, c_i32, c_i64, c_i64, c_vp, c_vp, c_i32, c_i32, c_i64, c_vp]),
     "rn_conv_igemm_grouped": (c_i32, [ctypes.POINTER(ConvGroup), c_vp, c_vp, c_vp, c_vp]),
     "rn_conv_igemm": (c_i32, [ctypes.POINTER(ConvDesc), c_vp, c_vp, c_vp, c_vp, c_vp, c_vp, c_vp, c_vp, c_vp]),
@@ -168,6 +171,7 @@
     "rn_upsample_add_bwd": (c_i32, [c_vp, c_vp] + [c_i32] * 6 + [c_vp, c_vp]),
     "rn_relu_mask": (c_i32, [c_vp, c_vp, c_i64, c_vp]),
     "rn_sigmoid_bwd_pad": (c_i32, [c_vp, c_vp, c_vp, c_i32, c_i64, c_i32, c_i32, c_i64, c_vp, c_vp]),
+    "rn_sigmoid_bwd_pad_flags": (c_i32, [c_vp, c_vp, c_vp, c_i32, c_i32, c_i32, c_i32, c_i32, c_i64, c_vp, c_vp, c_vp]),
     "rn_add_inplace": (c_i32, [c_vp, c_vp, c_i64, c_i64, c_vp, c_vp]),
     "rn_wino_input": (c_i32, [c_vp, c_vp, c_i32, c_i32, c_i32, c_i32, c_i64, c_i64, c_vp]),
     "rn_wino_output": (c_i32, [c_vp, c_vp, c_i32, c_i32, c_i32, c_i32, c_i64, c_i64, c_vp, c_vp, c_vp, c_vp, c_i32, c_i32, c_i64, c_vp]),
@@ -176,6 +180,7 @@
     "rn_wino_dw": (c_i32, [c_vp, c_vp, c_i32, c_i32, c_vp]),
     "rn_conv_wgrad_batched": (c_i32, [c_vp, c_i32, c_vp, c_vp, c_vp, c_i32, c_i64, c_i64, c_i64, c_i32] + [c_i32] * 12 + [c_vp, c_i32, c_vp, c_i32, c_vp]),
     "rn_conv_wgrad_batched_det": (c_i32, [c_vp, c_i32, c_vp, c_vp, c_vp, c_i32, c_i64, c_i64, c_i64, c_i32] + [c_i32] * 12 + [c_vp, c_i32, c_vp, c_i32, c_vp, c_i64, c_vp]),
+    "rn_conv_wgrad_batched_flags": (c_i32, [c_vp, c_i32, c_vp, c_vp, c_vp, c_i32, c_i64, c_i64, c_i64, c_i32] + [c_i32] * 12 + [c_vp, c_i32, c_vp, c_i32, c_vp, c_vp, c_i64, c_vp]),
     "rn_conv_wgrad_det_workspace_bytes": (c_i64, [c_i32, c_i32, c_i64] + [c_i32] * 9),
     "rn_f32_to_bf16": (c_i32, [c_vp, c_vp, c_i64, c_vp]),
     "rn_bf16_to_f32": (c_i32, [c_vp, c_vp, c_i64, c_vp]),
diff --git a/3d-playground_amd/retinanet_mi355x/conv.py b/3d-playground_amd/retinanet_mi355x/conv.py
--- a/3d-playground_amd/retinanet_mi355x/conv.py
+++ b/3d-playground_amd/retinanet_mi355x/conv.py
@@ -65,7 +65,7 @@
 def conv_igemm(x, w_packed, y, geom, scale=None, shift=None, add=None, add_mode=0, add_hw=(0, 0), mask=None,
                mask_mode=2, act=ACT_NONE, y_batch_stride=None, add_batch_stride=None, in_relu=False, flops=0.0,
                out_map=None, add2=None, w_batch_stride=0, kind=None, sign=False, bf16_products=False, x_amax=None, x_amax_rows=False,
-               amax=None):
+               amax=None, row_active=None):
     lib = _hip.load()
     N, Hi, Wi, Cin = x.shape
     Ho, Wo, Cout, kh, kw, a, b, p, ds = geom
@@ -80,6 +80,8 @@
                  mask_mode, int(in_relu), os_, oo_h, oo_w, Hy, Wy,
                  a2[0], a2[1], a2[2], a2[3], Hi * Wi * Cin, ybs, add_batch_stride, w_batch_stride)
     amax_drop(y)
+    if row_active is not None:
+        d.row_active = row_active.data_ptr()
     bits = _sign_words(y, sign and y_batch_stride is None and out_map is None)
     d.sign_out = None if bits is None else bits.data_ptr()
     yam = None
@@ -296,9 +298,19 @@
     set_option(OPT_DETERMINISTIC, on)
 
 
-def _wgrad_call(lib, dev, dy_ptr, ldy, x_ptr, dw_ptr, cs_ptr, nbatch, dy_bs, x_bs, dw_bs, cs_batch, geom, amax=(None, None)):
+def _wgrad_call(lib, dev, dy_ptr, ldy, x_ptr, dw_ptr, cs_ptr, nbatch, dy_bs, x_bs, dw_bs, cs_batch, geom, amax=(None, None), flags=None):
     cnt = lambda a: 0 if a is None else (-1 if a.numel() == 1 else a.numel() // AMAX_SUB)
     am = (_hip.ptr(amax[0]), cnt(amax[0]), _hip.ptr(amax[1]), cnt(amax[1]))
+    if flags is not None:
+        ws, nb = None, 0
+        if lib.rn_get_option(OPT_DETERMINISTIC):
+            N, Hi, Wi, Cin, Ho, Wo, Cout, kh, kw = geom[:9]
+            nb = lib.rn_conv_wgrad_det_workspace_bytes(ldy, nbatch, dw_bs, N, Hi, Wi, Cin, Ho, Wo, Cout, kh, kw)
+            if nb < 0:
+                return 1
+            ws = torch.empty(nb, dtype=torch.uint8, device=dev)
+        return lib.rn_conv_wgrad_batched_flags(dy_ptr, ldy, x_ptr, dw_ptr, cs_ptr, nbatch, dy_bs, x_bs, dw_bs, cs_batch, *geom, *am,
+                                               flags.data_ptr(), _hip.ptr(ws), nb, _hip.stream())
     if not lib.rn_get_option(OPT_DETERMINISTIC):
         return lib.rn_conv_wgrad_batched(dy_ptr, ldy, x_ptr, dw_ptr, cs_ptr, nbatch, dy_bs, x_bs, dw_bs, cs_batch, *geom, *am, _hip.stream())
     N, Hi, Wi, Cin, Ho, Wo, Cout, kh, kw = geom[:9]
@@ -378,8 +390,17 @@
     return ws
 
 
+def tile_flags(device, T):
+    return torch.zeros(wino_tpad(T), dtype=torch.uint8, device=device)
+
+
+def wino_flags_ok(T, C, cout):
+    lib = _hip.load()
+    return bool(get_fp32_mfma() != "native" and lib.rn_get_option(OPT_WGRAD_ONCE) and C > 64 and cout > 64 and T < 32000)
+
+
 def wino_conv_group(xs, U, outs=None, scale=None, shift=None, act=ACT_NONE, adds=None, masks=None, mask_mode=2,
-                    flops=0.0, keep_v=False, y_batch_stride=0, V_in=None, V_ready=None, sign=False):
+                    flops=0.0, keep_v=False, y_batch_stride=0, V_in=None, V_ready=None, sign=False, flags_out=None):
     lib = _hip.load()
     dev = xs[0].device
     C = xs[0].shape[3]
@@ -404,13 +425,16 @@
         v_am = src[2] if len(src) > 2 and src[2] is not None else (None, None)
     else:
         v_am = _wino_transform_in(xs, V, C, Tpad, 0, want_rows=True, want_tensor=keep_v)
+    flags = V_ready[3] if ready and len(V_ready) > 3 else None
+    if flags_out is not None:
+        assert flags_out.dtype == torch.uint8 and flags_out.numel() >= Tpad and len(xs) <= _hip.RN_MAX_GROUP
     Vv = V[:36 * Tpad * C].view(36, 1, Tpad, C)
     Mv = M[:36 * Tpad * cout].view(36, 1, Tpad, cout)
     Uv = _carry_split(U, U.view(36 * cout, U.shape[2]))
     if want_amax() and v_am[0] is None:
         Uv = U.view(36 * cout, U.shape[2])
     conv_igemm(Vv, Uv, Mv, (1, Tpad, cout, 1, 1, 1, 1, 0, 0), flops=2.0 * 36 * T * cout * C, w_batch_stride=cout * U.shape[2],
-               x_amax=v_am[0], x_amax_rows=True)
+               x_amax=v_am[0], x_amax_rows=True, row_active=flags)
     if outs is None:
         outs = [torch.empty((x.shape[0], x.shape[1], x.shape[2], cout), dtype=torch.float32, device=dev) for x in xs]
     off = 0
@@ -429,9 +453,14 @@
         nops = 1 + (pa is not None and pa[0] is not None) + (1.0 / 32 if mbits else 1.0) * has_mask + (1.0 / 32 if signs[0] is not None else 0.0)
         nb = 4.0 * (36 * t * cout + nops * sum(x.shape[0] * x.shape[1] * x.shape[2] for x in part) * cout)
         mm = (mask_mode | (MASK_BITS if mbits else 0)) if has_mask else 0
-        _hip.check(prof.timed("wino_output", nb, lambda: lib.rn_wino_output_group(
-            ctypes.byref(g), M.data_ptr(), cout, off, Tpad, _hip.ptr(scale), _hip.ptr(shift), mm,
-            act, y_batch_stride, _hip.stream())), "rn_wino_output_group")
+        if flags is not None or flags_out is not None:
+            _hip.check(prof.timed("wino_output", nb, lambda: lib.rn_wino_output_group_flags(
+                ctypes.byref(g), M.data_ptr(), cout, off, Tpad, _hip.ptr(scale), _hip.ptr(shift), mm,
+                act, y_batch_stride, _hip.ptr(flags), _hip.ptr(flags_out), _hip.stream())), "rn_wino_output_group_flags")
+        else:
+            _hip.check(prof.timed("wino_output", nb, lambda: lib.rn_wino_output_group(
+                ctypes.byref(g), M.data_ptr(), cout, off, Tpad, _hip.ptr(scale), _hip.ptr(shift), mm,
+                act, y_batch_stride, _hip.stream())), "rn_wino_output_group")
         if yams is not None:
             for o, w_ in zip(outs[sl], yams):
                 amax_attach(o, w_)
@@ -462,7 +491,7 @@
     return st, k
 
 
-def wino_wgrad_group(gs, xs, dw, colsum, flops=0.0, V=None, dU=None, fuse_dgrad_input=False, side=None):
+def wino_wgrad_group(gs, xs, dw, colsum, flops=0.0, V=None, dU=None, fuse_dgrad_input=False, side=None, flags=None):
     lib = _hip.load()
     dev = xs[0].device
     C, cout = xs[0].shape[3], gs[0].shape[3]
@@ -490,11 +519,16 @@
         vd_rows = torch.zeros(Tpad, dtype=torch.int32, device=dev) if am_on else None
         z_tw = amax_single(dev) if am_on else None
         nb = 4.0 * (sum(t.numel() for t in gs) + 2 * 36 * T * cout)
-        _hip.check(prof.timed("wino_input", nb, lambda: lib.rn_wino_input_both_group(
-            ctypes.byref(g), Vd.data_ptr(), Z.data_ptr(), cout, 0, Tpad, _hip.ptr(vd_rows), _hip.ptr(z_tw), _hip.stream())),
-            "rn_wino_input_both_group")
-        v_dy = (Vd, tuple(tuple(t.shape) for t in gs), (vd_rows, None))
+        if flags is not None and not wino_flags_ok(T, C, cout):
+            flags = None
+        if flags is not None:
+            assert flags.dtype == torch.uint8 and flags.numel() >= Tpad
+        _hip.check(prof.timed("wino_input", nb, lambda: lib.rn_wino_input_both_group_flags(
+            ctypes.byref(g), Vd.data_ptr(), Z.data_ptr(), cout, 0, Tpad, _hip.ptr(vd_rows), _hip.ptr(z_tw), _hip.ptr(flags),
+            _hip.stream())), "rn_wino_input_both_group_flags")
+        v_dy = (Vd, tuple(tuple(t.shape) for t in gs), (vd_rows, None)) + ((flags,) if flags is not None else ())
     else:
+        flags = None
         z_tw = _wino_transform_in(gs, Z, cout, Tpad, 1, want_tensor=True)[1]
     am = (z_tw, v_tw) if (want_amax() and z_tw is not None and v_tw is not None) else (None, None)
     ku = (C + 31) // 32 * 32
@@ -503,7 +537,7 @@
     def reductions():
         rc = prof.timed("conv_wgrad" + (" winograd T%d %d->%d" % (T, C, cout) if prof.BY_SHAPE else ""), 2.0 * 36 * T * cout * C, lambda: _wgrad_call(
             lib, dev, Z.data_ptr(), cout, V.data_ptr(), dU.data_ptr(), _hip.ptr(colsum), 36, Tpad * cout, Tpad * C, cout * ku, 7,
-            (1, 1, T, C, 1, T, cout, 1, 1, 1, 0, 0), amax=am))
+            (1, 1, T, C, 1, T, cout, 1, 1, 1, 0, 0), amax=am, flags=flags))
         _hip.check(rc, "rn_conv_wgrad_batched")
         _hip.check(lib.rn_wino_dw(dU.data_ptr(), dw.data_ptr(), cout, C, _hip.stream()), "rn_wino_dw")
     if zst is None:
@@ -513,7 +547,7 @@
         with torch.cuda.stream(side):
             reductions()
             zst["ev"][zk] = side.record_event()
-        SIDE_HELD.setdefault(side.cuda_stream, []).append((V, dU) + tuple(am))
+        SIDE_HELD.setdefault(side.cuda_stream, []).append((V, dU, flags) + tuple(am))
     return v_dy
 
 
@@ -731,9 +765,18 @@
     return g
 
 
-def sigmoid_bwd_pad(dy_ptr, s_ptr, B, rows_per_image, C, ld, src_batch_stride, device, bf16=False):
+def sigmoid_bwd_pad(dy_ptr, s_ptr, B, rows_per_image, C, ld, src_batch_stride, device, bf16=False, hw=None, flags=None):
     lib = _hip.load()
     out = torch.empty((B * rows_per_image, ld), dtype=torch.bfloat16 if bf16 else torch.float32, device=device)
+    if flags is not None:
+        H, W = hw
+        assert not bf16 and H * W == rows_per_image and flags.dtype == torch.uint8 and flags.numel() >= B * ((H + 3) // 4) * ((W + 3) // 4)
+        am = amax_slot(device, B) if want_amax() else None
+        _hip.check(lib.rn_sigmoid_bwd_pad_flags(dy_ptr, s_ptr, out.data_ptr(), B, H, W, C, ld, src_batch_stride, _hip.ptr(am),
+                                                flags.data_ptr(), _hip.stream()), "rn_sigmoid_bwd_pad_flags")
+        if am is not None:
+            out._rn_amax_words = am
+        return out
     if bf16:
         _hip.check(lib.rn_sigmoid_bwd_pad_bf16(dy_ptr, s_ptr, out.data_ptr(), B, rows_per_image, C, ld, src_batch_stride, _hip.stream()),
                    "rn_sigmoid_bwd_pad_bf16")
diff --git a/3d-playground_amd/retinanet_mi355x/engine.py b/3d-playground_amd/retinanet_mi355x/engine.py
--- a/3d-playground_amd/retinanet_mi355x/engine.py
+++ b/3d-playground_amd/retinanet_mi355x/engine.py
@@ -6,6 +6,7 @@
 
 
 FUSE_DY = os.environ.get("RN_WINO_FUSE_DY", "1") != "0"
+SPARSE_REG = os.environ.get("RN_SPARSE_REG", "1") != "0"
 GROUPED_WGRAD_BF16 = os.environ.get("RN_GROUPED_WGRAD_BF16", "1") != "0"
 S2_SHORTCUT_COMPACT = os.environ.get("RN_S2_SHORTCUT_COMPACT", "1") != "0"
 STEM_BF16_PRODUCTS = os.environ.get("RN_STEM_BF16_PRODUCTS", "1") != "0"
@@ -258,9 +259,10 @@
                 y._rn_qscale = self.out_scale
         return ys
 
-    def bwd_data_group(self, gs, in_hws, adds=None, masks=None, wino=False):
+    def bwd_data_group(self, gs, in_hws, adds=None, masks=None, wino=False, flags_out=None):
         s = self.spec
         assert s.stride == 1
+        self.flags_out_done = False
         if self.bf16:
             probs, outs, fl = [], [], 0.0
             for i, g in enumerate(gs):
@@ -275,7 +277,9 @@
         if (wino or self.wino_active) and self.wino_ok and all(g.shape[3] == s.cout for g in gs):
             fl = sum(self.flops(g.shape[0], g.shape[1], g.shape[2]) for g in gs)
             ready, self.dy_v = getattr(self, "dy_v", None), None
-            return cv.wino_conv_group(gs, self.wino_weights(1), adds=adds, masks=masks, mask_mode=2, flops=fl, V_ready=ready)
+            self.flags_out_done = flags_out is not None
+            return cv.wino_conv_group(gs, self.wino_weights(1), adds=adds, masks=masks, mask_mode=2, flops=fl, V_ready=ready,
+                                      flags_out=flags_out)
         probs, outs, fl = [], [], 0.0
         for i, g in enumerate(gs):
             N = g.shape[0]
@@ -310,7 +314,7 @@
         cv.wgrad(g, x, self.dw, s.cout, s.k, s.stride, s.pad, kw_pad=self.kw_pad, in_relu=in_relu,
                  flops=self.flops(g.shape[0], g.shape[1], g.shape[2]), colsum=self.cs)
 
-    def bwd_params_group(self, gs, xs, wino=False, side=None):
+    def bwd_params_group(self, gs, xs, wino=False, side=None, flags=None):
         s = self.spec
         if (wino or self.wino_active) and self.wino_ok and all(g.shape[3] == s.cout and g.is_contiguous() for g in gs):
             if self.dw is None:
@@ -318,7 +322,8 @@
                 self.cs = torch.zeros(s.cout, dtype=torch.float32, device=gs[0].device)
             fl = sum(self.flops(g.shape[0], g.shape[1], g.shape[2]) for g in gs)
             du, self.du = getattr(self, "du", None), None
-            self.dy_v = cv.wino_wgrad_group(gs, xs, self.dw, self.cs, flops=fl, V=self.saved_v, dU=du, fuse_dgrad_input=FUSE_DY, side=side)
+            self.dy_v = cv.wino_wgrad_group(gs, xs, self.dw, self.cs, flops=fl, V=self.saved_v, dU=du, fuse_dgrad_input=FUSE_DY, side=side,
+                                            flags=flags)
             self.saved_v = None
             return
         if self.bf16 and GROUPED_WGRAD_BF16 and 1 < len(gs) <= 5 and all(g.is_contiguous() and x.is_contiguous() for g, x in zip(gs, xs)) \
@@ -735,14 +740,16 @@
         for L in layers:
             L.dw = L.cs = L.wd = L.uf = L.ud = L.saved_v = L.dy_v = None
 
-    def _zero_grad_accumulators(self, device):
+    def _zero_grad_accumulators(self, device, flag_bytes=0, flag_arrays=0):
         wino = self.use_wino and not self.bwd16
         sizes = []
         for L in self.layers.values():
             s = L.spec
             du = 36 * s.cout * ((s.cin + 31) // 32 * 32) if (wino and L.wino_layer) else 0
             sizes.append((L, L.wf.numel(), (s.cout + 3) // 4 * 4, du))
-        total = sum(a + b + c for _, a, b, c in sizes)
+        total = (sum(a + b + c for _, a, b, c in sizes) + 3) // 4 * 4
+        acc_floats = total
+        total += flag_arrays * flag_bytes // 4
         arena = getattr(self, "_arena", None)
         if arena is None or arena.numel() != total or arena.device != device:
             arena = self._arena = torch.empty(total, dtype=torch.float32, device=device)
@@ -753,6 +760,8 @@
             L.cs = arena[o + a:o + a + L.spec.cout]
             L.du = arena[o + a + b:o + a + b + c].view(36, L.spec.cout, -1) if c else None
             o += a + b + c
+        fb = arena[acc_floats:].view(torch.uint8)
+        self._reg_flags = [fb[i * flag_bytes:(i + 1) * flag_bytes] for i in range(flag_arrays)]
 
     def calibrate(self, P, frames, margin=1.0):
         if self.fp8 or self.bf16:
@@ -928,7 +937,9 @@
     def backward(self, S, dreg, dcls, cls):
         Ls = self.layers
         grads = {}
-        self._zero_grad_accumulators(dreg.device)
+        sparse_reg = SPARSE_REG and self.use_wino and not self.bwd16 and not self.bf16 and not self.fp8 and dreg.is_cuda
+        reg_tiles = [dreg.shape[0] * ((f.shape[1] + 3) // 4) * ((f.shape[2] + 3) // 4) for f in S["pyramid"]]
+        self._zero_grad_accumulators(dreg.device, cv.wino_tpad(sum(reg_tiles)) if sparse_reg else 0, 5 if sparse_reg else 0)
         for L in Ls.values():
             L.saved_v = L.dy_v = None
         for n, v in S.pop("wino_v", {}).items():
@@ -975,11 +986,11 @@
             else:
                 aside(lambda: L.bwd_params(g, x, in_relu=in_relu), (g, x))
 
-        def wg_group(L, gs, xs, wino=False):
+        def wg_group(L, gs, xs, wino=False, flags=None):
             if wss is None or os.environ.get("RN_WGRAD_TOWERS", "0") == "0":
-                L.bwd_params_group(gs, xs, wino=wino)
+                L.bwd_params_group(gs, xs, wino=wino, flags=flags)
             elif wino or L.wino_active:
-                L.bwd_params_group(gs, xs, wino=wino, side=wss[0])
+                L.bwd_params_group(gs, xs, wino=wino, side=wss[0], flags=flags)
             else:
                 aside(lambda: L.bwd_params_group(gs, xs), tuple(gs) + tuple(xs))
 
@@ -1021,20 +1032,28 @@
                 side[ti].wait_event(fork)
             with torch.cuda.stream(side[ti] if side is not None else main):
                 acts = [[ACT(t) for t in lvl] for lvl in S["towers"][prefix]]
-                gs, off = [], 0
-                for (Hh, Ww), cnt in zip(hws, counts):
+                F = self._reg_flags if (ti == 0 and sparse_reg and Lout.wino_active) else None
+                fl = F[0] if F else None
+                gs, off, t_off = [], 0, 0
+                for li, ((Hh, Ww), cnt) in enumerate(zip(hws, counts)):
                     byte_off = 4 * off * width
                     g = cv.sigmoid_bwd_pad(dout.data_ptr() + byte_off, None if sig is None else sig.data_ptr() + byte_off,
                                            B, Hh * Ww, arch.NUM_ANCHORS * width, Lout.cout_pad, A * width, dout.device,
-                                           bf16=self.bwd16)
+                                           bf16=self.bwd16, hw=(Hh, Ww), flags=None if fl is None else fl[t_off:t_off + reg_tiles[li]])
                     gs.append(cv.amax_carry(g.view(B, Hh, Ww, Lout.cout_pad), g))
                     off += cnt
-                wg_group(Lout, gs, [acts[li][3] for li in range(5)])
-                gs = Lout.bwd_data_group(gs, hws, masks=[acts[li][3] for li in range(5)])
+                    t_off += reg_tiles[li]
+                wg_group(Lout, gs, [acts[li][3] for li in range(5)], flags=fl)
+                nxt = F[1] if fl is not None else None
+                gs = Lout.bwd_data_group(gs, hws, masks=[acts[li][3] for li in range(5)], flags_out=nxt)
+                fl = nxt if Lout.flags_out_done else None
                 for i in (3, 2, 1):
-                    wg_group(tower[i], gs, [acts[li][i - 1] for li in range(5)], wino=self.use_wino and not self.bwd16)
-                    gs = tower[i].bwd_data_group(gs, hws, masks=[acts[li][i - 1] for li in range(5)], wino=self.use_wino and not self.bwd16)
-                wg_group(tower[0], gs, pyramid, wino=self.use_wino and not self.bwd16)
+                    wg_group(tower[i], gs, [acts[li][i - 1] for li in range(5)], wino=self.use_wino and not self.bwd16, flags=fl)
+                    nxt = F[5 - i] if fl is not None else None
+                    gs = tower[i].bwd_data_group(gs, hws, masks=[acts[li][i - 1] for li in range(5)], wino=self.use_wino and not self.bwd16,
+                                                 flags_out=nxt)
+                    fl = nxt if tower[i].flags_out_done else None
+                wg_group(tower[0], gs, pyramid, wino=self.use_wino and not self.bwd16, flags=fl)
                 first = dpyr[0] is None
                 if side is not None and not first:
                     side[ti].wait_stream(side[0])
diff --git a/include/retinanet_mi355x.h b/include/retinanet_mi355x.h
--- a/include/retinanet_mi355x.h
+++ b/include/retinanet_mi355x.h
@@ -210,6 +210,7 @@
     void *y_amax;
     const float *w_unscale;
     int x_amax_img_stride, x_amax_row_stride;
+    const void *row_active;
 } rn_conv_desc;
 #define RN_MASK_BITS 4
 
@@ -271,6 +272,11 @@
                               int Cin, int Ho, int Wo, int Cout, int kh, int kw, int stride, int pad, int in_relu,
                               const void *dy_amax, int dy_amax_n, const void *x_amax, int x_amax_n, void *workspace, int64_t workspace_bytes,
                               void *stream);
+int rn_conv_wgrad_batched_flags(const float *dy, int ldy, const float *x, float *dw, float *colsum, int nbatch,
+                                int64_t dy_bstride, int64_t x_bstride, int64_t dw_bstride, int colsum_batch, int N, int Hi, int Wi,
+                                int Cin, int Ho, int Wo, int Cout, int kh, int kw, int stride, int pad, int in_relu,
+                                const void *dy_amax, int dy_amax_n, const void *x_amax, int x_amax_n, const void *k_active,
+                                void *workspace, int64_t workspace_bytes, void *stream);
 
 int rn_f32_to_bf16(const float *src, void *dst, int64_t n, void *stream);
 int rn_bf16_to_f32(const void *src, float *dst, int64_t n, void *stream);
@@ -322,6 +328,11 @@
                              void *v_row_amax, void *z_tensor_amax, void *stream);
 int rn_wino_output_group(const rn_wino_group *g, const float *M, int Cout, int64_t tile_offset, int64_t Tpad,
                          const float *scale, const float *shift, int mask_mode, int act, int64_t y_batch_stride, void *stream);
+int rn_wino_input_both_group_flags(const rn_wino_group *g, float *V, float *Z, int C, int64_t tile_offset, int64_t Tpad,
+                                   void *v_row_amax, void *z_tensor_amax, const void *flags, void *stream);
+int rn_wino_output_group_flags(const rn_wino_group *g, const float *M, int Cout, int64_t tile_offset, int64_t Tpad,
+                               const float *scale, const float *shift, int mask_mode, int act, int64_t y_batch_stride,
+                               const void *flags_in, void *flags_out, void *stream);
 int rn_wino_input(const float *x, float *V, int N, int H, int W, int C, int64_t tile_offset, int64_t Tpad, void *stream);
 int rn_wino_output(const float *M, float *y, int N, int H, int W, int Cout, int64_t tile_offset, int64_t Tpad,
                    const float *scale, const float *shift, const float *add, const float *mask, int mask_mode, int act,
@@ -370,6 +381,8 @@
 int rn_relu_mask(float *g, const float *z, int64_t n, void *stream);
 int rn_sigmoid_bwd_pad(const float *dy, const float *s, float *out, int B, int64_t rows_per_image, int C, int ld,
                        int64_t src_batch_stride, void *amax, void *stream);
+int rn_sigmoid_bwd_pad_flags(const float *dy, const float *s, float *out, int B, int H, int W, int C, int ld,
+                             int64_t src_batch_stride, void *amax, void *flags, void *stream);
 int rn_add_inplace(float *dst, const float *src, int64_t n, int64_t per_image, void *amax, void *stream);
 
 int64_t rn_opt_workspace_bytes(int n_chunks);
```

Result: faster. 134.1 images/sec, median of 6 (+5.5%).
